# algbio/founderblockgraphs

Hardware: AMD Instinct MI355X
Metric: MSA columns segmented/sec (higher is better)
Workload: dtype u32

## Files before the change

founderblockgraphs_amd/csrc/ctx.hip:

```cpp
#include "fbg_internal.h"
#include <chrono>
#include <stdarg.h>
#include <stdio.h>
#include <ctype.h>
#include <string.h>
#include <algorithm>
#include <atomic>
#include <thread>
#include <vector>

static std::string g_global_err;

int fbg_fail(fbg_ctx *ctx, int code, const char *fmt, ...)
{
    char buf[1024];
    va_list ap;
    va_start(ap, fmt);
    vsnprintf(buf, sizeof(buf), fmt, ap);
    va_end(ap);
    if (ctx) ctx->err = buf; else g_global_err = buf;
    return code;
}

int fbg_reserve(fbg_ctx *ctx, DevBuf &b, size_t bytes, std::vector<DevBuf *> *owner, bool accounted)
{
    if (bytes == 0) bytes = 256;
    if (b.cap >= bytes) return FBG_OK;
    const auto t_begin = std::chrono::steady_clock::now();
    if (b.p) {
        FBG_HIP_TRY(ctx, hipStreamSynchronize(ctx->stream));
        FBG_HIP_TRY(ctx, hipFree(b.p));
        if (accounted) ctx->held_bytes -= b.cap;
        b.p = nullptr; b.cap = 0;
    }
    size_t want = (bytes + 255) & ~(size_t)255;
    hipError_t e = hipMalloc(&b.p, want);
    if (e != hipSuccess) {
        b.p = nullptr;
        return fbg_fail(ctx, FBG_ERR_OOM, "hipMalloc(%zu bytes) failed: %s (context already holds %llu bytes)",
                        want, hipGetErrorString(e), (unsigned long long)ctx->held_bytes);
    }
    b.cap = want;
    if (owner && !b.listed) { owner->push_back(&b); b.listed = true; }
    if (!accounted) return FBG_OK;
    ctx->held_bytes += want;
    ctx->alloc_calls++;
    ctx->alloc_us += (uint64_t)std::chrono::duration_cast<std::chrono::microseconds>(std::chrono::steady_clock::now() - t_begin).count();
    if (ctx->opt.poison) FBG_HIP_TRY(ctx, hipMemsetAsync(b.p, (int)(ctx->opt.poison & 255), want, ctx->stream));
    return FBG_OK;
}

void fbg_release(fbg_ctx *ctx, DevBuf &b)
{
    if (b.p) {
        (void)hipFree(b.p);
        if (ctx) ctx->held_bytes -= b.cap;
        b.p = nullptr; b.cap = 0;
    }
}

void fbg_release_all(fbg_ctx *ctx, std::vector<DevBuf *> &bufs)
{
    for (DevBuf *b : bufs) { fbg_release(ctx, *b); b->listed = false; }
    bufs.clear();
}

#define FBG_STAGE_SLOT (8u << 20)
#define FBG_STAGE_SLOTS 16
#define FBG_STAGE_MIN (32u << 20)

static bool host_pointer_is_pinned(const void *p)
{
    hipPointerAttribute_t at;
    const hipError_t e = hipPointerGetAttributes(&at, p);
    if (e != hipSuccess) { (void)hipGetLastError(); return false; }
    return at.type == hipMemoryTypeHost;
}

static int stager_ready(fbg_ctx *ctx)
{
    Stager &s = ctx->stager;
    if (s.base) return FBG_OK;
    FBG_HIP_TRY(ctx, hipHostMalloc(&s.base, (size_t)FBG_STAGE_SLOT * FBG_STAGE_SLOTS, hipHostMallocDefault));
    s.slot_bytes = FBG_STAGE_SLOT; s.nslots = FBG_STAGE_SLOTS;
    s.ev = new hipEvent_t[s.nslots];
    for (int i = 0; i < s.nslots; i++) FBG_HIP_TRY(ctx, hipEventCreateWithFlags(&s.ev[i], hipEventDisableTiming));
    FBG_HIP_TRY(ctx, hipStreamCreateWithFlags(&s.stream, hipStreamNonBlocking));
    return FBG_OK;
}

static int staged_copy(fbg_ctx *ctx, void *dst, const void *src, size_t bytes, bool to_device)
{
    FBG_HIP_TRY(ctx, hipSetDevice(ctx->device));
    FBG_HIP_TRY(ctx, hipStreamSynchronize(ctx->stream));
    const void *host = to_device ? src : dst;
    if (bytes < FBG_STAGE_MIN || host_pointer_is_pinned(host)) {
        FBG_HIP_TRY(ctx, hipMemcpyAsync(dst, src, bytes, to_device ? hipMemcpyHostToDevice : hipMemcpyDeviceToHost, ctx->stream));
        FBG_HIP_TRY(ctx, hipStreamSynchronize(ctx->stream));
        return FBG_OK;
    }
    FBG_TRY(stager_ready(ctx));
    Stager &s = ctx->stager;
    const size_t nchunks = (bytes + s.slot_bytes - 1) / s.slot_bytes;
    unsigned hw = std::thread::hardware_concurrency();
    int T = (int)std::min<size_t>(std::min<unsigned>(std::max(2u, hw / 2), 8u), nchunks);
    if (T > s.nslots / 2) T = s.nslots / 2;
    std::atomic<int> failed{0};
    auto worker = [&](int t) {
        if (hipSetDevice(ctx->device) != hipSuccess) { failed = 1; return; }
        const int slots[2] = {t, t + T};
        uint8_t *pins[2] = {static_cast<uint8_t *>(s.base) + (size_t)slots[0] * s.slot_bytes,
                            static_cast<uint8_t *>(s.base) + (size_t)slots[1] * s.slot_bytes};
        if (to_device) {
            size_t k = 0;
            for (size_t c = (size_t)t; c < nchunks && !failed; c += (size_t)T, k++) {
                const int w = (int)(k & 1);
                const size_t off = c * s.slot_bytes, len = std::min(s.slot_bytes, bytes - off);
                if (k >= 2 && hipEventSynchronize(s.ev[slots[w]]) != hipSuccess) { failed = 1; return; }
                memcpy(pins[w], static_cast<const uint8_t *>(src) + off, len);
                if (hipMemcpyAsync(static_cast<uint8_t *>(dst) + off, pins[w], len, hipMemcpyHostToDevice, s.stream) != hipSuccess ||
                    hipEventRecord(s.ev[slots[w]], s.stream) != hipSuccess) { failed = 1; return; }
            }
        } else {
            auto issue = [&](size_t c, int w) {
                const size_t off = c * s.slot_bytes, len = std::min(s.slot_bytes, bytes - off);
                return hipMemcpyAsync(pins[w], static_cast<const uint8_t *>(src) + off, len, hipMemcpyDeviceToHost, s.stream) == hipSuccess &&
                       hipEventRecord(s.ev[slots[w]], s.stream) == hipSuccess;
            };
            if ((size_t)t < nchunks && !issue((size_t)t, 0)) { failed = 1; return; }
            size_t k = 0;
            for (size_t c = (size_t)t; c < nchunks && !failed; c += (size_t)T, k++) {
                const int w = (int)(k & 1);
                if (c + (size_t)T < nchunks && !issue(c + (size_t)T, w ^ 1)) { failed = 1; return; }
                if (hipEventSynchronize(s.ev[slots[w]]) != hipSuccess) { failed = 1; return; }
                const size_t off = c * s.slot_bytes, len = std::min(s.slot_bytes, bytes - off);
                memcpy(static_cast<uint8_t *>(dst) + off, pins[w], len);
            }
        }
    };
    std::vector<std::thread> th;
    for (int t = 1; t < T; t++) th.emplace_back(worker, t);
    worker(0);
    for (auto &t : th) t.join();
    FBG_HIP_TRY(ctx, hipStreamSynchronize(s.stream));
    if (failed) return fbg_fail(ctx, FBG_ERR_HIP, "staged %s copy of %zu bytes failed: %s", to_device ? "host-to-device" : "device-to-host",
                                bytes, hipGetErrorString(hipGetLastError()));
    return FBG_OK;
}

int fbg_upload(fbg_ctx *ctx, void *d_dst, const void *h_src, size_t bytes) { return staged_copy(ctx, d_dst, h_src, bytes, true); }
int fbg_download(fbg_ctx *ctx, void *h_dst, const void *d_src, size_t bytes) { return staged_copy(ctx, h_dst, d_src, bytes, false); }

int fbg_stage_begin(fbg_ctx *ctx, int stage)
{
    StageTimer &t = ctx->timers[stage];
    if (!t.start) {
        FBG_HIP_TRY(ctx, hipEventCreate(&t.start));
        FBG_HIP_TRY(ctx, hipEventCreate(&t.stop));
    }
    t.recorded = false;
    FBG_HIP_TRY(ctx, hipEventRecord(t.start, ctx->stream));
    return FBG_OK;
}

int fbg_stage_end(fbg_ctx *ctx, int stage, int launches)
{
    StageTimer &t = ctx->timers[stage];
    FBG_HIP_TRY(ctx, hipEventRecord(t.stop, ctx->stream));
    t.recorded = true;
    t.launches = launches;
    return FBG_OK;
}

struct OptKey { const char *name; int64_t FbgOptions::*field; };
static const OptKey g_opt_keys[] = {
    {"no_ranked", &FbgOptions::no_ranked},
    {"no_packed", &FbgOptions::no_packed},
    {"force_wide", &FbgOptions::force_wide},
    {"full_keys", &FbgOptions::full_keys},
    {"no_msd_sort", &FbgOptions::no_msd_sort},
    {"msd_min", &FbgOptions::msd_min},
    {"bp_min", &FbgOptions::bp_min},
    {"record_scatter", &FbgOptions::record_scatter},
    {"lcp_text", &FbgOptions::lcp_text},
    {"no_aux_stream", &FbgOptions::no_aux_stream},
    {"rank_no_threshold", &FbgOptions::rank_no_threshold},
    {"dp_literal", &FbgOptions::dp_literal},
    {"dp_wave", &FbgOptions::dp_wave},
    {"dp_safe_window", &FbgOptions::dp_safe_window},
    {"dp_tile", &FbgOptions::dp_tile},
    {"pure_scan", &FbgOptions::pure_scan},
    {"gapped_rank", &FbgOptions::gapped_rank},
    {"part_tricks_off", &FbgOptions::part_tricks_off},
    {"msd_sample_bins", &FbgOptions::msd_sample_bins},
    {"msd_min_force", &FbgOptions::msd_min_force},
    {"msd_probe", &FbgOptions::msd_probe},
    {"msd_xcd", &FbgOptions::msd_xcd},
    {"rank_no_lean", &FbgOptions::rank_no_lean},
    {"no_stream_upload", &FbgOptions::no_stream_upload},
    {"span_scan", &FbgOptions::span_scan},
    {"span_key_flags", &FbgOptions::span_key_flags},
    {"span_slow_split", &FbgOptions::span_slow_split},
    {"poison", &FbgOptions::poison},
    {"dpw_matrix", &FbgOptions::dpw_matrix},
    {"dp_chain1", &FbgOptions::dp_chain1},
    {"msd_ext", &FbgOptions::msd_ext},
    {"rows_wave", &FbgOptions::rows_wave},
    {"pairs_in_scan", &FbgOptions::pairs_in_scan},
    {"runs_wave_min", &FbgOptions::runs_wave_min},
    {"wave_list_cap", &FbgOptions::wave_list_cap},
    {"cand_local_sort", &FbgOptions::cand_local_sort},
    {"cand_lds_cap", &FbgOptions::cand_lds_cap},
    {"cand_sort_check", &FbgOptions::cand_sort_check},
    {"tie_gallop", &FbgOptions::tie_gallop},
    {"cand_counts_fused", &FbgOptions::cand_counts_fused},
    {"tie_sample_loop", &FbgOptions::tie_sample_loop},
    {"row_count_fast", &FbgOptions::row_count_fast},
    {"twin_hash", &FbgOptions::twin_hash},
    {"front_one_fill", &FbgOptions::front_one_fill},
    {"scan_rows_ahead", &FbgOptions::scan_rows_ahead},
    {"msd_cursors", &FbgOptions::msd_cursors},
    {"msd_lds_batch", &FbgOptions::msd_lds_batch},
    {"path_batch_kib", &FbgOptions::path_batch_kib},
    {"byrow_max", &FbgOptions::byrow_max},
    {"byrow_lds", &FbgOptions::byrow_lds},
    {"graph_batch_kib", &FbgOptions::graph_batch_kib},
};

struct InfoKey { const char *name; int64_t (*get)(const fbg_ctx &); };
static const InfoKey g_info_keys[] = {
    {"grs_threshold", [](const fbg_ctx &c) -> int64_t { return c.grs_t; }},
    {"grs_redone", [](const fbg_ctx &c) -> int64_t { return (int64_t)c.grs_redone; }},
    {"dp_kind", [](const fbg_ctx &c) -> int64_t { return c.dp_kind; }},
    {"dp_attempts", [](const fbg_ctx &c) -> int64_t { return c.dp_attempts; }},
    {"ne_dp_kind", [](const fbg_ctx &c) -> int64_t { return c.ne_dp_kind; }},
    {"msd_decline", [](const fbg_ctx &c) -> int64_t { return c.diag.msd_decline; }},
    {"pass1_ahead", [](const fbg_ctx &c) -> int64_t { return c.diag.pass1_ahead; }},
    {"ext_pairs", [](const fbg_ctx &c) -> int64_t { return c.diag.ext_pairs; }},
    {"text_pairs", [](const fbg_ctx &c) -> int64_t { return c.diag.text_pairs; }},
    {"sample_twins", [](const fbg_ctx &c) -> int64_t { return c.diag.sample_twins; }},
    {"cand_inversions", [](const fbg_ctx &c) -> int64_t { return c.diag.cand_inversions; }},
    {"cand_local_sorted", [](const fbg_ctx &c) -> int64_t { return c.diag.cand_local_sorted; }},
    {"wave_runs", [](const fbg_ctx &c) -> int64_t { return c.diag.wave_runs; }},
    {"rank_lean_used", [](const fbg_ctx &c) -> int64_t { return c.diag.rank_lean_used; }},
    {"rank_lean_launched", [](const fbg_ctx &c) -> int64_t { return c.diag.rank_lean_launched; }},
    {"pairs_rb", [](const fbg_ctx &c) -> int64_t { return c.diag.pairs_rb; }},
    {"key_b", [](const fbg_ctx &c) -> int64_t { return c.key_b; }},
    {"key_K", [](const fbg_ctx &c) -> int64_t { return c.key_K; }},
    {"key_packed", [](const fbg_ctx &c) -> int64_t { return c.key_packed; }},
    {"key_compact", [](const fbg_ctx &c) -> int64_t { return c.key_compact; }},
    {"alloc_calls", [](const fbg_ctx &c) -> int64_t { return (int64_t)c.alloc_calls; }},
    {"alloc_us", [](const fbg_ctx &c) -> int64_t { return (int64_t)c.alloc_us; }},
    {"span_decline", [](const fbg_ctx &c) -> int64_t { return c.diag.sp_decline; }},
    {"span_key_flags_used", [](const fbg_ctx &c) -> int64_t { return c.ix.index_valid && c.ix.spanned() && c.ix.sp_key_flags_sorted; }},
    {"span_scan_used", [](const fbg_ctx &c) -> int64_t { return c.ix.index_valid && c.ix.spanned(); }},
    {"span_scan_work", [](const fbg_ctx &c) -> int64_t { return (int64_t)c.sp_work; }},
    {"span_groups", [](const fbg_ctx &c) -> int64_t { return (int64_t)c.sp_G; }},
    {"span_odd_groups", [](const fbg_ctx &c) -> int64_t { return (int64_t)c.sp_n_odd[0] + c.sp_n_odd[1] + c.sp_n_odd[2] + c.sp_n_odd[3]; }},
    {"span_irregular", [](const fbg_ctx &c) -> int64_t { return (int64_t)c.sp_n_irr; }},
    {"span_chain", [](const fbg_ctx &c) -> int64_t { return (int64_t)c.sp_chain_n; }},
    {"span_slow_groups", [](const fbg_ctx &c) -> int64_t { return (int64_t)c.sp_slow_n; }},
    {"index_kind", [](const fbg_ctx &c) -> int64_t { return !c.ix.index_valid ? -1 : c.ix.part_active ? 3 : c.ix.granked() ? 2 : c.ix.ranked() ? 1 : 0; }},
};

static void options_from_env(FbgOptions &o)
{
    auto env = [](const std::string &name) -> const char * { return getenv(name.c_str()); };
    const char *dbg = env("FBG_DEBUG_ENV");
    if (!dbg || strcmp(dbg, "1") != 0) return;
    for (const OptKey &k : g_opt_keys) {
        std::string name = "FBG_";
        for (const char *c = k.name; *c; c++) name += (char)toupper((unsigned char)*c);
        if (const char *v = env(name)) o.*(k.field) = *v ? strtoll(v, nullptr, 10) : 1;
    }
}

void fbg_index_reset(fbg_ctx *ctx)
{
    ctx->ix = IndexState();
    ctx->diag = BuildDiag();
}

static int host_dp_v(fbg_ctx *ctx, int (*dp)(fbg_ctx *, const uint64_t *, uint64_t, uint64_t *, uint64_t *, uint64_t *, uint64_t *), const char *name,
                     const uint64_t *v, uint64_t n, uint64_t *s_out, uint64_t *prev_out, uint64_t *boundaries_out, uint64_t *count_out)
{
    if (!ctx) return FBG_ERR_INVALID;
    if (!v || !boundaries_out || !count_out || n == 0 || n >= (1ull << 31))
        return fbg_fail(ctx, FBG_ERR_INVALID, "%s: bad arguments", name);
    FBG_HIP_TRY(ctx, hipSetDevice(ctx->device));
    size_t w = n * sizeof(uint64_t);
    for (DevBuf *b : {&ctx->io_a, &ctx->io_b, &ctx->io_c, &ctx->io_d}) FBG_TRY(fbg_reserve(ctx, *b, w));
    FBG_HIP_TRY(ctx, hipMemcpyAsync(ctx->io_a.p, v, w, hipMemcpyHostToDevice, ctx->stream));
    int rc = dp(ctx, ctx->io_a.as<uint64_t>(), n, ctx->io_c.as<uint64_t>(), ctx->io_d.as<uint64_t>(), ctx->io_b.as<uint64_t>(), count_out);
    if (rc != FBG_OK && rc != FBG_ERR_NO_SEGMENTATION) return rc;
    if (s_out) FBG_HIP_TRY(ctx, hipMemcpyAsync(s_out, ctx->io_c.p, w, hipMemcpyDeviceToHost, ctx->stream));
    if (prev_out) FBG_HIP_TRY(ctx, hipMemcpyAsync(prev_out, ctx->io_d.p, w, hipMemcpyDeviceToHost, ctx->stream));
    if (rc == FBG_OK)
        FBG_HIP_TRY(ctx, hipMemcpyAsync(boundaries_out, ctx->io_b.p, *count_out * sizeof(uint64_t),
                                        hipMemcpyDeviceToHost, ctx->stream));
    FBG_HIP_TRY(ctx, hipStreamSynchronize(ctx->stream));
    return rc;
}

extern "C" {

int fbg_set_option(fbg_ctx *ctx, const char *key, int64_t value)
{
    if (!ctx || !key) return FBG_ERR_INVALID;
    for (const OptKey &k : g_opt_keys)
        if (strcmp(k.name, key) == 0) { ctx->opt.*(k.field) = value; return FBG_OK; }
    return fbg_fail(ctx, FBG_ERR_INVALID, "fbg_set_option: unknown key '%s'", key);
}

int fbg_get_option(const fbg_ctx *ctx, const char *key, int64_t *value)
{
    if (!ctx || !key || !value) return FBG_ERR_INVALID;
    for (const OptKey &k : g_opt_keys)
        if (strcmp(k.name, key) == 0) { *value = ctx->opt.*(k.field); return FBG_OK; }
    for (const InfoKey &k : g_info_keys)
        if (strcmp(k.name, key) == 0) { *value = k.get(*ctx); return FBG_OK; }
    if (strncmp(key, "span_dbg", 8) == 0 && key[8] >= '0' && key[8] <= '7' && !key[9]) {
        unsigned long long v = 0;
        if (hipStreamSynchronize(ctx->stream) != hipSuccess || ctx->scalars.cap < FBG_SCALARS_BYTES ||
            hipMemcpy(&v, fbg_scalars(ctx)->span + 24 + (key[8] - '0'), 8, hipMemcpyDeviceToHost) != hipSuccess) return FBG_ERR_HIP;
        *value = (int64_t)v;
        return FBG_OK;
    }
    return FBG_ERR_INVALID;
}

void *fbg_host_alloc(uint64_t bytes)
{
    void *p = nullptr;
    if (hipHostMalloc(&p, bytes ? bytes : 1, hipHostMallocDefault) != hipSuccess) { (void)hipGetLastError(); return nullptr; }
    return p;
}
void fbg_host_free(void *p) { if (p) (void)hipHostFree(p); }

int fbg_ctx_create(int device, fbg_ctx **out)
{
    if (!out) return FBG_ERR_INVALID;
    *out = nullptr;
    int count = 0;
    hipError_t e = hipGetDeviceCount(&count);
    if (e != hipSuccess || count <= 0)
        return fbg_fail(nullptr, FBG_ERR_NO_DEVICE,
                        "no HIP device visible (%s); libfbg_hip has no CPU fallback",
                        e != hipSuccess ? hipGetErrorString(e) : "device count 0");
    if (device < 0 || device >= count)
        return fbg_fail(nullptr, FBG_ERR_INVALID, "device %d out of range (0..%d)", device, count - 1);
    e = hipSetDevice(device);
    if (e != hipSuccess) return fbg_fail(nullptr, FBG_ERR_HIP, "hipSetDevice: %s", hipGetErrorString(e));
    fbg_ctx *ctx = new fbg_ctx();
    ctx->device = device;
    options_from_env(ctx->opt);
    e = hipStreamCreateWithFlags(&ctx->stream, hipStreamNonBlocking);
    if (e != hipSuccess) {
        delete ctx;
        return fbg_fail(nullptr, FBG_ERR_HIP, "hipStreamCreate: %s", hipGetErrorString(e));
    }
    ctx->own_stream = true;
    *out = ctx;
    return FBG_OK;
}

void fbg_ctx_destroy(fbg_ctx *ctx)
{
    if (!ctx) return;
    (void)hipSetDevice(ctx->device);
    (void)hipStreamSynchronize(ctx->stream);
    fbg_release_all(ctx, ctx->bufs);
    fbg_msd_pre_free(ctx);
    if (ctx->up_stream) {
        (void)hipStreamSynchronize(ctx->up_stream);
        for (auto &e : ctx->up_ev) if (e) (void)hipEventDestroy(e);
        (void)hipStreamDestroy(ctx->up_stream);
    }
    for (auto &t : ctx->timers) {
        if (t.start) (void)hipEventDestroy(t.start);
        if (t.stop) (void)hipEventDestroy(t.stop);
    }
    if (ctx->stager.base) {
        for (int i = 0; i < ctx->stager.nslots; i++) (void)hipEventDestroy(ctx->stager.ev[i]);
        delete[] ctx->stager.ev;
        (void)hipStreamDestroy(ctx->stager.stream);
        (void)hipHostFree(ctx->stager.base);
    }
    if (ctx->pin_pair) (void)hipHostFree(ctx->pin_pair);
    if (ctx->pin_twins) (void)hipHostFree(ctx->pin_twins);
    if (ctx->twin_ev) (void)hipEventDestroy(ctx->twin_ev);
    if (ctx->pin_front) (void)hipHostFree(ctx->pin_front);
    if (ctx->aux_fork) (void)hipEventDestroy(ctx->aux_fork);
    if (ctx->aux_join) (void)hipEventDestroy(ctx->aux_join);
    if (ctx->aux) (void)hipStreamDestroy(ctx->aux);
    if (ctx->own_stream) (void)hipStreamDestroy(ctx->stream);
    delete ctx;
}

const char *fbg_last_error(const fbg_ctx *ctx) { return ctx ? ctx->err.c_str() : g_global_err.c_str(); }

int fbg_set_stream(fbg_ctx *ctx, void *hip_stream)
{
    if (!ctx) return FBG_ERR_INVALID;
    FBG_HIP_TRY(ctx, hipStreamSynchronize(ctx->stream));
    if (ctx->own_stream) { (void)hipStreamDestroy(ctx->stream); ctx->own_stream = false; }
    if (hip_stream) {
        ctx->stream = (hipStream_t)hip_stream;
    } else {
        FBG_HIP_TRY(ctx, hipStreamCreateWithFlags(&ctx->stream, hipStreamNonBlocking));
        ctx->own_stream = true;
    }
    return FBG_OK;
}

int fbg_stage_ms(fbg_ctx *ctx, int stage, float *ms, int *launches)
{
    if (!ctx || stage < 0 || stage >= FBG_STAGE_COUNT) return FBG_ERR_INVALID;
    StageTimer &t = ctx->timers[stage];
    if (ms) *ms = 0.f;
    if (launches) *launches = 0;
    if (!t.recorded) return FBG_OK;
    FBG_HIP_TRY(ctx, hipEventSynchronize(t.stop));
    float v = 0.f;
    FBG_HIP_TRY(ctx, hipEventElapsedTime(&v, t.start, t.stop));
    if (ms) *ms = v;
    if (launches) *launches = t.launches;
    return FBG_OK;
}

uint64_t fbg_device_bytes(const fbg_ctx *ctx) { return ctx ? ctx->held_bytes : 0; }

int fbg_release_scratch(fbg_ctx *ctx)
{
    if (!ctx) return FBG_ERR_INVALID;
    FBG_HIP_TRY(ctx, hipSetDevice(ctx->device));
    FBG_HIP_TRY(ctx, hipStreamSynchronize(ctx->stream));
    const bool sorted_in_A = (ctx->ix.ranked() || ctx->ix.granked()) && ctx->ix.rk_keys == ctx->keysA.as<uint64_t>();
    const DevBuf *keep[] = {
        &ctx->msa_own, &ctx->text, &ctx->pos, &ctx->tot, &ctx->segtab, &ctx->colT, &ctx->gwin_rows,
        &ctx->valsB, sorted_in_A ? &ctx->keysA : &ctx->keysB,
        &ctx->prow, &ctx->igrow, &ctx->rec, &ctx->xlist, &ctx->gmax, &ctx->excol, &ctx->xslot, &ctx->xbits, &ctx->exc, &ctx->exc_scratch,
        &ctx->big_groups, &ctx->gwin, &ctx->gbits, &ctx->sp_cwin, &ctx->sp_gstart, &ctx->sp_gcol, &ctx->sp_gflags, &ctx->sp_rstart, &ctx->sp_rid,
        &ctx->sp_gplo, &ctx->sp_gphi, &ctx->sp_gval, &ctx->sp_odd, &ctx->sp_irr, &ctx->sp_chain, &ctx->sp_slow, &ctx->sp_mins,
        &ctx->small, &ctx->scalars, &ctx->kargs, &ctx->io_a, &ctx->io_b, &ctx->io_c, &ctx->io_d, &ctx->bt_up, &ctx->bt_dep};
    for (DevBuf *b : ctx->bufs)
        if (std::find(std::begin(keep), std::end(keep), b) == std::end(keep)) fbg_release(ctx, *b);
    return FBG_OK;
}

int fbg_sync(fbg_ctx *ctx)
{
    if (!ctx) return FBG_ERR_INVALID;
    FBG_HIP_TRY(ctx, hipStreamSynchronize(ctx->stream));
    return FBG_OK;
}

static int check_dims(fbg_ctx *ctx, uint64_t m, uint64_t n)
{
    if (!ctx) return FBG_ERR_INVALID;
    if (m == 0 || n == 0) return fbg_fail(ctx, FBG_ERR_INVALID, "empty MSA (m=%llu, n=%llu)",
                                          (unsigned long long)m, (unsigned long long)n);
    if (n >= (1ull << 31) || m * (n + 1) + 1 >= (1ull << 40))
        return fbg_fail(ctx, FBG_ERR_TOO_LARGE, "MSA of %llu x %llu cells is beyond this engine (n < 2^31, text < 2^40)",
                        (unsigned long long)m, (unsigned long long)n);
    return FBG_OK;
}

int fbg_msa_set_device(fbg_ctx *ctx, const uint8_t *d_msa, uint64_t m, uint64_t n)
{
    FBG_TRY(check_dims(ctx, m, n));
    if (!d_msa) return fbg_fail(ctx, FBG_ERR_INVALID, "null MSA pointer");
    ctx->d_msa = d_msa; ctx->m = m; ctx->n = n; ctx->ix.index_valid = false;
    return FBG_OK;
}

int fbg_msa_load_host(fbg_ctx *ctx, const uint8_t *msa, uint64_t m, uint64_t n)
{
    FBG_TRY(check_dims(ctx, m, n));
    if (!msa) return fbg_fail(ctx, FBG_ERR_INVALID, "null MSA pointer");
    FBG_HIP_TRY(ctx, hipSetDevice(ctx->device));
    FBG_TRY(fbg_reserve(ctx, ctx->msa_own, m * n));
    FBG_TRY(fbg_upload(ctx, ctx->msa_own.p, msa, m * n));
    ctx->d_msa = ctx->msa_own.as<uint8_t>(); ctx->m = m; ctx->n = n; ctx->ix.index_valid = false;
    return FBG_OK;
}

int fbg_index_build(fbg_ctx *ctx, int reversed, const uint8_t *ignore_chars, uint64_t ignore_len)
{
    if (!ctx) return FBG_ERR_INVALID;
    if (!ctx->d_msa) return fbg_fail(ctx, FBG_ERR_INVALID, "fbg_index_build: no MSA set");
    FBG_HIP_TRY(ctx, hipSetDevice(ctx->device));
    for (int st : {FBG_STAGE_SORT_PASS1, FBG_STAGE_SORT_PASS2, FBG_STAGE_SORT_PASS3, FBG_STAGE_RANK_KERNEL}) {
        ctx->timers[st].recorded = false;
        ctx->timers[st].launches = 0;
    }
    fbg_index_reset(ctx);
    ctx->reversed = reversed ? 1 : 0;
    FBG_TRY(fbg_build_text(ctx, reversed ? nullptr : ignore_chars, reversed ? 0 : ignore_len));
    FBG_TRY(fbg_suffix_sort(ctx));
    FBG_TRY(fbg_neighbour_lcp(ctx));
    if (ctx->N > 1500000000ull) {
        size_t free_b = 0, total_b = 0;
        FBG_HIP_TRY(ctx, hipMemGetInfo(&free_b, &total_b));
        if (free_b < total_b / 2) FBG_TRY(fbg_release_scratch(ctx));
    }
    ctx->ix.index_valid = true;
    return FBG_OK;
}

int fbg_part_index_build(fbg_ctx *ctx, int reversed, int part, int nparts, void *d_blob, int *ok)
{
    return fbg_part_index_build_ignore(ctx, reversed, part, nparts, nullptr, 0, d_blob, ok);
}

int fbg_part_index_build_ignore(fbg_ctx *ctx, int reversed, int part, int nparts, const uint8_t *ignore_chars, uint64_t ignore_len, void *d_blob, int *ok)
{
    if (!ctx) return FBG_ERR_INVALID;
    if (!ctx->d_msa) return fbg_fail(ctx, FBG_ERR_INVALID, "fbg_part_index_build: no MSA set");
    if (!d_blob || !ok || nparts < 1 || part < 0 || part >= nparts || (ignore_len && !ignore_chars))
        return fbg_fail(ctx, FBG_ERR_INVALID, "fbg_part_index_build: bad arguments");
    FBG_HIP_TRY(ctx, hipSetDevice(ctx->device));
    fbg_index_reset(ctx);
    ctx->reversed = reversed ? 1 : 0;
    ctx->allow_wide = true;
    const int rc = fbg_build_text(ctx, reversed ? nullptr : ignore_chars, reversed ? 0 : ignore_len);
    ctx->allow_wide = false;
    FBG_TRY(rc);
    return fbg_part_sort(ctx, part, nparts, static_cast<uint8_t *>(d_blob), ok);
}

int fbg_part_scan(fbg_ctx *ctx, const void *d_blobs, uint32_t *d_gmax, int *ok)
{
    if (!ctx) return FBG_ERR_INVALID;
    if (!ctx->ix.part_active || ctx->ix.index_valid)
        return fbg_fail(ctx, FBG_ERR_INVALID, "fbg_part_scan needs fbg_part_index_build first");
    if (!d_blobs || !d_gmax || !ok) return fbg_fail(ctx, FBG_ERR_INVALID, "fbg_part_scan: bad arguments");
    FBG_HIP_TRY(ctx, hipSetDevice(ctx->device));
    if (ctx->ix.gpart) return fbg_grs_part_scan(ctx, static_cast<const uint8_t *>(d_blobs), d_gmax, ok);
    return fbg_rank_part_runs(ctx, static_cast<const uint8_t *>(d_blobs), d_gmax, ok);
}

int fbg_part_finish(fbg_ctx *ctx, const uint32_t *d_gmax, int *ok)
{
    if (!ctx) return FBG_ERR_INVALID;
    if (!ctx->ix.part_active || ctx->ix.index_valid)
        return fbg_fail(ctx, FBG_ERR_INVALID, "fbg_part_finish needs fbg_part_scan first");
    if (!d_gmax || !ok) return fbg_fail(ctx, FBG_ERR_INVALID, "fbg_part_finish: bad arguments");
    FBG_HIP_TRY(ctx, hipSetDevice(ctx->device));
    uint32_t verdict = 1;
    FBG_HIP_TRY(ctx, hipMemcpyAsync(ctx->gmax.p, d_gmax, (ctx->n + 1) * 4, hipMemcpyDeviceToDevice, ctx->stream));
    FBG_HIP_TRY(ctx, hipMemcpyAsync(&verdict, d_gmax + ctx->n, 4, hipMemcpyDeviceToHost, ctx->stream));
    FBG_HIP_TRY(ctx, hipStreamSynchronize(ctx->stream));
    *ok = verdict == 0;
    if (*ok) {
        uint64_t unfilled = 0;
        if (ctx->ix.gpart) FBG_TRY(fbg_grs_part_unfilled(ctx, &unfilled));
        else FBG_TRY(fbg_rank_part_unfilled(ctx, &unfilled));
        if (unfilled) { *ok = 2; return FBG_OK; }
        ctx->ix.n_exc = 0; ctx->ix.index_valid = true;
        ctx->ix.kind = ctx->ix.gpart ? IndexKind::gapped : IndexKind::ranked;
    }
    return FBG_OK;
}

int fbg_part_rescan(fbg_ctx *ctx, uint32_t *d_gmax)
{
    if (!ctx) return FBG_ERR_INVALID;
    if (!ctx->ix.part_active || ctx->ix.index_valid)
        return fbg_fail(ctx, FBG_ERR_INVALID, "fbg_part_rescan follows a fbg_part_finish that returned *ok = 2");
    if (!d_gmax) return fbg_fail(ctx, FBG_ERR_INVALID, "fbg_part_rescan: bad arguments");
    FBG_HIP_TRY(ctx, hipSetDevice(ctx->device));
    uint32_t verdict = 0;
    if (ctx->ix.gpart) { FBG_TRY(fbg_grs_part_rescan(ctx)); verdict = ctx->grs_part_failed ? 1u : 0u; }
    else FBG_TRY(fbg_rank_part_rescan(ctx));
    FBG_HIP_TRY(ctx, hipMemcpyAsync(d_gmax, ctx->gmax.p, (ctx->n + 1) * 4, hipMemcpyDeviceToDevice, ctx->stream));
    FBG_HIP_TRY(ctx, hipMemcpyAsync(d_gmax + ctx->n, &verdict, 4, hipMemcpyHostToDevice, ctx->stream));
    FBG_HIP_TRY(ctx, hipStreamSynchronize(ctx->stream));
    return FBG_OK;
}

int fbg_scan_f(fbg_ctx *ctx, uint64_t x0, uint64_t x1, int disable_tricks, uint64_t *d_f)
{
    if (!ctx) return FBG_ERR_INVALID;
    if (!ctx->ix.index_valid || ctx->reversed)
        return fbg_fail(ctx, FBG_ERR_INVALID, "fbg_scan_f needs fbg_index_build(reversed=0) first");
    if (x0 > x1 || x1 > ctx->n || !d_f) return fbg_fail(ctx, FBG_ERR_INVALID, "fbg_scan_f: bad column range");
    FBG_HIP_TRY(ctx, hipSetDevice(ctx->device));
    return fbg_scan_columns(ctx, x0, x1, FBG_SCAN_F, disable_tricks, d_f);
}

int fbg_scan_v(fbg_ctx *ctx, uint64_t x0, uint64_t x1, uint64_t *d_v)
{
    if (!ctx) return FBG_ERR_INVALID;
    if (!ctx->ix.index_valid || !ctx->reversed)
        return fbg_fail(ctx, FBG_ERR_INVALID, "fbg_scan_v needs fbg_index_build(reversed=1) first");
    if (x0 > x1 || x1 > ctx->n || !d_v) return fbg_fail(ctx, FBG_ERR_INVALID, "fbg_scan_v: bad column range");
    FBG_HIP_TRY(ctx, hipSetDevice(ctx->device));
    return fbg_scan_columns(ctx, x0, x1, FBG_SCAN_V, 1, d_v);
}

int fbg_minmax_dp_device(fbg_ctx *ctx, const uint64_t *d_f, uint64_t n, uint64_t *d_boundaries,
                         uint64_t *count_out, uint64_t *d_mml, uint64_t *d_bt)
{
    if (!ctx) return FBG_ERR_INVALID;
    if (!d_f || !d_boundaries || !count_out || n == 0 || n >= (1ull << 31))
        return fbg_fail(ctx, FBG_ERR_INVALID, "fbg_minmax_dp_device: bad arguments");
    FBG_HIP_TRY(ctx, hipSetDevice(ctx->device));
    return fbg_dp_minmax(ctx, d_f, n, d_boundaries, count_out, d_mml, d_bt);
}

int fbg_repeatfree_dp_device(fbg_ctx *ctx, const uint64_t *d_v, uint64_t n, uint64_t *d_s,
                             uint64_t *d_prev, uint64_t *d_boundaries, uint64_t *count_out)
{
    if (!ctx) return FBG_ERR_INVALID;
    if (!d_v || !d_boundaries || !count_out || n == 0 || n >= (1ull << 31))
        return fbg_fail(ctx, FBG_ERR_INVALID, "fbg_repeatfree_dp_device: bad arguments");
    FBG_HIP_TRY(ctx, hipSetDevice(ctx->device));
    return fbg_dp_repeatfree(ctx, d_v, n, d_s, d_prev, d_boundaries, count_out);
}

int fbg_scan_gapped_v(fbg_ctx *ctx, uint64_t *d_v)
{
    if (!ctx) return FBG_ERR_INVALID;
    if (!ctx->ix.index_valid || ctx->reversed)
        return fbg_fail(ctx, FBG_ERR_INVALID, "fbg_scan_gapped_v needs fbg_index_build(reversed=0) first");
    if (!d_v) return fbg_fail(ctx, FBG_ERR_INVALID, "fbg_scan_gapped_v: null d_v");
    FBG_HIP_TRY(ctx, hipSetDevice(ctx->device));
    const uint64_t n = ctx->n;
    FBG_TRY(fbg_reserve(ctx, ctx->io_d, n * sizeof(uint64_t)));
    uint64_t *d_f = ctx->io_d.as<uint64_t>();
    FBG_HIP_TRY(ctx, hipMemsetAsync(d_f, 0, n * sizeof(uint64_t), ctx->stream));
    FBG_TRY(fbg_scan_columns(ctx, 0, n, FBG_SCAN_F, 1, d_f));
    return fbg_gapped_v_from_f(ctx, d_f, n, d_v);
}

int fbg_gapped_dp_device(fbg_ctx *ctx, const uint64_t *d_v, uint64_t n, uint64_t *d_s,
                         uint64_t *d_prev, uint64_t *d_boundaries, uint64_t *count_out)
{
    if (!ctx) return FBG_ERR_INVALID;
    if (!d_v || !d_boundaries || !count_out || n == 0 || n >= (1ull << 31))
        return fbg_fail(ctx, FBG_ERR_INVALID, "fbg_gapped_dp_device: bad arguments");
    FBG_HIP_TRY(ctx, hipSetDevice(ctx->device));
    return fbg_dp_gapped(ctx, d_v, n, d_s, d_prev, d_boundaries, count_out);
}


int fbg_elastic_f(fbg_ctx *ctx, const uint8_t *msa, uint64_t m, uint64_t n, const uint8_t *ignore_chars,
                  uint64_t ignore_len, int disable_tricks, uint64_t *f)
{
    if (!ctx) return FBG_ERR_INVALID;
    if (!f) return fbg_fail(ctx, FBG_ERR_INVALID, "fbg_elastic_f: null f");
    if (msa && ignore_len == 0 && !ctx->opt.no_stream_upload && m * n >= FBG_STAGE_MIN && host_pointer_is_pinned(msa) && check_dims(ctx, m, n) == FBG_OK) {
        FBG_HIP_TRY(ctx, hipSetDevice(ctx->device));
        FBG_HIP_TRY(ctx, hipStreamSynchronize(ctx->stream));
        FBG_TRY(fbg_reserve(ctx, ctx->msa_own, m * n));
        ctx->d_msa = ctx->msa_own.as<uint8_t>(); ctx->m = m; ctx->n = n; ctx->ix.index_valid = false;
        ctx->up_host = msa;
        const int rc = fbg_index_build(ctx, 0, ignore_chars, ignore_len);
        ctx->up_host = nullptr;
        if (ctx->up_stream) (void)hipStreamSynchronize(ctx->up_stream);
        if (rc != FBG_OK) return rc;
    } else {
        FBG_TRY(fbg_msa_load_host(ctx, msa, m, n));
        FBG_TRY(fbg_index_build(ctx, 0, ignore_chars, ignore_len));
    }
    FBG_TRY(fbg_reserve(ctx, ctx->io_a, n * sizeof(uint64_t)));
    FBG_HIP_TRY(ctx, hipMemcpyAsync(ctx->io_a.p, f, n * sizeof(uint64_t), hipMemcpyHostToDevice, ctx->stream));
    FBG_TRY(fbg_scan_f(ctx, 0, n, disable_tricks, ctx->io_a.as<uint64_t>()));
    FBG_HIP_TRY(ctx, hipMemcpyAsync(f, ctx->io_a.p, n * sizeof(uint64_t), hipMemcpyDeviceToHost, ctx->stream));
    FBG_HIP_TRY(ctx, hipStreamSynchronize(ctx->stream));
    if (disable_tricks && f[0] == n)
        return fbg_fail(ctx, FBG_ERR_NO_SEGMENTATION, "No valid segmentation found!");
    return FBG_OK;
}

int fbg_minmax_dp(fbg_ctx *ctx, const uint64_t *f, uint64_t n, uint64_t *boundaries_out, uint64_t *count_out,
                  uint64_t *minmaxlength_out, uint64_t *backtrack_out)
{
    if (!ctx) return FBG_ERR_INVALID;
    if (!f || !boundaries_out || !count_out || n == 0 || n >= (1ull << 31))
        return fbg_fail(ctx, FBG_ERR_INVALID, "fbg_minmax_dp: bad arguments");
    FBG_HIP_TRY(ctx, hipSetDevice(ctx->device));
    size_t w = (n + 1) * sizeof(uint64_t);
    for (DevBuf *b : {&ctx->io_a, &ctx->io_b, &ctx->io_c, &ctx->io_d}) FBG_TRY(fbg_reserve(ctx, *b, w));
    FBG_HIP_TRY(ctx, hipMemcpyAsync(ctx->io_a.p, f, n * sizeof(uint64_t), hipMemcpyHostToDevice, ctx->stream));
    int rc = fbg_dp_minmax(ctx, ctx->io_a.as<uint64_t>(), n, ctx->io_b.as<uint64_t>(), count_out,
                           ctx->io_c.as<uint64_t>(), ctx->io_d.as<uint64_t>());
    if (rc != FBG_OK && rc != FBG_ERR_NO_SEGMENTATION) return rc;
    if (minmaxlength_out)
        FBG_HIP_TRY(ctx, hipMemcpyAsync(minmaxlength_out, ctx->io_c.p, w, hipMemcpyDeviceToHost, ctx->stream));
    if (backtrack_out)
        FBG_HIP_TRY(ctx, hipMemcpyAsync(backtrack_out, ctx->io_d.p, w, hipMemcpyDeviceToHost, ctx->stream));
    if (rc == FBG_OK)
        FBG_HIP_TRY(ctx, hipMemcpyAsync(boundaries_out, ctx->io_b.p, *count_out * sizeof(uint64_t),
                                        hipMemcpyDeviceToHost, ctx->stream));
    FBG_HIP_TRY(ctx, hipStreamSynchronize(ctx->stream));
    return rc;
}

int fbg_repeatfree_v(fbg_ctx *ctx, const uint8_t *msa, uint64_t m, uint64_t n, uint64_t *v)
{
    if (!ctx) return FBG_ERR_INVALID;
    if (!v) return fbg_fail(ctx, FBG_ERR_INVALID, "fbg_repeatfree_v: null v");
    FBG_TRY(fbg_msa_load_host(ctx, msa, m, n));
    FBG_TRY(fbg_index_build(ctx, 1, nullptr, 0));
    FBG_TRY(fbg_reserve(ctx, ctx->io_a, n * sizeof(uint64_t)));
    FBG_TRY(fbg_scan_v(ctx, 0, n, ctx->io_a.as<uint64_t>()));
    FBG_HIP_TRY(ctx, hipMemcpyAsync(v, ctx->io_a.p, n * sizeof(uint64_t), hipMemcpyDeviceToHost, ctx->stream));
    FBG_HIP_TRY(ctx, hipStreamSynchronize(ctx->stream));
    return FBG_OK;
}

int fbg_repeatfree_dp(fbg_ctx *ctx, const uint64_t *v, uint64_t n, uint64_t *s_out, uint64_t *prev_out,
                      uint64_t *boundaries_out, uint64_t *count_out)
{
    return host_dp_v(ctx, fbg_dp_repeatfree, "fbg_repeatfree_dp", v, n, s_out, prev_out, boundaries_out, count_out);
}

int fbg_gapped_v(fbg_ctx *ctx, const uint8_t *msa, uint64_t m, uint64_t n, uint64_t *v)
{
    if (!ctx) return FBG_ERR_INVALID;
    if (!v) return fbg_fail(ctx, FBG_ERR_INVALID, "fbg_gapped_v: null v");
    FBG_TRY(fbg_msa_load_host(ctx, msa, m, n));
    FBG_TRY(fbg_index_build(ctx, 0, nullptr, 0));
    FBG_TRY(fbg_reserve(ctx, ctx->io_a, n * sizeof(uint64_t)));
    FBG_TRY(fbg_scan_gapped_v(ctx, ctx->io_a.as<uint64_t>()));
    FBG_HIP_TRY(ctx, hipMemcpyAsync(v, ctx->io_a.p, n * sizeof(uint64_t), hipMemcpyDeviceToHost, ctx->stream));
    FBG_HIP_TRY(ctx, hipStreamSynchronize(ctx->stream));
    return FBG_OK;
}

int fbg_gapped_dp(fbg_ctx *ctx, const uint64_t *v, uint64_t n, uint64_t *s_out, uint64_t *prev_out,
                  uint64_t *boundaries_out, uint64_t *count_out)
{
    return host_dp_v(ctx, fbg_dp_gapped, "fbg_gapped_dp", v, n, s_out, prev_out, boundaries_out, count_out);
}

uint64_t fbg_text_length(const fbg_ctx *ctx) { return ctx && ctx->ix.index_valid ? ctx->N : 0; }

int fbg_index_download(fbg_ctx *ctx, uint8_t *text, uint32_t *sa, uint32_t *isa, uint32_t *lcp_prev,
                       uint32_t *lcp_next)
{
    if (!ctx) return FBG_ERR_INVALID;
    if (!ctx->ix.index_valid) return fbg_fail(ctx, FBG_ERR_INVALID, "fbg_index_download: no index");
    if (ctx->ix.part_active) return fbg_fail(ctx, FBG_ERR_INVALID, "fbg_index_download: the index is partitioned over several GPUs");
    if (ctx->N >= (1ull << 32)) return fbg_fail(ctx, FBG_ERR_TOO_LARGE, "fbg_index_download: 32-bit arrays");
    if (ctx->ix.spanned() && (sa || isa || lcp_prev || lcp_next))
        return fbg_fail(ctx, FBG_ERR_INVALID, "fbg_index_download: the group-level scan (span_scan.hip) leaves the suffixes with equal keys unordered; "
                                              "set option span_scan = -1 for an index with a suffix array");
    size_t N = ctx->N;
    FBG_HIP_TRY(ctx, hipStreamSynchronize(ctx->stream));
    if (text) FBG_HIP_TRY(ctx, hipMemcpy(text, ctx->text.p, N, hipMemcpyDeviceToHost));
    if (sa && !ctx->ix.ranked() && !ctx->ix.granked()) FBG_HIP_TRY(ctx, hipMemcpy(sa, ctx->ix.sa_ptr, N * 4, hipMemcpyDeviceToHost));
    if ((sa || isa || lcp_prev || lcp_next) && (ctx->ix.ranked() || ctx->ix.granked())) {
        for (DevBuf *b : {&ctx->io_a, &ctx->io_b, &ctx->io_c, &ctx->io_d}) FBG_TRY(fbg_reserve(ctx, *b, N * 4));
        if (ctx->ix.granked())
            FBG_TRY(fbg_grs_materialize(ctx, ctx->io_d.as<uint32_t>(), ctx->io_a.as<uint32_t>(), ctx->io_b.as<uint32_t>(), ctx->io_c.as<uint32_t>()));
        else
            FBG_TRY(fbg_rank_materialize(ctx, ctx->io_d.as<uint32_t>(), ctx->io_a.as<uint32_t>(), ctx->io_b.as<uint32_t>(),
                                         ctx->io_c.as<uint32_t>()));
        FBG_HIP_TRY(ctx, hipStreamSynchronize(ctx->stream));
        if (sa) FBG_HIP_TRY(ctx, hipMemcpy(sa, ctx->io_d.p, N * 4, hipMemcpyDeviceToHost));
        if (isa) FBG_HIP_TRY(ctx, hipMemcpy(isa, ctx->io_a.p, N * 4, hipMemcpyDeviceToHost));
        if (lcp_prev) FBG_HIP_TRY(ctx, hipMemcpy(lcp_prev, ctx->io_b.p, N * 4, hipMemcpyDeviceToHost));
        if (lcp_next) FBG_HIP_TRY(ctx, hipMemcpy(lcp_next, ctx->io_c.p, N * 4, hipMemcpyDeviceToHost));
    } else if (isa || lcp_prev || lcp_next) {
        uint32_t *dst[3] = {isa, lcp_prev, lcp_next};
        for (int w = 0; w < 3; w++) {
            if (!dst[w]) continue;
            FBG_HIP_TRY(ctx, hipMemcpy2DAsync(dst[w], 4, (const char *)ctx->rec.p + 4 * w, 16, 4, N,
                                              hipMemcpyDeviceToHost, ctx->stream));
        }
        FBG_HIP_TRY(ctx, hipStreamSynchronize(ctx->stream));
        for (int w = 1; w < 3; w++)
            if (dst[w]) for (size_t k = 0; k < N; k++) dst[w][k] &= 0x7fffffffu;
    }
    FBG_HIP_TRY(ctx, hipStreamSynchronize(ctx->stream));
    return FBG_OK;
}

}
```

founderblockgraphs_amd/csrc/fbg_internal.h:

```cpp
#pragma once
#include <cstddef>
#include <cstring>
#include <cstdlib>
#include <hip/hip_runtime.h>
#include <stdint.h>
#include <string>
#include <vector>
#include "../../include/fbg_hip.h"

#define FBG_WAVE 64

struct DevBuf {
    void *p = nullptr;
    size_t cap = 0;
    bool listed = false;
    template <class T> T *as() const { return reinterpret_cast<T *>(p); }
};

struct Stager {
    void *base = nullptr;
    size_t slot_bytes = 0;
    int nslots = 0;
    hipEvent_t *ev = nullptr;
    hipStream_t stream = nullptr;
};

struct StageTimer {
    hipEvent_t start = nullptr, stop = nullptr;
    bool recorded = false;
    int launches = 0;
};

struct FbgOptions {
    int64_t no_ranked = 0, no_packed = 0, force_wide = 0, full_keys = 0, no_msd_sort = 0, msd_min = -1, bp_min = -1,
            record_scatter = 0, lcp_text = 0, no_aux_stream = 0, rank_no_threshold = 0, dp_literal = 0, dp_wave = 0,
            dp_safe_window = 0, dp_tile = 0, pure_scan = 0, gapped_rank = 0, part_tricks_off = 0, msd_sample_bins = 0, msd_min_force = 0, msd_probe = 0, msd_xcd = -1, rank_no_lean = 0, no_stream_upload = 0,
            span_scan = 0, span_key_flags = 0, span_slow_split = 0, poison = 0, dpw_matrix = 0, dp_chain1 = 0, msd_ext = 1, rows_wave = 0,
            pairs_in_scan = 1, runs_wave_min = 16, wave_list_cap = 0,
            cand_local_sort = 1, cand_lds_cap = 0, cand_sort_check = 0,
            tie_gallop = 1, cand_counts_fused = 1, tie_sample_loop = 1,
            row_count_fast = 1, twin_hash = 1, front_one_fill = 1,
            scan_rows_ahead = 0, msd_cursors = 1, msd_lds_batch = 1,
            path_batch_kib = 1 << 20, byrow_max = 1024, byrow_lds = 0, graph_batch_kib = 1 << 20;
};

enum class IndexKind { none, record, ranked, gapped, span };

struct IndexState {
    bool index_valid = false;
    IndexKind kind = IndexKind::none;
    bool ranked() const { return kind == IndexKind::ranked; }
    bool granked() const { return kind == IndexKind::gapped || kind == IndexKind::span; }
    bool spanned() const { return kind == IndexKind::span; }
    uint32_t *sa_ptr = nullptr;
    uint64_t *rk_keys = nullptr;
    int rk_b = 0, rk_key_bits = 0, rk_K = 0;
    int rk_layout = 0, rk_pb = 0;
    bool grs_flagged = false;
    bool sp_key_flags_sorted = false;
    bool msd_ext_valid = false;
    bool lcp_from_keys = false;
    bool grs_ties_done = false;
    uint32_t n_exc = 0;
    bool part_active = false;
    bool gpart = false;
    int part = 0, nparts = 1;
    uint64_t part_count = 0;
    uint64_t part_T = 0;
    uint32_t part_gmin = 0;
};

struct BuildDiag {
    int64_t msd_decline = -1;
    int pass1_ahead = 0;
    int64_t ext_pairs = -1, text_pairs = -1;
    int64_t sample_twins = -1;
    int64_t wave_runs = -1;
    int64_t cand_inversions = -1;
    int cand_local_sorted = -1;
    int rank_lean_launched = 0;
    int rank_lean_used = 0;
    int pairs_rb = -1;
    int sp_decline = 0;
};

struct SortExtras {
    const uint64_t *ebits = nullptr;
    const uint32_t *payload = nullptr;
    bool key_flags = false;
};

struct MsdPlan;
struct fbg_ctx {
    int device = 0;
    FbgOptions opt;
    std::string err;
    hipStream_t stream = nullptr;
    bool own_stream = false;
    hipStream_t aux = nullptr;
    hipEvent_t aux_fork = nullptr, aux_join = nullptr;
    bool aux_pending = false;
    uint32_t *pin_pair = nullptr;
    unsigned long long *pin_twins = nullptr;
    hipEvent_t twin_ev = nullptr;
    bool twin_pending = false;
    unsigned long long *pin_front = nullptr;
    Stager stager;
    StageTimer timers[FBG_STAGE_COUNT];

    const uint8_t *d_msa = nullptr;
    DevBuf msa_own;
    uint64_t m = 0, n = 0;
    int reversed = 0;
    bool gapfree = true;
    bool have_ignore = false;
    uint8_t ignore_tab[256] = {0};
    uint64_t N = 0;
    uint64_t byte_hist[256] = {0};
    bool allow_wide = false;
    uint32_t mp = 0;
    DevBuf text;
    DevBuf pos, tot;
    DevBuf segtab;
    DevBuf colT;
    DevBuf gwin_rows;

    const uint8_t *up_host = nullptr;
    hipStream_t up_stream = nullptr;
    hipEvent_t up_ev[9] = {};
    bool pre_pass1 = false;
    uint64_t pre_symbols[4] = {0, 0, 0, 0};
    MsdPlan *pre_plan = nullptr;
    uint64_t pre_tiles = 0;

    IndexState ix;
    BuildDiag diag;
    int key_b = -1, key_K = -1, key_packed = -1, key_compact = -1;
    int dp_kind = -1;
    int dp_attempts = 0;
    int ne_dp_kind = -1;
    bool grs_skip = false;
    bool cells_built = false;
    uint64_t held_bytes = 0;
    uint64_t alloc_calls = 0, alloc_us = 0;
    std::vector<DevBuf *> bufs;

    DevBuf prow;
    DevBuf igrow;
    DevBuf rec;
    DevBuf xlist;
    DevBuf gmax, excol, xslot;
    DevBuf xbits;
    DevBuf exc_scratch;
    DevBuf exc;
    int grs_tricks_off = 0;
    uint32_t grs_ign_lo = 0, grs_ign_hi = 0;
    DevBuf gwin;
    DevBuf gbits;
    bool pairs_similar = false;
    bool grs_part_failed = false;
    uint32_t grs_t = 1;
    uint64_t grs_redone = 0;
    DevBuf sp_cells;
    DevBuf sp_flagT;
    DevBuf sp_cwin;
    DevBuf sp_tiles, sp_gstart, sp_gcol, sp_gflags, sp_rstart, sp_rid, sp_gplo, sp_gphi, sp_gval, sp_odd, sp_irr, sp_chain, sp_slow, sp_mins;
    uint32_t sp_chain_n = 0, sp_slow_n = 0;
    uint64_t sp_G = 0, sp_R = 0, sp_n_irr = 0, sp_work = 0;
    uint32_t sp_n_odd[4] = {0, 0, 0, 0}, sp_odd_cap = 0;

    DevBuf keysA, keysB, valsA, valsB, grp, flags, list, tie_list, big_groups, tmp, small, scalars;
    DevBuf msd_ext;
    DevBuf wave_list;
    DevBuf kargs;
    alignas(16) unsigned char kargs_host[512];
    uint8_t code_host[256];
    DevBuf msd_w, msd_v;
    DevBuf dp_a, dp_b, dp_c, dp_d, dp_e, dp_f, dp_g, dp_h, io_a, io_b, io_c, io_d;
    DevBuf bt_up, bt_dep;
    DevBuf ps_a, ps_b, ps_c, ps_d, ps_e, ps_f, ps_g, ps_h;
};

int fbg_fail(fbg_ctx *ctx, int code, const char *fmt, ...);
#define FBG_HIP_TRY(ctx, expr)                                                              \
    do {                                                                                    \
        hipError_t e_ = (expr);                                                             \
        if (e_ != hipSuccess)                                                               \
            return fbg_fail((ctx), e_ == hipErrorOutOfMemory ? FBG_ERR_OOM : FBG_ERR_HIP,   \
                            "%s failed: %s (%s:%d)", #expr, hipGetErrorString(e_), __FILE__, \
                            __LINE__);                                                      \
    } while (0)
#define FBG_TRY(expr)                \
    do {                             \
        int rc_ = (expr);            \
        if (rc_ != FBG_OK) return rc_; \
    } while (0)

int fbg_reserve(fbg_ctx *ctx, DevBuf &b, size_t bytes, std::vector<DevBuf *> *owner, bool accounted);
inline int fbg_reserve(fbg_ctx *ctx, DevBuf &b, size_t bytes) { return fbg_reserve(ctx, b, bytes, &ctx->bufs, true); }

struct FbgScalars {
    alignas(64) unsigned long long front[8];
    unsigned long long sample_count;
    alignas(64) unsigned long long dp[16];
    unsigned long long scan_exceptions;
    alignas(64) unsigned long long rank[8];
    unsigned long long rank_hist[32];
    alignas(64) unsigned long long pure[4];
    alignas(64) unsigned long long msd[4];
    unsigned long long sample_twins;
    unsigned long long graph_collision;
    unsigned long long pair_stats[2];
    unsigned long long cand_inversions;
    unsigned long long by_position;
    alignas(64) unsigned long long gapped[8 + 66];
    alignas(64) unsigned long long span[34];
};
constexpr size_t FBG_SCALARS_WORDS = 256, FBG_SCALARS_BYTES = FBG_SCALARS_WORDS * sizeof(unsigned long long);
static_assert(sizeof(FbgScalars) <= FBG_SCALARS_BYTES, "the scalar words fit their buffer, whose size is part of fbg_device_bytes");
static_assert(offsetof(FbgScalars, rank_hist) == offsetof(FbgScalars, rank) + sizeof(FbgScalars::rank), "one fill clears counters and histogram");
inline int fbg_reserve_scalars(fbg_ctx *ctx) { return fbg_reserve(ctx, ctx->scalars, FBG_SCALARS_BYTES); }
inline FbgScalars *fbg_scalars(const fbg_ctx *ctx) { return ctx->scalars.as<FbgScalars>(); }

struct FbgSmall {
    alignas(2048) uint8_t ignore_tab[256];
    alignas(2048) uint8_t code_tab[256];
    alignas(2048) unsigned long long hist[256];
};
constexpr size_t FBG_SMALL_BYTES = 8192;
static_assert(sizeof(FbgSmall) <= FBG_SMALL_BYTES, "the byte tables fit their buffer");
inline FbgSmall *fbg_small(const fbg_ctx *ctx) { return ctx->small.as<FbgSmall>(); }

template <class F> int fbg_with_tmp(fbg_ctx *ctx, DevBuf &tmp, std::vector<DevBuf *> *owner, bool accounted, F &&call)
{
    size_t bytes = 0;
    hipError_t e = call(nullptr, bytes);
    if (e != hipSuccess) return fbg_fail(ctx, FBG_ERR_HIP, "rocprim size query: %s", hipGetErrorString(e));
    FBG_TRY(fbg_reserve(ctx, tmp, bytes, owner, accounted));
    size_t have = tmp.cap;
    e = call(tmp.p, have);
    if (e != hipSuccess)
        return fbg_fail(ctx, e == hipErrorOutOfMemory ? FBG_ERR_OOM : FBG_ERR_HIP, "rocprim call: %s", hipGetErrorString(e));
    return FBG_OK;
}
template <class F> int fbg_with_tmp(fbg_ctx *ctx, F &&call) { return fbg_with_tmp(ctx, ctx->tmp, &ctx->bufs, true, call); }

void fbg_release(fbg_ctx *ctx, DevBuf &b);
void fbg_release_all(fbg_ctx *ctx, std::vector<DevBuf *> &bufs);
void fbg_index_reset(fbg_ctx *ctx);
int fbg_upload(fbg_ctx *ctx, void *d_dst, const void *h_src, size_t bytes);
int fbg_download(fbg_ctx *ctx, void *h_dst, const void *d_src, size_t bytes);
int fbg_stage_begin(fbg_ctx *ctx, int stage);
int fbg_stage_end(fbg_ctx *ctx, int stage, int launches);

#define FBG_SLOTS_PAIRS 0
#define FBG_SLOTS_PACKED 1
#define FBG_SLOTS_WIDE 2
struct KeyGeom {
    int b = 0, K = 0, key_bits = 0;
    bool compact = false, packed = false;
    bool wide = false;
    int pb = 0;
    const uint8_t *d_code = nullptr;
};

inline void fbg_remember_slots(fbg_ctx *ctx, uint64_t *keys, uint32_t *vals, int layout, const KeyGeom &g)
{
    ctx->ix.rk_keys = keys; ctx->ix.sa_ptr = vals; ctx->ix.rk_layout = layout; ctx->ix.rk_pb = g.pb;
    ctx->ix.rk_b = g.b; ctx->ix.rk_key_bits = g.key_bits; ctx->ix.rk_K = g.K;
}

inline void fbg_note_key_geom(fbg_ctx *ctx, const KeyGeom &g)
{
    ctx->key_b = g.b; ctx->key_K = g.K; ctx->key_packed = g.packed ? 1 : 0; ctx->key_compact = g.compact ? 1 : 0;
}

int fbg_build_text(fbg_ctx *ctx, const uint8_t *ignore, uint64_t ignore_len);
int fbg_suffix_sort(fbg_ctx *ctx);
int fbg_neighbour_lcp(fbg_ctx *ctx);
int fbg_rank_scan_try(fbg_ctx *ctx, uint64_t *keys, uint32_t *vals, const KeyGeom &g, int *done);
int fbg_pure_scan_try(fbg_ctx *ctx, uint64_t *keys, uint32_t *vals, const KeyGeom &g, int *done);
int fbg_rank_finish(fbg_ctx *ctx, uint64_t x0, uint64_t x1, int mode, int disable_tricks, uint64_t *d_out);
int fbg_rank_materialize(fbg_ctx *ctx, uint32_t *d_sa, uint32_t *d_isa, uint32_t *d_pl, uint32_t *d_pr);
#define FBG_STAGE_RANKSCAN FBG_STAGE_TILE
int fbg_grs_prepare(fbg_ctx *ctx, const uint64_t **ebits, int *launches);
int fbg_grs_part_classify(fbg_ctx *ctx, uint64_t *keys, uint32_t *vals, uint64_t count, const KeyGeom &g, int eligible, uint8_t *d_blob, int *ok);
int fbg_grs_part_scan(fbg_ctx *ctx, const uint8_t *d_blobs, uint32_t *d_gmax, int *ok);
int fbg_grs_part_unfilled(fbg_ctx *ctx, uint64_t *unfilled);
int fbg_grs_part_rescan(fbg_ctx *ctx);
int fbg_grs_strip(fbg_ctx *ctx, uint32_t *vals);
int fbg_grs_try(fbg_ctx *ctx, uint64_t *keys, uint32_t *vals, const KeyGeom &g, int *done);
int fbg_grs_finish(fbg_ctx *ctx, uint64_t x0, uint64_t x1, int disable_tricks, uint64_t *d_out, int *ok);
int fbg_grs_materialize(fbg_ctx *ctx, uint32_t *d_sa, uint32_t *d_isa, uint32_t *d_pl, uint32_t *d_pr);
bool fbg_span_eligible(fbg_ctx *ctx, const KeyGeom &g);
bool fbg_span_key_flags(fbg_ctx *ctx, KeyGeom &g);
int fbg_span_prepare(fbg_ctx *ctx, const KeyGeom &g, const SortExtras &x, int *launches);
int fbg_span_try(fbg_ctx *ctx, uint64_t *keys, uint32_t *vals, const KeyGeom &g, int *done);
int fbg_span_rescan(fbg_ctx *ctx, int disable_tricks, int *ok);
int fbg_build_cell_tables(fbg_ctx *ctx);
int fbg_key_setup(fbg_ctx *ctx, bool compact, KeyGeom *g, int *launches);
int fbg_rank_part_classify(fbg_ctx *ctx, uint64_t *keys, uint32_t *vals, uint64_t count, const KeyGeom &g, int pre_ok,
                           uint8_t *d_blob, int *ok);
int fbg_rank_part_runs(fbg_ctx *ctx, const uint8_t *d_blobs, uint32_t *d_gmax, int *ok);
int fbg_rank_part_unfilled(fbg_ctx *ctx, uint64_t *unfilled);
int fbg_rank_part_rescan(fbg_ctx *ctx);
int fbg_part_sort(fbg_ctx *ctx, int part, int nparts, uint8_t *d_blob, int *ok);
int fbg_msd_sort(fbg_ctx *ctx, const KeyGeom &g, uint64_t **sorted, int *ok, int *launches);
int fbg_msd_pre_begin(fbg_ctx *ctx, int *ok);
int fbg_msd_pre_pass1(fbg_ctx *ctx, uint64_t avail);
bool fbg_msd_pre_geom(fbg_ctx *ctx, KeyGeom *g);
void fbg_msd_pre_free(fbg_ctx *ctx);
int fbg_msd_sort_part(fbg_ctx *ctx, const KeyGeom &g, uint64_t lo, uint64_t hi, int nohi, int nparts, uint64_t out_offset,
                      uint64_t *count, int *ok, int *launches);
int fbg_sample_sort_pairs(fbg_ctx *ctx, const KeyGeom &g, const SortExtras &x, int *ok, int *launches);
int fbg_scan_columns(fbg_ctx *ctx, uint64_t x0, uint64_t x1, int mode, int disable_tricks,
                     uint64_t *d_out);
int fbg_dp_minmax(fbg_ctx *ctx, const uint64_t *d_f, uint64_t n, uint64_t *d_boundaries,
                  uint64_t *count_out, uint64_t *d_mml, uint64_t *d_bt);
struct BlockGraphDev {
    const uint64_t *bounds = nullptr;
    const uint32_t *node_of = nullptr, *rep_row = nullptr, *count = nullptr;
    const unsigned long long *first = nullptr, *edge_count = nullptr, *edges = nullptr;
    uint64_t n_nodes = 0;
    bool collision = false;
};
int fbg_block_graph_device(fbg_ctx *ctx, const uint64_t *boundaries, uint64_t nb, BlockGraphDev *g);
int fbg_dp_repeatfree(fbg_ctx *ctx, const uint64_t *d_v, uint64_t n, uint64_t *d_s,
                      uint64_t *d_prev, uint64_t *d_boundaries, uint64_t *count_out);
int fbg_gapped_v_from_f(fbg_ctx *ctx, const uint64_t *d_f, uint64_t n, uint64_t *d_v);
int fbg_dp_gapped(fbg_ctx *ctx, const uint64_t *d_v, uint64_t n, uint64_t *d_s, uint64_t *d_prev,
                  uint64_t *d_boundaries, uint64_t *count_out);

#define FBG_SCAN_F 0
#define FBG_SCAN_V 1

static inline unsigned fbg_blocks(uint64_t work, unsigned per_block, unsigned cap = 0x7fffffffu)
{
    uint64_t b = (work + per_block - 1) / per_block;
    if (b < 1) b = 1;
    if (b > cap) b = cap;
    return (unsigned)b;
}
```

founderblockgraphs_amd/csrc/host/host_selftest.cpp:

```cpp
#include <cstdio>
#include <cstdlib>
#include <string>
#include <vector>
#include "fasta.hpp"
#include "xgfa.hpp"
#include "../tie_extent.h"
#include "../twin_hash.h"
#include "../pindex_stage.h"

static int tie_extent_selftest()
{
    const uint32_t cap = 8192;
    std::vector<uint32_t> sizes;
    for (uint32_t s = 1; s <= 70; s++) sizes.push_back(s);
    for (uint32_t s = 8191; s <= 8194; s++) sizes.push_back(s);
    unsigned long long cases = 0;
    for (const uint32_t s : sizes)
        for (int where = 0; where < 3; where++) {
            const uint64_t before = where == 0 ? 0 : 37, after = where == 2 ? 0 : 29;
            std::vector<uint64_t> keys;
            for (uint64_t i = 0; i < before; i++) keys.push_back(10 + i / 3);
            const uint64_t key = 1000;
            for (uint32_t i = 0; i < s; i++) keys.push_back(key);
            for (uint64_t i = 0; i < after; i++) keys.push_back(2000 + i / 2);
            const uint64_t k0 = before;
            uint64_t reads = 0;
            auto key_at = [&](uint64_t k) -> uint64_t {
                reads++;
                if (k >= keys.size()) { std::fprintf(stderr, "tie_extent: read of slot %llu beyond the array\n", (unsigned long long)k); std::exit(1); }
                return keys[k];
            };
            std::vector<uint64_t> his = {keys.size()};
            for (uint64_t cut = 0; cut <= 3 && cut < s; cut++) his.push_back(k0 + s - cut);
            for (const uint64_t hi : his) {
                uint32_t want = 1;
                while (k0 + want < hi && want <= cap && keys[k0 + want] == key) want++;
                reads = 0;
                const uint32_t got = fbg_tie_extent(k0, hi, cap, key, key_at);
                const uint64_t most = FBG_TIE_PROBE + 2 * 14;
                if (got != want || reads > most) {
                    std::printf("tie_extent differs: size %u position %d hi %llu: got %u, want %u, %llu reads\n", s, where,
                                (unsigned long long)hi, got, want, (unsigned long long)reads);
                    return 1;
                }
                cases++;
            }
        }
    std::printf("tie_extent ok %llu\n", cases);
    return 0;
}

static int pindex_stages_selftest()
{
    std::printf("stages");
    for (int s = 0; s < PS_COUNT; s++) std::printf(" %s", ps_table[s].name);
    std::printf("\n");
    for (int x = 0; x < PS_COUNT; x++) {
        bool done[PS_COUNT] = {};
        for (int s = 0; s < PS_COUNT; s++) ps_finish(done, (PsStage)s);
        ps_begin(done, (PsStage)x);
        std::printf("begin %s", ps_table[x].name);
        for (int s = 0; s < PS_COUNT; s++)
            if (done[s]) std::printf(" %s", ps_table[s].name);
        std::printf("\n");
    }
    for (unsigned mask = 0; mask < 1u << PS_COUNT; mask++) {
        bool done[PS_COUNT] = {};
        for (int s = 0; s < PS_COUNT; s++)
            if (mask >> s & 1) ps_finish(done, (PsStage)s);
        std::printf("need %u", mask);
        for (int y = 0; y < PS_COUNT; y++) {
            const int miss = ps_missing(done, (PsStage)y);
            std::printf(" %s", miss == PS_COUNT ? "-" : ps_table[miss].name);
        }
        std::printf("\n");
    }
    return 0;
}

static int twin_hash_selftest(const char *path, int bits, bool slots_only)
{
    FILE *fh = std::fopen(path, "rb");
    if (!fh || bits < 1 || bits > 30) { std::fprintf(stderr, "twin-hash: cannot read %s, or BITS not in 1 .. 30\n", path); return 2; }
    std::vector<uint64_t> keys;
    uint64_t k;
    while (std::fread(&k, 8, 1, fh) == 1) keys.push_back(k);
    std::fclose(fh);
    if (slots_only) {
        for (const uint64_t key : keys) std::printf("%llu\n", (unsigned long long)fbg_twin_slot(key, bits));
        return 0;
    }
    std::vector<uint64_t> table((1ull << bits) + 2, FBG_TWIN_EMPTY);
    uint64_t *counters = table.data() + (1ull << bits);
    uint64_t longest = 0;
    for (const uint64_t key : keys) {
        if (key == FBG_TWIN_EMPTY) { counters[1]++; continue; }
        uint64_t probes = 0;
        counters[0] += fbg_twin_insert(key, bits, [&](uint64_t slot, uint64_t kk) -> uint64_t {
            if (slot >= (1ull << bits)) { std::fprintf(stderr, "twin-hash: slot %llu beyond the table\n", (unsigned long long)slot); std::exit(1); }
            probes++;
            const uint64_t seen = table[slot];
            if (seen == FBG_TWIN_EMPTY) table[slot] = kk;
            return seen;
        });
        if (probes > longest) longest = probes;
    }
    std::printf("twin_hash %llu %llu\n", (unsigned long long)fbg_twin_total(counters[0], counters[1]), (unsigned long long)longest);
    return 0;
}

int main(int argc, char **argv)
{
    if (argc == 4 && (std::string(argv[1]) == "twin-hash" || std::string(argv[1]) == "twin-slots"))
        return twin_hash_selftest(argv[2], std::atoi(argv[3]), std::string(argv[1]) == "twin-slots");
    if (argc == 2 && std::string(argv[1]) == "tie-extent") return tie_extent_selftest();
    if (argc == 2 && std::string(argv[1]) == "pindex-stages") return pindex_stages_selftest();
    if (argc < 6) {
        std::fprintf(stderr, "usage: %s FASTA GAP_LIMIT ELASTIC PATHS OUT.gfa [BOUNDARY ...]\n", argv[0]);
        return 2;
    }
    Msa msa;
    if (!read_msa(argv[1], std::atol(argv[2]), std::atoi(argv[3]) != 0, std::atoi(argv[4]) != 0, msa)) {
        std::fprintf(stderr, "cannot read %s\n", argv[1]);
        return 3;
    }
    std::printf("%llu %llu\n", (unsigned long long)msa.m, (unsigned long long)msa.n);
    if (argc == 6 || msa.m == 0) return 0;
    std::vector<uint64_t> boundaries;
    int first_boundary = 6;
    BlockGraph g;
    bool have_graph = false;
    if (std::string(argv[6]).rfind("GRAPH=", 0) == 0) {
        first_boundary = 7;
        have_graph = true;
        FILE *fh = std::fopen(argv[6] + 6, "rb");
        uint64_t hdr[2];
        if (!fh || std::fread(hdr, 8, 2, fh) != 2) { std::fprintf(stderr, "cannot read %s\n", argv[6] + 6); return 5; }
        const uint64_t nb = hdr[0], m = hdr[1];
        g.node_of.resize(nb * m); g.rep_row.resize(nb * m); g.first_node.resize(nb + 1); g.edge_count.resize(nb); g.edges.resize(nb * m);
        const bool ok = std::fread(g.node_of.data(), 4, nb * m, fh) == nb * m && std::fread(g.rep_row.data(), 4, nb * m, fh) == nb * m &&
                        std::fread(g.first_node.data(), 8, nb + 1, fh) == nb + 1 && std::fread(g.edge_count.data(), 8, nb, fh) == nb &&
                        std::fread(g.edges.data(), 8, nb * m, fh) == nb * m;
        std::fclose(fh);
        if (!ok || m != msa.m) { std::fprintf(stderr, "%s does not hold the arrays of this MSA\n", argv[6] + 6); return 5; }
    }
    for (int i = first_boundary; i < argc; i++) boundaries.push_back(std::strtoull(argv[i], nullptr, 10));
    std::string error;
    const bool paths = std::atoi(argv[4]) != 0;
    if (!(have_graph ? write_xgfa_graph(msa, boundaries, g, paths, argv[5], error) : write_xgfa(msa, boundaries, paths, argv[5], error))) {
        std::fprintf(stderr, "%s\n", error.c_str());
        return 4;
    }
    const GraphStats st = segment_stats(msa, boundaries);
    std::printf("%llu %llu %llu %llu\n", (unsigned long long)st.nodes, (unsigned long long)st.total_label_length,
                (unsigned long long)st.founders, (unsigned long long)st.edges);
    return 0;
}
```

founderblockgraphs_amd/csrc/rank_scan.hip:

```cpp
#include <algorithm>
#include <cstring>
#include <vector>
#include "fbg_internal.h"
#include "text_cmp.h"
#include <rocprim/rocprim.hpp>

#include "rank_common.h"
#include "tie_extent.h"

#define RS_ITEMS 4
#define RS_THREADS 256
#define RS_CHUNK (RS_THREADS * RS_ITEMS)

template <int L, bool PLAIN> __global__ __launch_bounds__(RS_THREADS) __attribute__((amdgpu_waves_per_eu(7, 8))) void k_rank_scan(RankArgs a)
{
    __shared__ uint64_t skey[RS_CHUNK + 2 * RS_HALO];
    __shared__ uint32_t srem[RS_CHUNK + 2 * RS_HALO];
    __shared__ uint16_t sq[RS_CHUNK];
    __shared__ uint32_t sqn, s_cand_n, s_tie_n;
    const int lane = threadIdx.x & 63;
    const uint64_t nchunks = (a.own_hi - a.own_lo + RS_CHUNK - 1) / RS_CHUNK;
    if (threadIdx.x == 0) { s_cand_n = 0; s_tie_n = 0; }
    uint64_t w[RS_ITEMS + 1];
    uint32_t v[RS_ITEMS + 1];
    const int my_i = RS_HALO + RS_ITEMS * (int)threadIdx.x;
    const int halo_i = (int)threadIdx.x < RS_HALO ? (int)threadIdx.x : RS_CHUNK + (int)threadIdx.x;
    auto fetch = [&](uint64_t c) {
        const uint64_t base = a.own_lo + c * RS_CHUNK;
        const int lo_i = c == 0 ? RS_HALO : 0;
        const int hi_i = (int)min((uint64_t)(RS_CHUNK + 2 * RS_HALO), a.own_hi - base + RS_HALO);
#pragma unroll
        for (int r = 0; r < RS_ITEMS; r++) {
            w[r] = 0; v[r] = 0;
            if (my_i + r < hi_i) {
                w[r] = a.keys[base + (uint64_t)(my_i + r - RS_HALO)];
                if (L != FBG_SLOTS_PACKED) v[r] = a.vals[base + (uint64_t)(my_i + r - RS_HALO)];
            }
        }
        w[RS_ITEMS] = 0; v[RS_ITEMS] = 0;
        if (threadIdx.x < 2 * RS_HALO && halo_i >= lo_i && halo_i < hi_i) {
            w[RS_ITEMS] = a.keys[base + halo_i - RS_HALO];
            if (L != FBG_SLOTS_PACKED) v[RS_ITEMS] = a.vals[base + halo_i - RS_HALO];
        }
    };
    if (blockIdx.x < nchunks) fetch(blockIdx.x);
    for (uint64_t c = blockIdx.x; c < nchunks; c += gridDim.x) {
        const uint64_t base = a.own_lo + c * RS_CHUNK;
        const int lo_i = c == 0 ? RS_HALO : 0;
        const int hi_i = (int)min((uint64_t)(RS_CHUNK + 2 * RS_HALO), a.own_hi - base + RS_HALO);
        if (threadIdx.x == 0) sqn = 0;
        uint64_t kk[RS_ITEMS + 6];
        uint32_t cc[RS_ITEMS + 4];
#pragma unroll
        for (int r = 0; r < RS_ITEMS; r++) {
            uint64_t key = 0;
            uint32_t rem = 0;
            if (my_i + r < hi_i) {
                key = w[r] >> a.pb;
                rem = rs_rem<L>(a, rs_pos_of<L>(a, w[r], v[r]));
            }
            kk[r + 3] = key; cc[r + 2] = rem;
            skey[my_i + r] = key; srem[my_i + r] = rem;
        }
        if (threadIdx.x < 2 * RS_HALO) {
            uint64_t key = 0;
            uint32_t rem = 0;
            if (halo_i >= lo_i && halo_i < hi_i) {
                key = w[RS_ITEMS] >> a.pb;
                rem = rs_rem<L>(a, rs_pos_of<L>(a, w[RS_ITEMS], v[RS_ITEMS]));
            }
            skey[halo_i] = key; srem[halo_i] = rem;
        }
        __syncthreads();
        if (c + gridDim.x < nchunks) fetch(c + gridDim.x);
#pragma unroll
        for (int j = 0; j < 3; j++) {
            kk[j] = __shfl_up(kk[RS_ITEMS + j], 1, 64);
            kk[RS_ITEMS + 3 + j] = __shfl_down(kk[3 + j], 1, 64);
        }
#pragma unroll
        for (int j = 0; j < 2; j++) {
            cc[j] = __shfl_up(cc[RS_ITEMS + j], 1, 64);
            cc[RS_ITEMS + 2 + j] = __shfl_down(cc[2 + j], 1, 64);
        }
        if (lane == 0) {
#pragma unroll
            for (int j = 0; j < 3; j++) kk[j] = skey[my_i - 3 + j];
            cc[0] = srem[my_i - 2]; cc[1] = srem[my_i - 1];
        }
        if (lane == 63) {
#pragma unroll
            for (int j = 0; j < 3; j++) kk[RS_ITEMS + 3 + j] = skey[my_i + RS_ITEMS + j];
            cc[RS_ITEMS + 2] = srem[my_i + RS_ITEMS]; cc[RS_ITEMS + 3] = srem[my_i + RS_ITEMS + 1];
        }
        uint32_t upd_g[RS_ITEMS], upd_c[RS_ITEMS];
#pragma unroll
        for (int r = 0; r < RS_ITEMS; r++) { upd_g[r] = 0; upd_c[r] = 0; }
        uint32_t slow4 = 0, tie4 = 0, cand4 = 0;
        uint32_t lcp[RS_ITEMS + 1];
#pragma unroll
        for (int r = 0; r <= RS_ITEMS; r++) lcp[r] = PLAIN ? rs_key_lcp(kk[r + 2], kk[r + 3], a.b, a.key_bits) : 0u;
#pragma unroll
        for (int r = 0; r < RS_ITEMS; r++) {
            const int i = my_i + r;
            const bool in = i < hi_i;
            const bool window = i - 3 >= lo_i && i + 3 < hi_i;
            const uint64_t key = kk[r + 3];
            const uint32_t rem = cc[r + 2];
            const bool eqp = kk[r + 2] == key, eqn = kk[r + 4] == key;
            bool slow = in && !window;
            bool want_cand = false, want_cand2 = false, want_tie = false;
            if (window) {
                const bool prev_tie = kk[r + 1] == kk[r + 2], next_tie = kk[r + 5] == kk[r + 4];
                if (!eqp && !eqn) {
                    if (rem != 0) {
                        if ((prev_tie && kk[r] == kk[r + 1]) || (next_tie && kk[r + 6] == kk[r + 5])) slow = true;
                        else {
                            bool run = cc[r + 1] == rem || cc[r + 3] == rem;
                            uint32_t mrp = cc[r + 1], mrn = cc[r + 3];
                            if (prev_tie) { run = run || cc[r] == rem; mrp = max(mrp, cc[r]); }
                            if (next_tie) { run = run || cc[r + 4] == rem; mrn = max(mrn, cc[r + 4]); }
                            if (run) want_cand = true;
                            else if (PLAIN) {
                                const uint32_t g = max(min(lcp[r], min(rem, mrp)), min(lcp[r + 1], min(rem, mrn))) + 1;
                                if (g >= a.g_min || rem <= 64) { upd_g[r] = g; upd_c[r] = rs_col_of_rem(a, rem); }
                            } else if (rem <= 64) slow = true;
                        }
                    }
                } else if (!eqp && kk[r + 5] != key && i + 4 < hi_i) {
                    const uint32_t r1 = cc[r + 3], rb = cc[r + 1], ra = cc[r + 4];
                    const bool simple = rem >= (uint32_t)a.K && r1 >= (uint32_t)a.K && rem != r1 &&
                                        !prev_tie && rb != rem && rb != r1 &&
                                        kk[r + 6] != kk[r + 5] && ra != rem && ra != r1;
                    if (simple) want_tie = true;
                    else { want_cand = true; want_cand2 = true; }
                } else if (!(eqp && !eqn && kk[r + 1] != key && i - 4 >= lo_i)) slow = true;
            }
            slow4 |= (slow ? 1u : 0u) << r;
            tie4 |= (want_tie ? 1u : 0u) << r;
            cand4 |= ((want_cand ? 1u : 0u) << r) | ((want_cand2 ? 16u : 0u) << r);
        }
        for (uint32_t bits = slow4; __ballot(bits != 0);) {
            const bool on = bits != 0;
            const int rr = on ? __ffs((int)bits) - 1 : 0;
            bits &= bits - 1;
            const unsigned long long smask = __ballot(on);
            uint32_t qb = 0;
            const int leader = __ffsll((long long)smask) - 1;
            if (lane == leader) qb = atomicAdd(&sqn, (uint32_t)__popcll(smask));
            qb = __shfl(qb, leader, 64);
            if (on) sq[qb + (uint32_t)__popcll(smask & ((1ull << lane) - 1))] = (uint16_t)(my_i + rr);
        }
        if (!a.values_only) {
            const uint32_t k_first = (uint32_t)(base + (uint64_t)(my_i - RS_HALO));
            for (uint32_t bits = tie4; __ballot(bits != 0);) {
                const bool on = bits != 0;
                const int rr = on ? __ffs((int)bits) - 1 : 0;
                bits &= bits - 1;
                rs_append(on, &s_tie_n, a.ties, a.tie_region, k_first + (uint32_t)rr);
            }
            for (uint32_t bits = cand4; __ballot(bits != 0);) {
                const bool on = bits != 0;
                const int rr = on ? __ffs((int)bits) - 1 : 0;
                bits &= bits - 1;
                rs_append(on, &s_cand_n, a.cand, a.region, k_first + (uint32_t)(rr & 3) + (uint32_t)(rr >> 2));
            }
        }
        uint32_t cur[RS_ITEMS];
#pragma unroll
        for (int r = 0; r < RS_ITEMS; r++) cur[r] = (PLAIN && upd_g[r]) ? a.gmax[upd_c[r]] : 0xffffffffu;
        __syncthreads();
        {
            const uint32_t qn = sqn;
            for (uint32_t q0 = 0; q0 < qn; q0 += RS_THREADS) {
                if (q0 + (threadIdx.x & ~63u) >= qn) break;
                const uint32_t q = q0 + threadIdx.x;
                bool want_cand = false, want_tie = false;
                uint64_t k = 0;
                if (q < qn) {
                    const int i = sq[q];
                    k = base + (uint64_t)(i - RS_HALO);
                    const bool is_tie = (i > lo_i && skey[i - 1] == skey[i]) || (i + 1 < hi_i && skey[i + 1] == skey[i]);
                    if (!(a.values_only && is_tie)) rank_scan_slow(a, RsLdsView{skey, srem}, i, lo_i, hi_i, k, want_cand, want_tie);
                }
                if (!a.values_only) {
                    rs_append(want_cand, &s_cand_n, a.cand, a.region, (uint32_t)k);
                    rs_append(want_tie, &s_tie_n, a.ties, a.tie_region, (uint32_t)k);
                }
            }
        }
        if (PLAIN) {
#pragma unroll
            for (int r = 0; r < RS_ITEMS; r++)
                if (cur[r] < upd_g[r]) atomicMax(&a.gmax[upd_c[r]], upd_g[r]);
        }
        __syncthreads();
    }
    if (threadIdx.x == 0 && !a.values_only) { a.blk_count[blockIdx.x] = s_cand_n; a.tie_count[blockIdx.x] = s_tie_n; }
}

#define RL_EV_LO 3
#define RL_EV_HI 60
#define RL_EV (RL_EV_HI - RL_EV_LO + 1)
#define RL_THREADS 256
#define RL_WAVES (RL_THREADS / 64)
#define RL_LIST 128

struct LeanArgs {
    const uint64_t *keys;
    const uint8_t *ext;
    uint64_t own_lo, own_hi;
    uint32_t per_wave, pmask;
    int pb;
    float inv_row_len, eps, one_minus_eps, near_end;
};

__device__ __forceinline__ uint32_t rl_from_next(uint32_t v) { return (uint32_t)__builtin_amdgcn_update_dpp(0, (int)v, 0x130, 0xf, 0xf, false); }
__device__ __forceinline__ uint32_t rl_lanes_below(unsigned long long m)
{
    return __builtin_amdgcn_mbcnt_hi((uint32_t)(m >> 32), __builtin_amdgcn_mbcnt_lo((uint32_t)m, 0u));
}

__device__ __attribute__((noinline)) void rl_noted(const RankArgs &a, const uint2 *list, uint32_t n, uint32_t *s_pair_n, uint32_t *s_code_n)
{
    const int lane = threadIdx.x & 63;
    bool keep = (uint32_t)lane < n;
    const uint2 p = keep ? list[lane] : make_uint2(0u, 0u);
    if (a.pairs_in_scan) {
        const uint32_t c = (p.x >> 30) | (((p.y >> 30) & 1u) << 2);
        const bool coded = keep && c < 4;
        if (coded) {
            const uint32_t g = fbg_clamp_lcp((uint32_t)a.K + c) + 1;
            rs_update(a, rs_col_of_rem(a, rs_rem<FBG_SLOTS_PACKED>(a, p.x & 0x3fffffffu)), g);
            rs_update(a, rs_col_of_rem(a, rs_rem<FBG_SLOTS_PACKED>(a, p.y & 0x3fffffffu)), g);
        }
        keep = keep && !coded;
        const unsigned long long cm = __ballot(coded);
        if (lane == 0 && cm) atomicAdd(s_code_n, (uint32_t)__popcll(cm));
    }
    const unsigned long long mask = __ballot(keep);
    if (!mask) return;
    uint32_t base = 0;
    const int leader = __ffsll((long long)mask) - 1;
    if (lane == leader) base = atomicAdd(s_pair_n, (uint32_t)__popcll(mask));
    base = __shfl(base, leader, 64) + rl_lanes_below(mask);
    if (keep && base < a.tie_region) a.pairs[(size_t)blockIdx.x * a.tie_region + base] = p;
}

__device__ __attribute__((noinline)) void rl_queued(const RankArgs &a, const uint32_t *list, uint32_t n, uint32_t *s_cand_n, uint32_t *s_tie_n)
{
    const int lane = threadIdx.x & 63;
    bool want_cand = false, want_tie = false;
    uint64_t k = 0;
    if ((uint32_t)lane < n) {
        k = list[lane];
        const int64_t base = (int64_t)k - RS_HALO;
        const int lo_i = (int)max((int64_t)0, (int64_t)a.own_lo - base);
        const int hi_i = (int)min((int64_t)(2 * RS_HALO + 1), (int64_t)a.own_hi - base);
        const RsWordView view{a.keys + base, &a, lo_i, hi_i};
        rank_scan_slow(a, view, RS_HALO, lo_i, hi_i, k, want_cand, want_tie);
    }
    rs_append(want_cand, s_cand_n, a.cand, a.region, (uint32_t)k);
    rs_append(want_tie, s_tie_n, a.ties, a.tie_region, (uint32_t)k);
}

template <class E> __device__ __forceinline__ void rl_shift(E *list, uint32_t &n)
{
    const int lane = threadIdx.x & 63;
    const uint32_t rest = n - 64;
    if ((uint32_t)lane < rest) { const E v = list[64 + lane]; list[lane] = v; }
    n = rest;
}

#define RL_ROWS_AHEAD_DEFAULT 3
template <int D, bool EXT>
__global__ __launch_bounds__(RL_THREADS) __attribute__((amdgpu_waves_per_eu(8, 8))) void k_rank_scan_lean(const RankArgs *__restrict__ ap, LeanArgs f)
{
    __shared__ uint2 s_note[RL_WAVES][RL_LIST];
    __shared__ uint32_t s_queue[RL_WAVES][RL_LIST];
    __shared__ uint32_t s_cand_n, s_tie_n, s_pair_n, s_code_n;
    const int lane = threadIdx.x & 63;
    const int wv = __builtin_amdgcn_readfirstlane((int)(threadIdx.x >> 6));
    if (threadIdx.x == 0) { s_cand_n = 0; s_tie_n = 0; s_pair_n = 0; s_code_n = 0; }
    __syncthreads();
    uint2 *my_note = s_note[wv];
    uint32_t *my_queue = s_queue[wv];
    uint32_t nn = 0, nq = 0;
    const uint32_t own_lo = (uint32_t)f.own_lo, own_hi = (uint32_t)f.own_hi;
    const uint32_t wlo = own_lo + ((uint32_t)blockIdx.x * RL_WAVES + (uint32_t)wv) * f.per_wave;
    const uint32_t whi = min(own_hi, wlo + f.per_wave);
    const unsigned long long EVM = ((1ull << (RL_EV_HI + 1)) - 1) & ~((1ull << RL_EV_LO) - 1);
    const unsigned long long RNG = ~(1ull << 63);
    const uint64_t *__restrict__ keys = f.keys;
    const uint8_t *__restrict__ ext = f.ext;
    auto row_slot = [&](uint32_t k0) -> uint32_t { return min(max(k0 - RL_EV_LO + (uint32_t)lane, own_lo), own_hi - 1); };
    auto row = [&](const uint32_t k0, const uint64_t x, const uint32_t ex) __attribute__((always_inline)) {
        const uint32_t slot = k0 - RL_EV_LO + (uint32_t)lane;
        if (k0 < own_lo + 2 * RS_HALO || k0 + RL_EV + 2 * RS_HALO > own_hi || k0 + RL_EV > whi) {
            const unsigned long long Q = EVM & __ballot(slot < whi);
            if ((Q >> lane) & 1ull) my_queue[nq + rl_lanes_below(Q)] = slot;
            nq += (uint32_t)__popcll(Q);
        } else {
            const uint32_t hi = (uint32_t)(x >> 32), lo = (uint32_t)x;
            const uint32_t lo_n = rl_from_next(lo);
            const uint32_t dh = hi ^ rl_from_next(hi), dl = (lo ^ lo_n) >> f.pb;
            const float fr = __builtin_amdgcn_fractf((float)(lo & f.pmask) * f.inv_row_len);
            const float f1 = __uint_as_float(rl_from_next(__float_as_uint(fr))), f2 = __uint_as_float(rl_from_next(__float_as_uint(f1)));
            const float d1 = fabsf(fr - f1), d2 = fabsf(fr - f2);
            const unsigned long long E = __ballot((dh | dl) == 0);
            const unsigned long long R1 = __ballot(d1 < f.eps) | __ballot(d1 > f.one_minus_eps);
            const unsigned long long R2 = __ballot(d2 < f.eps) | __ballot(d2 > f.one_minus_eps);
            const unsigned long long NE = __ballot(fr >= f.near_end) | __ballot(fr < f.eps);
            unsigned long long SS, Q;
            if (((R1 | R2 | NE | (E & (E << 1))) & RNG) == 0) {
                SS = EVM & E & ~((E << 2) | (E >> 2));
                Q = EVM & E & ~SS;
                Q |= Q << 1;
            } else {
                const unsigned long long TIE = E | (E << 1);
                const unsigned long long PH = E & ~((E << 1) | (E >> 1));
                const unsigned long long LONG = TIE & ~(PH | (PH << 1));
                const unsigned long long ADJL = ((LONG >> 1) | (LONG << 1)) & ~TIE;
                SS = EVM & PH & ~(NE | (NE >> 1) | R1 | (R1 << 1) | (R2 << 1) | R2 | (R1 >> 1) | (E << 2) | (E >> 2));
                const unsigned long long QP = EVM & PH & ~SS;
                const unsigned long long RUN = R1 | (R1 << 1) | ((PH & R2) << 2) | ((PH >> 1) & R2);
                Q = QP | (QP << 1) | (EVM & (LONG | ADJL | (~TIE & (RUN | NE))));
            }
            if (SS) {
                uint32_t cx = 0, cy = 0;
                if (EXT) {
                    const uint32_t d = (ex ^ rl_from_next(ex)) & 255u;
                    const uint32_t c = d ? (uint32_t)(__builtin_clz(d) - 24) >> 1 : 4u;
                    cx = c << 30; cy = (c >> 2) << 30;
                }
                if ((SS >> lane) & 1ull) my_note[nn + rl_lanes_below(SS)] = make_uint2((lo & f.pmask) | cx, (lo_n & f.pmask) | cy);
                nn += (uint32_t)__popcll(SS);
            }
            if (Q) {
                if ((Q >> lane) & 1ull) my_queue[nq + rl_lanes_below(Q)] = slot;
                nq += (uint32_t)__popcll(Q);
            }
        }
        while (nq >= 64) { rl_queued(*ap, my_queue, 64, &s_cand_n, &s_tie_n); rl_shift(my_queue, nq); }
        if (nn >= 64) { rl_noted(*ap, my_note, 64, &s_pair_n, &s_code_n); rl_shift(my_note, nn); }
    };
    if constexpr (D == 1) {
        uint64_t xnext = wlo < whi ? keys[row_slot(wlo)] : 0ull;
        uint32_t enext = EXT && wlo < whi ? ext[row_slot(wlo)] : 0u;
        for (uint32_t k0 = wlo; k0 < whi; k0 += RL_EV) {
            const uint64_t x = xnext;
            const uint32_t ex = enext;
            if (k0 + RL_EV < whi) {
                const uint32_t kn = row_slot(k0 + RL_EV);
                xnext = keys[kn];
                if (EXT) enext = ext[kn];
            }
            row(k0, x, ex);
        }
    } else if constexpr (D == 4) {
        uint64_t xs[D];
        uint32_t es[D];
#pragma unroll
        for (int d = 0; d < D; d++) {
            const uint32_t kn = row_slot(wlo + (uint32_t)d * RL_EV);
            xs[d] = keys[kn];
            es[d] = EXT ? ext[kn] : 0u;
        }
        for (uint32_t k0 = wlo; k0 < whi; k0 += D * RL_EV) {
#pragma unroll
            for (int d = 0; d < D; d++) {
                const uint64_t x = xs[d];
                const uint32_t ex = es[d];
                const uint32_t kn = row_slot(k0 + (uint32_t)(D + d) * RL_EV);
                xs[d] = keys[kn];
                es[d] = EXT ? ext[kn] : 0u;
                if (k0 + (uint32_t)d * RL_EV < whi) row(k0 + (uint32_t)d * RL_EV, x, ex);
            }
        }
    } else {
        uint64_t xa[D], xb[D];
        uint32_t ea[D], eb[D];
        auto fetch = [&](const uint32_t k0, uint64_t (&xs)[D], uint32_t (&es)[D]) __attribute__((always_inline)) {
#pragma unroll
            for (int d = 0; d < D; d++) {
                const uint32_t kn = row_slot(k0 + (uint32_t)d * RL_EV);
                xs[d] = keys[kn];
                es[d] = EXT ? ext[kn] : 0u;
            }
        };
        if (wlo < whi) fetch(wlo, xa, ea);
        for (uint32_t k0 = wlo; k0 < whi; k0 += 2 * D * RL_EV) {
            fetch(k0 + D * RL_EV, xb, eb);
#pragma unroll
            for (int d = 0; d < D; d++)
                if (k0 + (uint32_t)d * RL_EV < whi) row(k0 + (uint32_t)d * RL_EV, xa[d], ea[d]);
            fetch(k0 + 2 * D * RL_EV, xa, ea);
#pragma unroll
            for (int d = 0; d < D; d++)
                if (k0 + (uint32_t)(D + d) * RL_EV < whi) row(k0 + (uint32_t)(D + d) * RL_EV, xb[d], eb[d]);
        }
    }
    if (nn) rl_noted(*ap, my_note, nn, &s_pair_n, &s_code_n);
    if (nq) rl_queued(*ap, my_queue, nq, &s_cand_n, &s_tie_n);
    __syncthreads();
    if (threadIdx.x == 0) { ap->blk_count[blockIdx.x] = s_cand_n; ap->tie_count[blockIdx.x] = s_tie_n; ap->pair_count[blockIdx.x] = s_pair_n; }
    if (threadIdx.x == 0 && s_code_n) atomicAdd(&ap->pair_stats[0], (unsigned long long)s_code_n);
}

static bool rs_lean_setup(const RankArgs &a, int pb, unsigned blocks, LeanArgs *f)
{
    const uint64_t own = a.own_hi - a.own_lo, waves = (uint64_t)blocks * RL_WAVES;
    f->per_wave = (uint32_t)(((own + waves - 1) / waves + RL_EV - 1) / RL_EV * RL_EV);
    f->keys = a.keys; f->ext = nullptr; f->own_lo = a.own_lo; f->own_hi = a.own_hi; f->pmask = (uint32_t)a.pmask; f->pb = pb;
    const double L = (double)a.row_len;
    const double delta = (ldexp(1.0, pb - 25) + ldexp(1.0, pb - 22) + 2.0) / L + 1e-6;
    f->inv_row_len = (float)(1.0 / L);
    f->eps = (float)(2.0 * delta);
    f->one_minus_eps = 1.0f - f->eps;
    f->near_end = (float)(1.0 - 65.0 / L - delta);
    return 2.0 * delta < 0.01 && pb <= 31 && a.own_hi < (1ull << 31);
}

template <int L> __global__ __launch_bounds__(256) void k_tie_simple(RankArgs a)
{
    const uint32_t have = a.tie_count[blockIdx.x];
    if (have > a.tie_region) { if (threadIdx.x == 0) a.counters[1] = 1; return; }
    for (uint32_t e = threadIdx.x; e < have; e += blockDim.x) {
        const uint64_t h = a.ties[(size_t)blockIdx.x * a.tie_region + e];
        uint64_t key[RS_TG], pos[RS_TG];
        uint32_t best[RS_TG];
#pragma unroll
        for (int i = 0; i < RS_TG; i++) {
            const bool ok = h + i < a.own_hi;
            const uint64_t w = ok ? a.keys[h + i] : 0ull;
            key[i] = w >> a.pb;
            pos[i] = rs_pos_of<L>(a, w, (ok && L != FBG_SLOTS_PACKED) ? a.vals[h + i] : 0u);
            if (!ok) key[i] = ~key[0];
            best[i] = 0;
        }
        int s = 1;
#pragma unroll
        for (int i = 1; i < RS_TG; i++)
            if (s == i && key[i] == key[0]) s = i + 1;
        const uint64_t x01 = fbg_load8(a.T, pos[0] + a.K) ^ fbg_load8(a.T, pos[1] + a.K);
#pragma unroll
        for (int i = 0; i < RS_TG; i++)
#pragma unroll
            for (int j = i + 1; j < RS_TG; j++)
                if (j < s) {
                    uint32_t x;
                    if (i == 0 && j == 1 && x01 != 0) x = (uint32_t)(__ffsll((unsigned long long)x01) - 1) / 8;
                    else x = fbg_extend_match(a.T, pos[i] + a.K, pos[j] + a.K, 0);
                    best[i] = max(best[i], x);
                    best[j] = max(best[j], x);
                }
#pragma unroll
        for (int i = 0; i < RS_TG; i++)
            if (i < s) rs_update(a, rs_col_of_rem(a, rs_rem<L>(a, pos[i])), fbg_clamp_lcp(best[i] + (uint32_t)a.K) + 1);
    }
}

__global__ __launch_bounds__(256) void k_tie_pairs(RankArgs a)
{
    __shared__ uint32_t s_stats[2];
    const uint32_t have = a.pair_count[blockIdx.x];
    if (have > a.tie_region) { if (threadIdx.x == 0) a.counters[1] = 1; return; }
    if (threadIdx.x < 2) s_stats[threadIdx.x] = 0;
    __syncthreads();
    uint32_t n_code = 0, n_text = 0;
    for (uint32_t e = threadIdx.x; e < have; e += blockDim.x) {
        uint2 p = a.pairs[(size_t)blockIdx.x * a.tie_region + e];
        uint32_t h, from = (uint32_t)a.K;
        const uint32_t c = a.pair_codes ? (p.x >> 30) | (((p.y >> 30) & 1u) << 2) : 4u;
        if (a.pair_codes) { p.x &= 0x3fffffffu; p.y &= 0x3fffffffu; from += 4; }
        if (c < 4) {
            h = c;
            n_code++;
        } else {
            const uint64_t x = fbg_load8(a.T, (uint64_t)p.x + from) ^ fbg_load8(a.T, (uint64_t)p.y + from);
            h = (from - (uint32_t)a.K) +
                (x != 0 ? (uint32_t)(__ffsll((unsigned long long)x) - 1) / 8 : fbg_extend_match(a.T, (uint64_t)p.x + from, (uint64_t)p.y + from, 8));
            n_text++;
        }
        const uint32_t g = fbg_clamp_lcp(h + (uint32_t)a.K) + 1;
        rs_update(a, rs_col_of_rem(a, rs_rem<FBG_SLOTS_PACKED>(a, p.x)), g);
        rs_update(a, rs_col_of_rem(a, rs_rem<FBG_SLOTS_PACKED>(a, p.y)), g);
    }
    if (a.pair_stats) {
        if (n_code) atomicAdd(&s_stats[0], n_code);
        if (n_text) atomicAdd(&s_stats[1], n_text);
        __syncthreads();
        if (threadIdx.x < 2 && s_stats[threadIdx.x]) atomicAdd(&a.pair_stats[threadIdx.x], (unsigned long long)s_stats[threadIdx.x]);
    }
}

__global__ __launch_bounds__(256) void k_tie_sample(const uint64_t *__restrict__ keys, int shift, uint64_t N, int b, int key_bits,
                                                    unsigned long long *__restrict__ counters,
                                                    unsigned int *__restrict__ hist)
{
    __shared__ unsigned int sh[64];
    __shared__ unsigned int sties;
    if (threadIdx.x < 64) sh[threadIdx.x] = 0;
    if (threadIdx.x == 0) sties = 0;
    __syncthreads();
    const uint64_t k = (uint64_t)blockIdx.x * 1024 * 256 + threadIdx.x;
    uint32_t bin = 0xffffffffu;
    if (k < N) {
        const uint64_t key = keys[k] >> shift;
        const uint64_t kp = k > 0 ? keys[k - 1] >> shift : ~key, kn = k + 1 < N ? keys[k + 1] >> shift : ~key;
        if (kp == key || kn == key) {
            bin = 64;
        } else {
            const uint32_t lp = k > 0 ? rs_key_lcp(kp, key, b, key_bits) : 0u;
            const uint32_t ln = k + 1 < N ? rs_key_lcp(key, kn, b, key_bits) : 0u;
            bin = min(max(lp, ln) + 1, 63u);
        }
    }
    {
        const int lane = threadIdx.x & 63;
        unsigned long long rest = __ballot(bin != 0xffffffffu);
        while (rest) {
            const int l = __ffsll((long long)rest) - 1;
            const uint32_t v = __shfl(bin, l, 64);
            const unsigned long long same = __ballot(bin == v);
            if (lane == l) { if (v == 64) atomicAdd(&sties, (uint32_t)__popcll(same)); else atomicAdd(&sh[v], (uint32_t)__popcll(same)); }
            rest &= ~same;
        }
    }
    __syncthreads();
    if (threadIdx.x < 64 && sh[threadIdx.x]) atomicAdd(&hist[threadIdx.x], sh[threadIdx.x]);
    if (threadIdx.x == 0) {
        atomicAdd(&counters[2], (unsigned long long)sties);
        atomicAdd(&counters[3], (unsigned long long)min((uint64_t)256, N - (uint64_t)blockIdx.x * 1024 * 256));
    }
}

#define RS_SAMPLE_BLOCKS 512
__global__ __launch_bounds__(256) void k_tie_sample_loop(const uint64_t *__restrict__ keys, int shift, uint64_t N, int b, int key_bits,
                                                         uint64_t clusters, unsigned long long *__restrict__ counters,
                                                         unsigned int *__restrict__ hist)
{
    __shared__ unsigned int sh[64];
    __shared__ unsigned int sties;
    if (threadIdx.x < 64) sh[threadIdx.x] = 0;
    if (threadIdx.x == 0) sties = 0;
    __syncthreads();
    const int lane = threadIdx.x & 63;
    unsigned long long looked = 0;
    uint64_t w[3] = {0, 0, 0};
    auto fetch = [&](uint64_t c) {
        const uint64_t k = c * 1024 * 256 + threadIdx.x;
        if (k < N) {
            w[1] = keys[k];
            w[0] = k > 0 ? keys[k - 1] : 0ull;
            w[2] = k + 1 < N ? keys[k + 1] : 0ull;
        }
    };
    if (blockIdx.x < clusters) fetch(blockIdx.x);
    for (uint64_t c = blockIdx.x; c < clusters; c += gridDim.x) {
        const uint64_t k = c * 1024 * 256 + threadIdx.x;
        const uint64_t key = w[1] >> shift;
        const uint64_t kp = k > 0 ? w[0] >> shift : ~key, kn = k + 1 < N ? w[2] >> shift : ~key;
        if (c + gridDim.x < clusters) fetch(c + gridDim.x);
        uint32_t bin = 0xffffffffu;
        if (k < N) {
            if (kp == key || kn == key) {
                bin = 64;
            } else {
                const uint32_t lp = k > 0 ? rs_key_lcp(kp, key, b, key_bits) : 0u;
                const uint32_t ln = k + 1 < N ? rs_key_lcp(key, kn, b, key_bits) : 0u;
                bin = min(max(lp, ln) + 1, 63u);
            }
        }
        unsigned long long rest = __ballot(bin != 0xffffffffu);
        while (rest) {
            const int l = __ffsll((long long)rest) - 1;
            const uint32_t v = __shfl(bin, l, 64);
            const unsigned long long same = __ballot(bin == v);
            if (lane == l) { if (v == 64) atomicAdd(&sties, (uint32_t)__popcll(same)); else atomicAdd(&sh[v], (uint32_t)__popcll(same)); }
            rest &= ~same;
        }
        looked += min((uint64_t)256, N - c * 1024 * 256);
    }
    __syncthreads();
    if (threadIdx.x < 64 && sh[threadIdx.x]) atomicAdd(&hist[threadIdx.x], sh[threadIdx.x]);
    if (threadIdx.x == 0 && looked) {
        if (sties) atomicAdd(&counters[2], (unsigned long long)sties);
        atomicAdd(&counters[3], looked);
    }
}

__global__ void k_count_unfilled(const uint32_t *__restrict__ gmax, uint64_t n, uint32_t g_min, int reversed,
                                 unsigned long long *__restrict__ counters)
{
    const uint64_t x = (uint64_t)blockIdx.x * blockDim.x + threadIdx.x;
    const uint64_t rem = reversed ? x + 1 : n - x;
    const bool miss = x < n && rem > 64 && gmax[x] < g_min;
    const unsigned long long mask = __ballot(miss);
    if ((threadIdx.x & 63) == 0 && mask) atomicAdd(&counters[1 + 3], (unsigned long long)__popcll(mask));
}

__global__ void k_cand_compact(const uint32_t *__restrict__ regions, const uint32_t *__restrict__ counts,
                               const uint32_t *__restrict__ offsets, uint32_t region, uint32_t *__restrict__ out)
{
    const uint32_t c = counts[blockIdx.x] < region ? counts[blockIdx.x] : region, o = offsets[blockIdx.x];
    for (uint32_t i = threadIdx.x; i < c; i += blockDim.x) out[o + i] = regions[(size_t)blockIdx.x * region + i];
}

#define RS_CAND_LDS 4096
__global__ __launch_bounds__(256) void k_cand_sort_compact(const uint32_t *__restrict__ regions, const uint32_t *__restrict__ counts,
                                                           const uint32_t *__restrict__ offsets, uint32_t region, uint32_t *__restrict__ out)
{
    __shared__ uint32_t buf[RS_CAND_LDS];
    const uint32_t c = min(min(counts[blockIdx.x], region), (uint32_t)RS_CAND_LDS), o = offsets[blockIdx.x];
    if (c == 0) return;
    uint32_t P = 2;
    while (P < c) P <<= 1;
    for (uint32_t i = threadIdx.x; i < P; i += blockDim.x) buf[i] = i < c ? regions[(size_t)blockIdx.x * region + i] : 0xffffffffu;
    __syncthreads();
    for (uint32_t k = 2; k <= P; k <<= 1)
        for (uint32_t j = k >> 1; j > 0; j >>= 1) {
            for (uint32_t i = threadIdx.x; i < P; i += blockDim.x) {
                const uint32_t l = i ^ j;
                if (l > i) {
                    const uint32_t x = buf[i], y = buf[l];
                    if ((x > y) == ((i & k) == 0)) { buf[i] = y; buf[l] = x; }
                }
            }
            __syncthreads();
        }
    for (uint32_t i = threadIdx.x; i < c; i += blockDim.x) out[o + i] = buf[i];
}

#define RS_COUNTS_THREADS 1024
__global__ __launch_bounds__(RS_COUNTS_THREADS) void k_cand_counts(const uint32_t *__restrict__ counts, uint32_t nb, uint32_t *__restrict__ offs,
                                                                   uint32_t *__restrict__ tot_max)
{
    __shared__ uint32_t wsum[RS_COUNTS_THREADS / 64], wmax[RS_COUNTS_THREADS / 64];
    const uint32_t lane = threadIdx.x & 63, wv = threadIdx.x >> 6;
    const uint32_t per = (nb + RS_COUNTS_THREADS - 1) / RS_COUNTS_THREADS;
    const uint32_t i0 = min(threadIdx.x * per, nb), i1 = min(i0 + per, nb);
    uint32_t sum = 0, mx = 0;
    for (uint32_t i = i0; i < i1; i++) { const uint32_t c = counts[i]; sum += c; mx = max(mx, c); }
    uint32_t inc = sum;
    for (int d = 1; d < 64; d <<= 1) {
        const uint32_t o = __shfl_up(inc, d, 64);
        if (lane >= (uint32_t)d) inc += o;
    }
    for (int d = 32; d > 0; d >>= 1) mx = max(mx, (uint32_t)__shfl_xor(mx, d, 64));
    if (lane == 63) wsum[wv] = inc;
    if (lane == 0) wmax[wv] = mx;
    __syncthreads();
    uint32_t before = inc - sum, total = 0, largest = 0;
    for (uint32_t v = 0; v < RS_COUNTS_THREADS / 64; v++) {
        if (v < wv) before += wsum[v];
        total += wsum[v];
        largest = max(largest, wmax[v]);
    }
    for (uint32_t i = i0; i < i1; i++) { offs[i] = before; before += counts[i]; }
    if (threadIdx.x == 0) { offs[nb] = total; tot_max[0] = total; tot_max[1] = largest; }
}

__global__ void k_cand_inversions(const uint32_t *__restrict__ cand, uint64_t T, unsigned long long *__restrict__ count)
{
    const uint64_t t = (uint64_t)blockIdx.x * blockDim.x + threadIdx.x;
    const unsigned long long mask = __ballot(t + 1 < T && cand[t] >= cand[t + 1]);
    if ((threadIdx.x & 63) == 0 && mask) atomicAdd(count, (unsigned long long)__popcll(mask));
}

#define RS_BIG_GROUPS 1024
#define RS_BIG_MEMBERS 8192
template <int L> __global__ void k_tie_groups(RankArgs a, uint64_t T, int by_list, int gallop)
{
    const uint64_t t = (uint64_t)blockIdx.x * blockDim.x + threadIdx.x;
    if (t >= T) return;
    const uint64_t k0 = by_list ? (uint64_t)a.cand[t] : a.own_lo + t;
    const uint64_t key = rs_key<L>(a, k0);
    if (k0 > a.own_lo && rs_key<L>(a, k0 - 1) == key) return;
    if (k0 + 1 >= a.own_hi || rs_key<L>(a, k0 + 1) != key) return;
    uint32_t s = 1;
    if (gallop) s = fbg_tie_extent(k0, a.own_hi, RS_BIG_MEMBERS, key, [&](uint64_t k) { return rs_key<L>(a, k); });
    else while (k0 + s < a.own_hi && s <= RS_BIG_MEMBERS && rs_key<L>(a, k0 + s) == key) s++;
    if (s > 64) {
        if (s > RS_BIG_MEMBERS) { a.counters[1] = 1; return; }
        const unsigned long long e = atomicAdd(&a.counters[5], 1ull);
        if (e >= RS_BIG_GROUPS) { a.counters[1] = 1; return; }
        a.big[2 * e] = (uint32_t)k0;
        a.big[2 * e + 1] = s;
        return;
    }
    typedef typename PosT<L>::type pos_t;
    pos_t pos[64];
    uint32_t from = (uint32_t)a.K;
    for (uint32_t i = 0; i < s; i++) {
        pos[i] = (pos_t)rs_pos<L>(a, k0 + i);
        if (rs_rem<L>(a, pos[i]) < (uint32_t)a.K) from = 0;
    }
    for (uint32_t i = 1; i < s; i++) {
        const pos_t cur = pos[i];
        uint32_t j = i;
        while (j > 0) {
            const pos_t o = pos[j - 1];
            const uint32_t h = fbg_extend_match(a.T, (uint64_t)o + from, (uint64_t)cur + from, 0);
            if (a.T[(uint64_t)o + from + h] < a.T[(uint64_t)cur + from + h]) break;
            pos[j] = o;
            j--;
        }
        pos[j] = cur;
    }
    for (uint32_t i = 0; i < s; i++) rs_set_pos<L>(a, k0 + i, pos[i]);
}

template <int L> __global__ __launch_bounds__(256) void k_tie_big(RankArgs a, int exact)
{
    __shared__ uint32_t pos_lo[RS_BIG_MEMBERS];
    __shared__ uint8_t pos_hi[L == FBG_SLOTS_WIDE ? RS_BIG_MEMBERS : 1];
    __shared__ uint8_t cls[RS_BIG_MEMBERS];
    __shared__ uint32_t offs[66];
    __shared__ uint32_t q_start, q_count;
    if (blockIdx.x >= a.counters[5]) return;
    const uint64_t k0 = a.big[2 * blockIdx.x];
    const uint32_t s = a.big[2 * blockIdx.x + 1];
    auto member = [&](uint32_t i) -> uint64_t {
        return L == FBG_SLOTS_WIDE ? ((uint64_t)pos_hi[L == FBG_SLOTS_WIDE ? i : 0] << 32) | pos_lo[i] : (uint64_t)pos_lo[i];
    };
    if (threadIdx.x < 66) offs[threadIdx.x] = 0;
    __syncthreads();
    for (uint32_t i = threadIdx.x; i < s; i += blockDim.x) {
        const uint64_t p = rs_pos<L>(a, k0 + i);
        const uint32_t c = min(rs_rem<L>(a, p), (uint32_t)a.K);
        pos_lo[i] = (uint32_t)p;
        if (L == FBG_SLOTS_WIDE) pos_hi[L == FBG_SLOTS_WIDE ? i : 0] = (uint8_t)(p >> 32);
        cls[i] = (uint8_t)c;
        atomicAdd(&offs[c + 1], 1u);
    }
    __syncthreads();
    if (threadIdx.x == 0) {
        q_count = offs[a.K + 1];
        for (int c = 1; c <= a.K + 1; c++) offs[c] += offs[c - 1];
        q_start = offs[a.K];
    }
    __syncthreads();
    if (!exact) {
        for (uint32_t i = threadIdx.x; i < s; i += blockDim.x) {
            const uint32_t dst = atomicAdd(&offs[cls[i]], 1u);
            rs_set_pos<L>(a, k0 + dst, member(i));
        }
        __threadfence();
        __syncthreads();
        if (threadIdx.x == 0) {
            const uint32_t q = q_count;
            if (q > 64) { a.counters[1] = 1; return; }
            const uint64_t kq = k0 + q_start;
            for (uint32_t i = 1; i < q; i++) {
                const uint64_t cur = rs_pos<L>(a, kq + i);
                uint32_t j = i;
                while (j > 0) {
                    const uint64_t o = rs_pos<L>(a, kq + j - 1);
                    const uint32_t h = fbg_extend_match(a.T, o + a.K, cur + a.K, 0);
                    if (a.T[o + a.K + h] < a.T[cur + a.K + h]) break;
                    rs_set_pos<L>(a, kq + j, o);
                    j--;
                }
                rs_set_pos<L>(a, kq + j, cur);
            }
        }
        return;
    }
    for (uint32_t i = threadIdx.x; i < s; i += blockDim.x) {
        const uint64_t p = member(i);
        uint32_t rank = 0;
        for (uint32_t j = 0; j < s; j++) {
            if (j == i) continue;
            const uint64_t o = member(j);
            const uint32_t h = fbg_extend_match(a.T, o, p, 0);
            rank += a.T[o + h] < a.T[p + h] ? 1u : 0u;
        }
        rs_set_pos<L>(a, k0 + rank, p);
    }
}

template <int L> __device__ __forceinline__ uint32_t rs_slot_lcp(const RankArgs &a, uint64_t k)
{
    if (k == (a.first_part ? a.own_lo : 0) || k >= (a.last_part ? a.own_hi : a.N)) return 0;
    const Slot x = rs_slot<L>(a, k - 1), y = rs_slot<L>(a, k);
    if (x.key != y.key) return min(min(rs_key_lcp(x.key, y.key, a.b, a.key_bits), x.rem), y.rem);
    const uint32_t from = (x.rem < (uint32_t)a.K || y.rem < (uint32_t)a.K) ? 0u : (uint32_t)a.K;
    return fbg_clamp_lcp(fbg_extend_match(a.T, (uint64_t)x.pos + from, (uint64_t)y.pos + from, 0) + from);
}

template <int L> __global__ void k_rank_materialize(RankArgs a, uint32_t *sa, uint32_t *isa, uint32_t *pl, uint32_t *pr)
{
    const uint64_t k = (uint64_t)blockIdx.x * blockDim.x + threadIdx.x;
    if (k >= a.N) return;
    const uint32_t p = (uint32_t)rs_pos<L>(a, k);
    sa[k] = p;
    isa[p] = (uint32_t)k;
    pl[p] = rs_slot_lcp<L>(a, k);
    pr[p] = rs_slot_lcp<L>(a, k + 1);
}

template <int L> __global__ void k_runs(RankArgs a, uint64_t T)
{
    const uint64_t t = (uint64_t)blockIdx.x * blockDim.x + threadIdx.x;
    if (t >= T) return;
    const uint64_t k0 = a.cand[t];
    const uint32_t col = rs_col<L>(a, k0);
    if (col == a.n) return;
    if (k0 > a.own_lo && rs_col<L>(a, k0 - 1) == col) return;
    const uint64_t lo_slot = a.first_part ? a.own_lo : 0, hi_slot = a.last_part ? a.own_hi : a.N;
    uint64_t ks = k0;
    while (ks > lo_slot && rs_col<L>(a, ks - 1) == col) ks--;
    if (ks == 0 && !a.first_part) { a.counters[1] = 1; return; }
    uint32_t run = rs_slot_lcp<L>(a, ks);
    uint64_t s = ks;
    for (;;) {
        if (s >= k0 && s < a.own_hi) a.pm[t + (s - k0)] = run;
        if (s + 1 >= hi_slot || rs_col<L>(a, s + 1) != col) break;
        s++;
        if (a.runs_wave_min && s - ks + 1 == a.runs_wave_min) {
            const unsigned long long e = atomicAdd(&a.counters[7], 1ull);
            if (e < a.wl_cap) { a.wl[2 * e] = (uint32_t)t; a.wl[2 * e + 1] = (uint32_t)ks; return; }
        }
        run = min(run, rs_slot_lcp<L>(a, s));
    }
    if (s + 1 == a.N && !a.last_part) { a.counters[1] = 1; return; }
    uint32_t rmin = 0xffffffffu;
    for (;; s--) {
        rmin = min(rmin, rs_slot_lcp<L>(a, s + 1));
        if (s >= k0 && s < a.own_hi) rs_update(a, col, max(a.pm[t + (s - k0)], rmin) + 1);
        if (s == ks || s <= k0) break;
    }
}

template <int L> __global__ __launch_bounds__(64) void k_runs_long(RankArgs a)
{
    if (blockIdx.x >= a.counters[7]) return;
    const uint64_t t = a.wl[2 * blockIdx.x], ks = a.wl[2 * blockIdx.x + 1];
    const uint32_t lane = threadIdx.x;
    const uint32_t col = rs_col<L>(a, ks);
    uint64_t len = 0;
    uint32_t carry = 0xffffffffu;
    for (uint64_t c0 = 0;; c0 += 64) {
        const uint64_t s = ks + c0 + lane;
        const unsigned long long out = ~__ballot(s < a.own_hi && rs_col<L>(a, s) == col);
        const uint32_t cnt = out ? (uint32_t)__ffsll((long long)out) - 1 : 64u;
        uint32_t v = lane < cnt ? rs_slot_lcp<L>(a, s) : 0xffffffffu;
        for (int d = 1; d < 64; d <<= 1) {
            const uint32_t o = __shfl_up(v, d, 64);
            if (lane >= (uint32_t)d) v = min(v, o);
        }
        v = min(v, carry);
        if (lane < cnt) a.pm[t + c0 + lane] = v;
        carry = __shfl(v, 63, 64);
        len += cnt;
        if (cnt < 64) break;
    }
    uint32_t best = 0;
    carry = 0xffffffffu;
    for (uint64_t c0 = (len - 1) / 64 * 64;; c0 -= 64) {
        const uint64_t i = c0 + lane;
        uint32_t v = i < len ? rs_slot_lcp<L>(a, ks + i + 1) : 0xffffffffu;
        for (int d = 1; d < 64; d <<= 1) {
            const uint32_t o = __shfl_down(v, d, 64);
            if (lane + (uint32_t)d < 64) v = min(v, o);
        }
        v = min(v, carry);
        if (i < len) best = max(best, max(a.pm[t + i], v) + 1);
        carry = __shfl(v, 0, 64);
        if (c0 == 0) break;
    }
    for (int d = 32; d > 0; d >>= 1) best = max(best, (uint32_t)__shfl_xor(best, d, 64));
    if (lane == 0) rs_update(a, col, best);
}

struct FinishArgs {
    const uint32_t *gmax;
    uint64_t n, x0, x1;
    int mode, disable_tricks;
    uint64_t *out;
};

__global__ void k_rank_finish(FinishArgs a)
{
    const uint64_t x = a.x0 + (uint64_t)blockIdx.x * blockDim.x + threadIdx.x;
    if (x >= a.x1) return;
    const unsigned long long g = a.gmax[x];
    if (a.mode == FBG_SCAN_V) {
        a.out[x] = g <= x + 1 ? x + 1 - g : x + 1;
        return;
    }
    unsigned long long fx = x;
    const bool any_active = a.disable_tricks || x != 0;
    if (any_active && g > 0) {
        const unsigned long long gg = x + g;
        const unsigned long long fi = gg > a.n ? (a.disable_tricks ? a.n : a.n - 1) : gg - 1;
        fx = max(fx, fi);
    }
    a.out[x] = max((unsigned long long)a.out[x], fx);
}

#define RS_LAUNCH(kernel, layout, grid, block, st, ...)                                                     \
    do {                                                                                                    \
        if ((layout) == FBG_SLOTS_PACKED) hipLaunchKernelGGL((kernel<FBG_SLOTS_PACKED>), grid, block, 0, st, __VA_ARGS__);  \
        else if ((layout) == FBG_SLOTS_WIDE) hipLaunchKernelGGL((kernel<FBG_SLOTS_WIDE>), grid, block, 0, st, __VA_ARGS__); \
        else hipLaunchKernelGGL((kernel<FBG_SLOTS_PAIRS>), grid, block, 0, st, __VA_ARGS__);                                \
    } while (0)

#define RS_LAUNCH_SCAN(layout, plain, grid, st, args)                                                                         \
    do {                                                                                                                     \
        const dim3 blk_(RS_THREADS);                                                                                         \
        if ((layout) == FBG_SLOTS_PACKED) { if (plain) hipLaunchKernelGGL((k_rank_scan<FBG_SLOTS_PACKED, true>), grid, blk_, 0, st, args);   \
                                            else hipLaunchKernelGGL((k_rank_scan<FBG_SLOTS_PACKED, false>), grid, blk_, 0, st, args); }      \
        else if ((layout) == FBG_SLOTS_WIDE) { if (plain) hipLaunchKernelGGL((k_rank_scan<FBG_SLOTS_WIDE, true>), grid, blk_, 0, st, args);  \
                                               else hipLaunchKernelGGL((k_rank_scan<FBG_SLOTS_WIDE, false>), grid, blk_, 0, st, args); }     \
        else { if (plain) hipLaunchKernelGGL((k_rank_scan<FBG_SLOTS_PAIRS, true>), grid, blk_, 0, st, args);                               \
               else hipLaunchKernelGGL((k_rank_scan<FBG_SLOTS_PAIRS, false>), grid, blk_, 0, st, args); }                                  \
    } while (0)

static int rs_fork(fbg_ctx *ctx)
{
    if (!ctx->aux) {
        FBG_HIP_TRY(ctx, hipStreamCreateWithFlags(&ctx->aux, hipStreamNonBlocking));
        FBG_HIP_TRY(ctx, hipEventCreateWithFlags(&ctx->aux_fork, hipEventDisableTiming));
        FBG_HIP_TRY(ctx, hipEventCreateWithFlags(&ctx->aux_join, hipEventDisableTiming));
    }
    FBG_HIP_TRY(ctx, hipEventRecord(ctx->aux_fork, ctx->stream));
    FBG_HIP_TRY(ctx, hipStreamWaitEvent(ctx->aux, ctx->aux_fork, 0));
    ctx->aux_pending = true;
    return FBG_OK;
}
static int rs_join(fbg_ctx *ctx)
{
    if (!ctx->aux_pending) return FBG_OK;
    ctx->aux_pending = false;
    FBG_HIP_TRY(ctx, hipEventRecord(ctx->aux_join, ctx->aux));
    FBG_HIP_TRY(ctx, hipStreamWaitEvent(ctx->stream, ctx->aux_join, 0));
    return FBG_OK;
}

static int rs_wave_list(fbg_ctx *ctx, RankArgs &a)
{
    FBG_TRY(fbg_reserve(ctx, ctx->wave_list, (size_t)2 * RS_WAVE_LIST * 4));
    a.wl = ctx->wave_list.as<uint32_t>();
    const int64_t cap = ctx->opt.wave_list_cap;
    a.wl_cap = cap > 0 && cap < RS_WAVE_LIST ? (uint32_t)cap : RS_WAVE_LIST;
    a.runs_wave_min = ctx->opt.runs_wave_min > 0 ? (uint32_t)ctx->opt.runs_wave_min : 0u;
    return FBG_OK;
}

static int rs_order_candidates(fbg_ctx *ctx, RankArgs &a, int layout, uint64_t T, bool sorted_already, int *launches)
{
    hipStream_t st = ctx->stream;
    FBG_TRY(fbg_reserve(ctx, ctx->dp_a, T * 4));
    FBG_TRY(fbg_reserve(ctx, ctx->dp_b, T * 4));
    uint32_t *sorted = ctx->dp_a.as<uint32_t>();
    uint32_t *flat = ctx->dp_e.as<uint32_t>();
    if (!sorted_already)
        FBG_TRY(fbg_with_tmp(ctx, [&](void *tmp, size_t &bytes) {
            return rocprim::radix_sort_keys(tmp, bytes, flat, sorted, (size_t)T, 0u, 32u, st);
        }));
    if (ctx->opt.cand_sort_check) {
        unsigned long long *d_inv = &fbg_scalars(ctx)->cand_inversions, inv = 0;
        FBG_HIP_TRY(ctx, hipMemsetAsync(d_inv, 0, sizeof(inv), st));
        hipLaunchKernelGGL(k_cand_inversions, dim3(fbg_blocks(T, 256)), dim3(256), 0, st, sorted, T, d_inv);
        FBG_HIP_TRY(ctx, hipMemcpyAsync(&inv, d_inv, sizeof(inv), hipMemcpyDeviceToHost, st));
        FBG_HIP_TRY(ctx, hipStreamSynchronize(st));
        ctx->diag.cand_inversions = (int64_t)inv;
    }
    a.cand = sorted;
    a.pm = ctx->dp_b.as<uint32_t>();
    RS_LAUNCH(k_tie_groups, layout, dim3(fbg_blocks(T, 64)), dim3(64), st, a, T, 1, ctx->opt.tie_gallop != 0 ? 1 : 0);
    RS_LAUNCH(k_tie_big, layout, dim3(RS_BIG_GROUPS), dim3(256), st, a, 0);
    *launches += 3;
    return FBG_OK;
}

static int rs_classify(fbg_ctx *ctx, RankArgs &a, int layout, uint64_t *T_out, int *launches)
{
    hipStream_t st = ctx->stream;
    const uint64_t own = a.own_hi - a.own_lo;
    const unsigned rs_blocks = fbg_blocks(own, RS_CHUNK, 256 * 16);
    const uint32_t region = (uint32_t)((own / rs_blocks) / 8 + 256);
    const uint32_t tie_region = (uint32_t)((own / rs_blocks) / 6 + 256);
    FBG_TRY(fbg_reserve(ctx, ctx->list, (size_t)rs_blocks * region * 4));
    FBG_TRY(fbg_reserve(ctx, ctx->tie_list, (size_t)rs_blocks * tie_region * 4));
    FBG_TRY(fbg_reserve(ctx, ctx->big_groups, RS_BIG_GROUPS * 8));
    a.big = ctx->big_groups.as<uint32_t>();
    if (!a.part_mode) FBG_TRY(rs_wave_list(ctx, a));
    FBG_TRY(fbg_reserve(ctx, ctx->dp_c, (size_t)(rs_blocks + 1) * 4));
    FBG_TRY(fbg_reserve(ctx, ctx->dp_d, (size_t)(rs_blocks + 1) * 4));
    FBG_TRY(fbg_reserve(ctx, ctx->dp_f, (size_t)(rs_blocks + 1) * 4));
    FBG_HIP_TRY(ctx, hipMemsetAsync(ctx->dp_c.p, 0, (size_t)(rs_blocks + 1) * 4, st));
    FBG_HIP_TRY(ctx, hipMemsetAsync(ctx->dp_f.p, 0, (size_t)(rs_blocks + 1) * 4, st));
    a.cand = ctx->list.as<uint32_t>();
    a.blk_count = ctx->dp_c.as<uint32_t>(); a.region = region;
    a.ties = ctx->tie_list.as<uint32_t>();
    a.tie_count = ctx->dp_f.as<uint32_t>(); a.tie_region = tie_region;
    FBG_TRY(fbg_stage_begin(ctx, FBG_STAGE_RANK_KERNEL));
    LeanArgs lf;
    const bool lean = layout == FBG_SLOTS_PACKED && a.g_min > (uint32_t)a.K && !a.values_only && !a.part_mode && !ctx->opt.rank_no_lean &&
                      rs_lean_setup(a, a.pb, rs_blocks, &lf);
    ctx->diag.rank_lean_launched = lean ? 1 : 0;
    if (ctx->opt.cand_sort_check) ctx->diag.cand_inversions = 0;
    if (lean)
    {
        if (ctx->ix.msd_ext_valid && a.keys == ctx->keysA.as<uint64_t>() && a.b == 2 && a.pb <= 30 && a.own_lo == 0 && a.own_hi == ctx->N) {
            lf.ext = ctx->msd_ext.as<uint8_t>();
            a.pair_codes = 1;
            a.pairs_in_scan = ctx->opt.pairs_in_scan != 0;
        }
        a.pair_stats = fbg_scalars(ctx)->pair_stats;
        FBG_HIP_TRY(ctx, hipMemsetAsync(a.pair_stats, 0, 2 * sizeof(unsigned long long), st));
        FBG_TRY(fbg_reserve(ctx, ctx->ps_g, (size_t)rs_blocks * tie_region * 8));
        FBG_TRY(fbg_reserve(ctx, ctx->ps_h, (size_t)rs_blocks * 4));
        a.pairs = ctx->ps_g.as<uint2>(); a.pair_count = ctx->ps_h.as<uint32_t>();
        static_assert(sizeof(RankArgs) <= sizeof(ctx->kargs_host), "room for the scan's arguments");
        FBG_TRY(fbg_reserve(ctx, ctx->kargs, sizeof(RankArgs)));
        memcpy(ctx->kargs_host, &a, sizeof(RankArgs));
        FBG_HIP_TRY(ctx, hipMemcpyAsync(ctx->kargs.p, ctx->kargs_host, sizeof(RankArgs), hipMemcpyHostToDevice, st));
        const RankArgs *d_args = (const RankArgs *)ctx->kargs.p;
#define RL_LAUNCH(D) \
    do { \
        if (lf.ext) hipLaunchKernelGGL((k_rank_scan_lean<D, true>), dim3(rs_blocks), dim3(RL_THREADS), 0, st, d_args, lf); \
        else hipLaunchKernelGGL((k_rank_scan_lean<D, false>), dim3(rs_blocks), dim3(RL_THREADS), 0, st, d_args, lf); \
    } while (0)
        switch (ctx->opt.scan_rows_ahead >= 1 && ctx->opt.scan_rows_ahead <= 4 ? (int)ctx->opt.scan_rows_ahead : RL_ROWS_AHEAD_DEFAULT) {
        case 1: RL_LAUNCH(1); break;
        case 2: RL_LAUNCH(2); break;
        case 3: RL_LAUNCH(3); break;
        default: RL_LAUNCH(4); break;
        }
#undef RL_LAUNCH
    }
    else
        RS_LAUNCH_SCAN(layout, a.g_min <= (uint32_t)a.K || a.values_only, dim3(rs_blocks), st, a);
    FBG_TRY(fbg_stage_end(ctx, FBG_STAGE_RANK_KERNEL, 1));
    {
        hipStream_t ts = st;
        if (!ctx->opt.no_aux_stream) { FBG_TRY(rs_fork(ctx)); ts = ctx->aux; }
        if (lean) hipLaunchKernelGGL(k_tie_pairs, dim3(rs_blocks), dim3(256), 0, ts, a);
        RS_LAUNCH(k_tie_simple, layout, dim3(rs_blocks), dim3(256), ts, a);
    }
    *launches += 2;
    const int rc_rest = [&]() -> int {
        uint32_t *d_counts = a.blk_count, *d_offs = ctx->dp_d.as<uint32_t>();
        uint32_t *d_max = reinterpret_cast<uint32_t *>(a.counters + 6);
        uint32_t tot = 0, mx = 0;
        if (ctx->opt.cand_counts_fused) {
            if (!ctx->pin_pair) FBG_HIP_TRY(ctx, hipHostMalloc(reinterpret_cast<void **>(&ctx->pin_pair), 2 * sizeof(uint32_t), hipHostMallocDefault));
            hipLaunchKernelGGL(k_cand_counts, dim3(1), dim3(RS_COUNTS_THREADS), 0, st, d_counts, (uint32_t)rs_blocks, d_offs, d_max);
            FBG_HIP_TRY(ctx, hipMemcpyAsync(ctx->pin_pair, d_max, 2 * sizeof(uint32_t), hipMemcpyDeviceToHost, st));
            FBG_HIP_TRY(ctx, hipStreamSynchronize(st));
            tot = ctx->pin_pair[0]; mx = ctx->pin_pair[1];
        } else {
            FBG_TRY(fbg_with_tmp(ctx, [&](void *tmp, size_t &bytes) {
                return rocprim::exclusive_scan(tmp, bytes, d_counts, d_offs, 0u, (size_t)(rs_blocks + 1), rocprim::plus<uint32_t>(), st);
            }));
            FBG_TRY(fbg_with_tmp(ctx, [&](void *tmp, size_t &bytes) {
                return rocprim::reduce(tmp, bytes, d_counts, d_max, 0u, (size_t)rs_blocks, rocprim::maximum<uint32_t>(), st);
            }));
            FBG_HIP_TRY(ctx, hipMemcpyAsync(&tot, d_offs + rs_blocks, 4, hipMemcpyDeviceToHost, st));
            FBG_HIP_TRY(ctx, hipMemcpyAsync(&mx, d_max, 4, hipMemcpyDeviceToHost, st));
            FBG_HIP_TRY(ctx, hipStreamSynchronize(st));
        }
        const uint64_t T = tot;
        *T_out = T;
        if (mx > region) { *T_out = ~0ull; return rs_join(ctx); }
        if (T > 0) {
            const int64_t cap_opt = ctx->opt.cand_lds_cap;
            const uint32_t lds_cap = cap_opt > 0 && cap_opt < RS_CAND_LDS ? (uint32_t)cap_opt : RS_CAND_LDS;
            const bool local = lean && ctx->opt.cand_local_sort && mx <= lds_cap;
            ctx->diag.cand_local_sorted = local ? 1 : 0;
            if (local) {
                FBG_TRY(fbg_reserve(ctx, ctx->dp_a, T * 4));
                hipLaunchKernelGGL(k_cand_sort_compact, dim3(rs_blocks), dim3(256), 0, st, a.cand, d_counts, d_offs, region, ctx->dp_a.as<uint32_t>());
            } else {
                FBG_TRY(fbg_reserve(ctx, ctx->dp_e, T * 4));
                hipLaunchKernelGGL(k_cand_compact, dim3(rs_blocks), dim3(256), 0, st, a.cand, d_counts, d_offs, region, ctx->dp_e.as<uint32_t>());
            }
            FBG_TRY(rs_order_candidates(ctx, a, layout, T, local, launches));
        }
        return FBG_OK;
    }();
    if (rc_rest != FBG_OK) { (void)rs_join(ctx); return rc_rest; }
    return FBG_OK;
}

static int rs_zero_counters(fbg_ctx *ctx, unsigned long long *cnt, uint64_t count)
{
    const size_t bytes = 8 * sizeof(unsigned long long) + (count > (1u << 22) ? 64 * sizeof(unsigned int) : 0);
    FBG_HIP_TRY(ctx, hipMemsetAsync(cnt, 0, bytes, ctx->stream));
    return FBG_OK;
}

static int rs_pick_threshold(fbg_ctx *ctx, RankArgs &a, const uint64_t *keys, uint64_t count, const KeyGeom &geom, int *reject,
                             int *launches)
{
    *reject = 0;
    if (count <= (1u << 22)) return FBG_OK;
    hipStream_t st = ctx->stream;
    unsigned long long *cnt = a.counters;
    unsigned int *d_hist = reinterpret_cast<unsigned int *>(cnt + 8);
    const unsigned clusters = fbg_blocks(count, 1024 * 256);
    if (ctx->opt.tie_sample_loop > 0) {
        const unsigned grid = ctx->opt.tie_sample_loop == 1 ? RS_SAMPLE_BLOCKS : (unsigned)std::min<int64_t>(ctx->opt.tie_sample_loop, 4096);
        hipLaunchKernelGGL(k_tie_sample_loop, dim3(std::min(clusters, grid)), dim3(256), 0, st, keys, a.pb, count, geom.b, geom.key_bits,
                           (uint64_t)clusters, cnt, d_hist);
    }
    else
        hipLaunchKernelGGL(k_tie_sample, dim3(clusters), dim3(256), 0, st, keys, a.pb, count, geom.b, geom.key_bits, cnt, d_hist);
    (*launches)++;
    unsigned long long hs[4];
    unsigned int hh[64];
    FBG_HIP_TRY(ctx, hipMemcpyAsync(hs, cnt, sizeof(hs), hipMemcpyDeviceToHost, st));
    FBG_HIP_TRY(ctx, hipMemcpyAsync(hh, d_hist, sizeof(hh), hipMemcpyDeviceToHost, st));
    FBG_HIP_TRY(ctx, hipStreamSynchronize(st));
    if (hs[2] * 4 > hs[3]) { *reject = 1; return FBG_OK; }
    if (!ctx->opt.rank_no_threshold) {
        const double need = 32.0 / (double)ctx->m * (double)hs[3];
        unsigned long long above = 0;
        for (int g = 63; g >= 1; g--) {
            above += hh[g];
            if ((double)above >= need) { a.g_min = (uint32_t)g; break; }
        }
        if ((double)hs[2] / (double)hs[3] * (double)ctx->m >= 32.0) a.g_min = (uint32_t)geom.K + 1;
    }
    return FBG_OK;
}

int fbg_rank_scan_try(fbg_ctx *ctx, uint64_t *keys, uint32_t *vals, const KeyGeom &geom, int *done)
{
    *done = 0;
    const uint64_t N = ctx->N, n = ctx->n;
    const int layout = rs_layout(geom);
    hipStream_t st = ctx->stream;
    FBG_TRY(fbg_stage_begin(ctx, FBG_STAGE_RANKSCAN));
    unsigned long long *cnt = fbg_scalars(ctx)->rank;
    int launches = 0;
    FBG_TRY(fbg_reserve(ctx, ctx->gmax, (n + 1) * 4));
    RankArgs a;
    rs_args_init(ctx, a, keys, vals, N, layout, geom.pb, geom.b, geom.key_bits, geom.K);
    uint64_t T = 0;
    FBG_TRY(rs_zero_counters(ctx, cnt, N));
    FBG_HIP_TRY(ctx, hipMemsetAsync(ctx->gmax.p, 0, (n + 1) * 4, st));
    int reject = 0;
    FBG_TRY(rs_pick_threshold(ctx, a, keys, N, geom, &reject, &launches));
    if (reject) return fbg_stage_end(ctx, FBG_STAGE_RANKSCAN, launches);
    FBG_TRY(rs_classify(ctx, a, layout, &T, &launches));
    if (T == ~0ull) return fbg_stage_end(ctx, FBG_STAGE_RANKSCAN, launches);
    if (T > 0) {
        RS_LAUNCH(k_runs, layout, dim3(fbg_blocks(T, 64)), dim3(64), st, a, T);
        launches++;
        if (a.runs_wave_min) { RS_LAUNCH(k_runs_long, layout, dim3(a.wl_cap), dim3(64), st, a); launches++; }
    }
    FBG_TRY(rs_join(ctx));
    unsigned long long h[8], ps[2] = {0, 0};
    if (a.g_min > 1)
        hipLaunchKernelGGL(k_count_unfilled, dim3(fbg_blocks(n, 256)), dim3(256), 0, st, a.gmax, n, a.g_min, a.reversed, cnt);
    FBG_HIP_TRY(ctx, hipMemcpyAsync(h, cnt, sizeof(h), hipMemcpyDeviceToHost, st));
    if (a.pair_stats) FBG_HIP_TRY(ctx, hipMemcpyAsync(ps, a.pair_stats, sizeof(ps), hipMemcpyDeviceToHost, st));
    FBG_HIP_TRY(ctx, hipStreamSynchronize(st));
    ctx->diag.ext_pairs = (int64_t)ps[0];
    ctx->diag.text_pairs = (int64_t)ps[1];
    ctx->diag.wave_runs = (int64_t)std::min(h[7], (unsigned long long)a.wl_cap);
    launches++;
    if (h[1] != 0) return fbg_stage_end(ctx, FBG_STAGE_RANKSCAN, launches);
    if (a.g_min > 1 && h[4] != 0) {
        a.g_min = 0;
        a.values_only = 1;
        RS_LAUNCH_SCAN(layout, true, dim3(fbg_blocks(N, RS_CHUNK, 256 * 16)), st, a);
        launches++;
    }
    FBG_HIP_TRY(ctx, hipGetLastError());
    ctx->ix.n_exc = 0;
    ctx->ix.kind = IndexKind::ranked;
    ctx->diag.rank_lean_used = ctx->diag.rank_lean_launched;
    fbg_remember_slots(ctx, keys, vals, rs_layout(geom), geom);
    *done = 1;
    return fbg_stage_end(ctx, FBG_STAGE_RANKSCAN, launches);
}

__global__ void k_halo_export(const uint64_t *__restrict__ keys, const uint32_t *__restrict__ vals, uint64_t own_lo,
                              uint64_t own_hi, uint64_t ok, uint8_t *__restrict__ blob)
{
    uint64_t *bk = reinterpret_cast<uint64_t *>(blob);
    uint32_t *bv = reinterpret_cast<uint32_t *>(blob + 2 * FBG_PART_HALO * 8);
    uint64_t *tail = reinterpret_cast<uint64_t *>(blob + 2 * FBG_PART_HALO * 12);
    const uint32_t t = threadIdx.x;
    if (ok & 1) {
        const uint64_t k = t < FBG_PART_HALO ? own_lo + t : own_hi - 2 * FBG_PART_HALO + t;
        bk[t] = keys[k]; bv[t] = vals ? vals[k] : 0u;
    } else { bk[t] = 0; bv[t] = 0; }
    if (t == 0) { tail[0] = ok; tail[1] = own_hi - own_lo; }
}

__global__ void k_halo_import(const uint8_t *__restrict__ blobs, int part, int nparts, uint64_t own_lo, uint64_t own_hi,
                              uint64_t *__restrict__ keys, uint32_t *__restrict__ vals)
{
    const uint32_t t = threadIdx.x;
    if (part > 0) {
        const uint8_t *bl = blobs + (size_t)(part - 1) * FBG_PART_HALO_BYTES;
        keys[t] = reinterpret_cast<const uint64_t *>(bl)[FBG_PART_HALO + t];
        if (vals) vals[t] = reinterpret_cast<const uint32_t *>(bl + 2 * FBG_PART_HALO * 8)[FBG_PART_HALO + t];
    }
    if (part + 1 < nparts) {
        const uint8_t *bl = blobs + (size_t)(part + 1) * FBG_PART_HALO_BYTES;
        keys[own_hi + t] = reinterpret_cast<const uint64_t *>(bl)[t];
        if (vals) vals[own_hi + t] = reinterpret_cast<const uint32_t *>(bl + 2 * FBG_PART_HALO * 8)[t];
    }
}

static void rs_part_args(fbg_ctx *ctx, RankArgs &a)
{
    rs_args_init(ctx, a, ctx->ix.rk_keys, ctx->ix.sa_ptr, ctx->ix.part_count + 2 * FBG_PART_HALO, ctx->ix.rk_layout, ctx->ix.rk_pb, ctx->ix.rk_b,
                 ctx->ix.rk_key_bits, ctx->ix.rk_K);
    a.own_lo = FBG_PART_HALO; a.own_hi = FBG_PART_HALO + ctx->ix.part_count;
    a.first_part = ctx->ix.part == 0; a.last_part = ctx->ix.part + 1 == ctx->ix.nparts;
    a.part_mode = ctx->ix.nparts > 1;
}

int fbg_rank_part_classify(fbg_ctx *ctx, uint64_t *keys, uint32_t *vals, uint64_t count, const KeyGeom &geom, int pre_ok,
                           uint8_t *d_blob, int *ok)
{
    const uint64_t n = ctx->n;
    hipStream_t st = ctx->stream;
    FBG_TRY(fbg_stage_begin(ctx, FBG_STAGE_RANKSCAN));
    int launches = 0;
    ctx->ix.part_count = count;
    ctx->ix.part_T = 0;
    fbg_remember_slots(ctx, keys, vals, rs_layout(geom), geom);
    const int layout = rs_layout(geom);
    FBG_TRY(fbg_reserve(ctx, ctx->gmax, (n + 1) * 4));
    unsigned long long *cnt = fbg_scalars(ctx)->rank;
    FBG_TRY(rs_zero_counters(ctx, cnt, count));
    FBG_HIP_TRY(ctx, hipMemsetAsync(ctx->gmax.p, 0, (n + 1) * 4, st));
    int good = pre_ok && count >= 2 * FBG_PART_HALO;
    RankArgs a;
    rs_part_args(ctx, a);
    if (good) {
        int reject = 0;
        FBG_TRY(rs_pick_threshold(ctx, a, keys + a.own_lo, count, geom, &reject, &launches));
        if (reject) good = 0;
    }
    ctx->ix.part_gmin = a.g_min;
    if (good) {
        uint64_t T = 0;
        FBG_TRY(rs_classify(ctx, a, layout, &T, &launches));
        FBG_TRY(rs_join(ctx));
        if (T == ~0ull) good = 0;
        else {
            ctx->ix.part_T = T;
            unsigned long long h[2];
            FBG_HIP_TRY(ctx, hipMemcpyAsync(h, cnt, sizeof(h), hipMemcpyDeviceToHost, st));
            FBG_HIP_TRY(ctx, hipStreamSynchronize(st));
            if (h[1] != 0) good = 0;
        }
    }
    hipLaunchKernelGGL(k_halo_export, dim3(1), dim3(2 * FBG_PART_HALO), 0, st, keys, vals, a.own_lo, a.own_hi,
                       (uint64_t)good | ((uint64_t)a.g_min << 8), d_blob);
    launches++;
    FBG_HIP_TRY(ctx, hipGetLastError());
    *ok = good;
    return fbg_stage_end(ctx, FBG_STAGE_RANKSCAN, launches);
}

int fbg_rank_part_runs(fbg_ctx *ctx, const uint8_t *d_blobs, uint32_t *d_gmax, int *ok)
{
    const uint64_t n = ctx->n;
    hipStream_t st = ctx->stream;
    FBG_TRY(fbg_stage_begin(ctx, FBG_STAGE_RANKSCAN));
    int launches = 0;
    std::vector<uint8_t> hb((size_t)ctx->ix.nparts * FBG_PART_HALO_BYTES);
    FBG_HIP_TRY(ctx, hipMemcpyAsync(hb.data(), d_blobs, hb.size(), hipMemcpyDeviceToHost, st));
    FBG_HIP_TRY(ctx, hipStreamSynchronize(st));
    int good = 1;
    uint32_t gmin_all = 0;
    for (int p = 0; p < ctx->ix.nparts; p++) {
        uint64_t tail[2];
        memcpy(tail, hb.data() + (size_t)p * FBG_PART_HALO_BYTES + 2 * FBG_PART_HALO * 12, sizeof(tail));
        if (!(tail[0] & 1)) good = 0;
        gmin_all = std::max(gmin_all, (uint32_t)(tail[0] >> 8));
    }
    ctx->ix.part_gmin = gmin_all;
    if (good) {
        RankArgs a;
        rs_part_args(ctx, a);
        a.cand = ctx->dp_a.as<uint32_t>(); a.pm = ctx->dp_b.as<uint32_t>();
        hipLaunchKernelGGL(k_halo_import, dim3(1), dim3(FBG_PART_HALO), 0, st, d_blobs, ctx->ix.part, ctx->ix.nparts, a.own_lo,
                           a.own_hi, a.keys, a.vals);
        launches++;
        if (ctx->ix.part_T > 0) {
            RS_LAUNCH(k_runs, ctx->ix.rk_layout, dim3(fbg_blocks(ctx->ix.part_T, 64)), dim3(64), st, a, ctx->ix.part_T);
            launches++;
            unsigned long long h[2];
            FBG_HIP_TRY(ctx, hipMemcpyAsync(h, a.counters, sizeof(h), hipMemcpyDeviceToHost, st));
            FBG_HIP_TRY(ctx, hipStreamSynchronize(st));
            if (h[1] != 0) good = 0;
        }
    }
    FBG_HIP_TRY(ctx, hipMemcpyAsync(d_gmax, ctx->gmax.p, (n + 1) * 4, hipMemcpyDeviceToDevice, st));
    const uint32_t verdict = good ? 0u : 1u;
    FBG_HIP_TRY(ctx, hipMemcpyAsync(d_gmax + n, &verdict, 4, hipMemcpyHostToDevice, st));
    FBG_HIP_TRY(ctx, hipStreamSynchronize(st));
    *ok = good;
    return fbg_stage_end(ctx, FBG_STAGE_RANKSCAN, launches);
}

int fbg_rank_part_unfilled(fbg_ctx *ctx, uint64_t *unfilled)
{
    *unfilled = 0;
    if (ctx->ix.part_gmin <= 1) return FBG_OK;
    hipStream_t st = ctx->stream;
    unsigned long long *cnt = fbg_scalars(ctx)->rank;
    FBG_HIP_TRY(ctx, hipMemsetAsync(cnt + 4, 0, sizeof(unsigned long long), st));
    hipLaunchKernelGGL(k_count_unfilled, dim3(fbg_blocks(ctx->n, 256)), dim3(256), 0, st, ctx->gmax.as<uint32_t>(), ctx->n, ctx->ix.part_gmin,
                       ctx->reversed, cnt);
    unsigned long long h = 0;
    FBG_HIP_TRY(ctx, hipMemcpyAsync(&h, cnt + 4, sizeof(h), hipMemcpyDeviceToHost, st));
    FBG_HIP_TRY(ctx, hipStreamSynchronize(st));
    *unfilled = h;
    return FBG_OK;
}

int fbg_rank_part_rescan(fbg_ctx *ctx)
{
    FBG_TRY(fbg_stage_begin(ctx, FBG_STAGE_RANKSCAN));
    RankArgs a;
    rs_part_args(ctx, a);
    a.g_min = 0;
    a.values_only = 1;
    RS_LAUNCH_SCAN(ctx->ix.rk_layout, true, dim3(fbg_blocks(ctx->ix.part_count, RS_CHUNK, 256 * 16)), ctx->stream, a);
    FBG_HIP_TRY(ctx, hipGetLastError());
    ctx->ix.part_gmin = 0;
    return fbg_stage_end(ctx, FBG_STAGE_RANKSCAN, 1);
}

int fbg_rank_finish(fbg_ctx *ctx, uint64_t x0, uint64_t x1, int mode, int disable_tricks, uint64_t *d_out)
{
    FinishArgs f;
    f.gmax = ctx->gmax.as<uint32_t>();
    f.n = ctx->n; f.x0 = x0; f.x1 = x1; f.mode = mode; f.disable_tricks = disable_tricks; f.out = d_out;
    hipLaunchKernelGGL(k_rank_finish, dim3(fbg_blocks(x1 - x0, 256)), dim3(256), 0, ctx->stream, f);
    FBG_HIP_TRY(ctx, hipGetLastError());
    return FBG_OK;
}

int fbg_rank_materialize(fbg_ctx *ctx, uint32_t *d_sa, uint32_t *d_isa, uint32_t *d_pl, uint32_t *d_pr)
{
    RankArgs a;
    rs_args_init(ctx, a, ctx->ix.rk_keys, ctx->ix.sa_ptr, ctx->N, ctx->ix.rk_layout, ctx->ix.rk_pb, ctx->ix.rk_b, ctx->ix.rk_key_bits, ctx->ix.rk_K);
    FBG_TRY(fbg_reserve(ctx, ctx->big_groups, RS_BIG_GROUPS * 8));
    a.big = ctx->big_groups.as<uint32_t>();
    FBG_HIP_TRY(ctx, hipMemsetAsync(a.counters + 5, 0, sizeof(unsigned long long), ctx->stream));
    RS_LAUNCH(k_tie_groups, ctx->ix.rk_layout, dim3(fbg_blocks(ctx->N, 256)), dim3(256), ctx->stream, a, ctx->N, 0, ctx->opt.tie_gallop != 0 ? 1 : 0);
    RS_LAUNCH(k_tie_big, ctx->ix.rk_layout, dim3(RS_BIG_GROUPS), dim3(256), ctx->stream, a, 1);
    RS_LAUNCH(k_rank_materialize, ctx->ix.rk_layout, dim3(fbg_blocks(ctx->N, 256)), dim3(256), ctx->stream, a, d_sa, d_isa, d_pl, d_pr);
    FBG_HIP_TRY(ctx, hipGetLastError());
    return FBG_OK;
}
```

Before: 71.51 million.

## Fuse candidate region sort, tie grouping and LCP runs into new tail kernels

Adds a new candidate-tail path, on by default. One region kernel sorts candidates in LDS and resolves small tie groups in the same pass, replacing the separate compact, tie-group and sort launches. A dedicated LCP kernel precomputes per-candidate flags and LCP arrays, and new run kernels use them for per-run prefix and suffix minima, with a wave-scan variant for long runs. This is meant to cut launches and repeated slot/text reads, at the cost of extra device buffers, more LDS use and a more complex code path with its own host-side selftest.

```diff
diff --git a/founderblockgraphs_amd/csrc/cand_tail.h b/founderblockgraphs_amd/csrc/cand_tail.h
--- /dev/null
+++ b/founderblockgraphs_amd/csrc/cand_tail.h
@@ -0,0 +1,101 @@
+#pragma once
+#include <stdint.h>
+
+#if defined(__HIPCC__)
+#define FBG_CT_HD __host__ __device__ __forceinline__
+#define FBG_CT_UNROLL _Pragma("unroll")
+#else
+#define FBG_CT_HD inline
+#define FBG_CT_UNROLL
+#endif
+
+#define FBG_CT_NONE 0xffffffffu
+
+template <class KeyAt> FBG_CT_HD bool fbg_ct_heads_group(uint64_t k, uint64_t lo, uint64_t hi, KeyAt key_at)
+{
+    const uint64_t key = key_at(k);
+    if (k > lo && key_at(k - 1) == key) return false;
+    return k + 1 < hi && key_at(k + 1) == key;
+}
+
+template <class SlotAt, class KeyLocal, class KeySlot>
+FBG_CT_HD uint64_t fbg_ct_key_from(uint32_t i, uint32_t c, uint64_t k0, uint64_t k, SlotAt slot_at, KeyLocal key_local, KeySlot key_slot)
+{
+    const uint64_t j = (uint64_t)i + (k - k0);
+    return j < c && slot_at((uint32_t)j) == k ? key_local((uint32_t)j) : key_slot(k);
+}
+
+template <class RemAt> FBG_CT_HD uint32_t fbg_ct_from(uint32_t s, uint32_t K, RemAt rem_at)
+{
+    uint32_t from = K;
+    for (uint32_t i = 0; i < s; i++)
+        if (rem_at(i) < K) from = 0;
+    return from;
+}
+
+template <class Less> FBG_CT_HD uint32_t fbg_ct_rank(uint32_t me, uint32_t s, Less less)
+{
+    uint32_t rank = 0;
+    for (uint32_t j = 0; j < s; j++) rank += less(j, me) ? 1u : 0u;
+    return rank;
+}
+
+template <int S, class Less> FBG_CT_HD void fbg_ct_small_ranks(uint32_t s, Less less, uint32_t (&rank)[S])
+{
+FBG_CT_UNROLL
+    for (int i = 0; i < S; i++) rank[i] = 0;
+FBG_CT_UNROLL
+    for (int i = 0; i < S; i++)
+FBG_CT_UNROLL
+        for (int j = i + 1; j < S; j++)
+            if ((uint32_t)j < s) {
+                if (less(i, j)) rank[j]++;
+                else rank[i]++;
+            }
+}
+
+
+
+template <class LpAt, class PmSet> FBG_CT_HD uint32_t fbg_ct_min_forward(uint32_t i0, uint32_t i1, uint32_t carry, LpAt lp_at, PmSet pm_set)
+{
+    uint32_t i = i0;
+    for (; i1 - i >= 4; i += 4) {
+        uint32_t v[4];
+FBG_CT_UNROLL
+        for (int q = 0; q < 4; q++) v[q] = lp_at(i + (uint32_t)q);
+FBG_CT_UNROLL
+        for (int q = 0; q < 4; q++) {
+            carry = v[q] < carry ? v[q] : carry;
+            pm_set(i + (uint32_t)q, carry);
+        }
+    }
+    for (; i < i1; i++) {
+        const uint32_t v = lp_at(i);
+        carry = v < carry ? v : carry;
+        pm_set(i, carry);
+    }
+    return carry;
+}
+
+template <class NxAt, class PmAt, class Emit>
+FBG_CT_HD uint32_t fbg_ct_min_backward(uint32_t i0, uint32_t i1, uint32_t carry, NxAt nx_at, PmAt pm_at, Emit emit)
+{
+    uint32_t i = i1;
+    for (; i - i0 >= 4; i -= 4) {
+        uint32_t v[4], p[4];
+FBG_CT_UNROLL
+        for (int q = 0; q < 4; q++) { v[q] = nx_at(i - 1 - (uint32_t)q); p[q] = pm_at(i - 1 - (uint32_t)q); }
+FBG_CT_UNROLL
+        for (int q = 0; q < 4; q++) {
+            carry = v[q] < carry ? v[q] : carry;
+            emit(i - 1 - (uint32_t)q, (p[q] > carry ? p[q] : carry) + 1);
+        }
+    }
+    for (; i > i0; i--) {
+        const uint32_t v = nx_at(i - 1);
+        carry = v < carry ? v : carry;
+        const uint32_t p = pm_at(i - 1);
+        emit(i - 1, (p > carry ? p : carry) + 1);
+    }
+    return carry;
+}
diff --git a/founderblockgraphs_amd/csrc/ctx.hip b/founderblockgraphs_amd/csrc/ctx.hip
--- a/founderblockgraphs_amd/csrc/ctx.hip
+++ b/founderblockgraphs_amd/csrc/ctx.hip
@@ -212,6 +212,7 @@
     {"cand_local_sort", &FbgOptions::cand_local_sort},
     {"cand_lds_cap", &FbgOptions::cand_lds_cap},
     {"cand_sort_check", &FbgOptions::cand_sort_check},
+    {"cand_tail", &FbgOptions::cand_tail},
     {"tie_gallop", &FbgOptions::tie_gallop},
     {"cand_counts_fused", &FbgOptions::cand_counts_fused},
     {"tie_sample_loop", &FbgOptions::tie_sample_loop},
@@ -241,6 +242,7 @@
     {"sample_twins", [](const fbg_ctx &c) -> int64_t { return c.diag.sample_twins; }},
     {"cand_inversions", [](const fbg_ctx &c) -> int64_t { return c.diag.cand_inversions; }},
     {"cand_local_sorted", [](const fbg_ctx &c) -> int64_t { return c.diag.cand_local_sorted; }},
+    {"cand_tail_used", [](const fbg_ctx &c) -> int64_t { return c.diag.cand_tail_used; }},
     {"wave_runs", [](const fbg_ctx &c) -> int64_t { return c.diag.wave_runs; }},
     {"rank_lean_used", [](const fbg_ctx &c) -> int64_t { return c.diag.rank_lean_used; }},
     {"rank_lean_launched", [](const fbg_ctx &c) -> int64_t { return c.diag.rank_lean_launched; }},
diff --git a/founderblockgraphs_amd/csrc/fbg_internal.h b/founderblockgraphs_amd/csrc/fbg_internal.h
--- a/founderblockgraphs_amd/csrc/fbg_internal.h
+++ b/founderblockgraphs_amd/csrc/fbg_internal.h
@@ -37,7 +37,7 @@
             dp_safe_window = 0, dp_tile = 0, pure_scan = 0, gapped_rank = 0, part_tricks_off = 0, msd_sample_bins = 0, msd_min_force = 0, msd_probe = 0, msd_xcd = -1, rank_no_lean = 0, no_stream_upload = 0,
             span_scan = 0, span_key_flags = 0, span_slow_split = 0, poison = 0, dpw_matrix = 0, dp_chain1 = 0, msd_ext = 1, rows_wave = 0,
             pairs_in_scan = 1, runs_wave_min = 16, wave_list_cap = 0,
-            cand_local_sort = 1, cand_lds_cap = 0, cand_sort_check = 0,
+            cand_local_sort = 1, cand_lds_cap = 0, cand_sort_check = 0, cand_tail = 1,
             tie_gallop = 1, cand_counts_fused = 1, tie_sample_loop = 1,
             row_count_fast = 1, twin_hash = 1, front_one_fill = 1,
             scan_rows_ahead = 0, msd_cursors = 1, msd_lds_batch = 1,
@@ -78,6 +78,7 @@
     int64_t wave_runs = -1;
     int64_t cand_inversions = -1;
     int cand_local_sorted = -1;
+    int cand_tail_used = -1;
     int rank_lean_launched = 0;
     int rank_lean_used = 0;
     int pairs_rb = -1;
@@ -172,6 +173,7 @@
     DevBuf keysA, keysB, valsA, valsB, grp, flags, list, tie_list, big_groups, tmp, small, scalars;
     DevBuf msd_ext;
     DevBuf wave_list;
+    DevBuf cand_cf, cand_lp, cand_ln;
     DevBuf kargs;
     alignas(16) unsigned char kargs_host[512];
     uint8_t code_host[256];
diff --git a/founderblockgraphs_amd/csrc/host/host_selftest.cpp b/founderblockgraphs_amd/csrc/host/host_selftest.cpp
--- a/founderblockgraphs_amd/csrc/host/host_selftest.cpp
+++ b/founderblockgraphs_amd/csrc/host/host_selftest.cpp
@@ -4,7 +4,10 @@
 #include <vector>
 #include "fasta.hpp"
 #include "xgfa.hpp"
+#include <algorithm>
+#include <cstring>
 #include "../tie_extent.h"
+#include "../cand_tail.h"
 #include "../twin_hash.h"
 #include "../pindex_stage.h"
 
@@ -50,6 +53,124 @@
     return 0;
 }
 
+static int cand_tail_selftest()
+{
+    uint64_t rng = 0x9e3779b97f4a7c15ull;
+    auto rnd = [&](uint32_t mod) -> uint32_t { rng = rng * 6364136223846793005ull + 1442695040888963407ull; return (uint32_t)(rng >> 33) % mod; };
+    unsigned long long n_groups = 0, n_heads = 0, n_runs = 0;
+    const uint32_t K = 8, n = 60, rows = 80;
+    for (int shorts = 0; shorts < 2; shorts++)
+        for (uint32_t g = 2; g <= 70; g++) {
+            std::string T;
+            std::vector<uint32_t> pos;
+            const uint32_t col = rnd(n - K - 4);
+            std::string stretch;
+            for (uint32_t i = 0; i < K; i++) stretch += shorts ? 'A' : "ACGT"[rnd(4)];
+            for (uint32_t r = 0; r < rows; r++) {
+                std::string row;
+                for (uint32_t i = 0; i < n; i++) row += "ACGT"[rnd(4)];
+                if (shorts && r < K && r < g) {
+                    for (uint32_t i = 0; i < r; i++) row[n - 1 - i] = 'A';
+                    if (r < n) row[n - 1 - r] = 'C';
+                    pos.push_back((uint32_t)T.size() + n - r);
+                } else if (pos.size() < g) {
+                    const uint32_t c = shorts ? col + r % 4 : col;
+                    row.replace(c, K, stretch);
+                    pos.push_back((uint32_t)T.size() + c);
+                }
+                T += row + '#';
+            }
+            T.back() = '\0';
+            T += std::string(64, '\0');
+            if (pos.size() != g) { std::printf("cand_tail: group of %u not built\n", g); return 1; }
+            const uint32_t row_len = n + 1;
+            auto rem_at = [&](uint32_t i) { return n - pos[i] % row_len; };
+            const uint32_t from = fbg_ct_from(g, K, rem_at);
+            if (from != (shorts ? 0u : K)) { std::printf("cand_tail: from %u, group of %u, shorts %d\n", from, g, shorts); return 1; }
+            auto less_from = [&](uint32_t x, uint32_t y, uint32_t f) { return x != y && std::strcmp(T.c_str() + pos[x] + f, T.c_str() + pos[y] + f) < 0; };
+            std::vector<uint32_t> order(g);
+            for (uint32_t i = 0; i < g; i++) order[i] = i;
+            std::sort(order.begin(), order.end(), [&](uint32_t x, uint32_t y) { return less_from(x, y, 0); });
+            std::vector<bool> taken(g, false);
+            for (uint32_t me = 0; me < g; me++) {
+                const uint32_t rank = fbg_ct_rank(me, g, [&](uint32_t j, uint32_t i) { return less_from(j, i, from); });
+                if (rank >= g || order[rank] != me || taken[rank]) { std::printf("cand_tail: rank %u of member %u, group of %u, shorts %d\n", rank, me, g, shorts); return 1; }
+                taken[rank] = true;
+            }
+            if (g <= 4) {
+                uint32_t rank[4];
+                fbg_ct_small_ranks<4>(g, [&](int x, int y) { return less_from((uint32_t)x, (uint32_t)y, from); }, rank);
+                for (uint32_t me = 0; me < g; me++)
+                    if (rank[me] >= g || order[rank[me]] != me) { std::printf("cand_tail: small rank %u of member %u, group of %u\n", rank[me], me, g); return 1; }
+            }
+            n_groups++;
+        }
+    {
+        std::vector<uint64_t> keys;
+        std::vector<uint32_t> cand;
+        uint64_t key = 5;
+        for (uint32_t g = 1; g <= 70; g++)
+            for (uint32_t rep = 0; rep < 2; rep++) {
+                key += 1 + rnd(3);
+                const uint32_t s = rep ? 1 + rnd(3) : g;
+                for (uint32_t i = 0; i < s; i++) {
+                    if (s > 1 || rnd(2)) cand.push_back((uint32_t)keys.size());
+                    keys.push_back(key);
+                }
+            }
+        const uint64_t N = keys.size();
+        for (const uint32_t region : {7u, 64u, 100u, 4096u})
+            for (size_t r0 = 0; r0 < cand.size(); r0 += region) {
+                const uint32_t c = (uint32_t)std::min<size_t>(region, cand.size() - r0);
+                std::vector<uint64_t> local(c);
+                for (uint32_t i = 0; i < c; i++) local[i] = keys[cand[r0 + i]];
+                for (uint32_t i = 0; i < c; i++) {
+                    const uint64_t k0 = cand[r0 + i];
+                    const bool want_head = !(k0 > 0 && keys[k0 - 1] == keys[k0]) && k0 + 1 < N && keys[k0 + 1] == keys[k0];
+                    if (fbg_ct_heads_group(k0, 0, N, [&](uint64_t k) { return keys[k]; }) != want_head) { std::printf("cand_tail: head test at slot %llu\n", (unsigned long long)k0); return 1; }
+                    if (!want_head) continue;
+                    uint32_t want = 1;
+                    while (k0 + want < N && keys[k0 + want] == keys[k0]) want++;
+                    uint64_t local_reads = 0;
+                    auto key_at = [&](uint64_t k) {
+                        return fbg_ct_key_from(i, c, k0, k, [&](uint32_t j) { return (uint64_t)cand[r0 + j]; }, [&](uint32_t j) { local_reads++; return local[j]; },
+                                               [&](uint64_t q) { return keys[q]; });
+                    };
+                    const uint32_t got = fbg_tie_extent(k0, N, 8192, keys[k0], key_at);
+                    if (got != want || (i + want <= c && local_reads == 0)) { std::printf("cand_tail: size %u of the group at slot %llu, want %u, region %u, %llu local reads\n", got, (unsigned long long)k0, want, region, (unsigned long long)local_reads); return 1; }
+                    n_heads++;
+                }
+            }
+    }
+    for (uint32_t len = 1; len <= 200; len++) {
+        std::vector<uint32_t> lp(len + 1);
+        for (auto &v : lp) v = rnd(len % 3 ? 50 : 5);
+        std::vector<uint32_t> want(len);
+        for (uint32_t i = 0; i < len; i++) {
+            uint32_t a = FBG_CT_NONE, b = FBG_CT_NONE;
+            for (uint32_t j = 0; j <= i; j++) a = std::min(a, lp[j]);
+            for (uint32_t j = i + 1; j <= len; j++) b = std::min(b, lp[j]);
+            want[i] = std::max(a, b) + 1;
+        }
+        for (const uint32_t piece : {len, 64u, 7u, 1u}) {
+            std::vector<uint32_t> pm(len, 12345), got(len, 0);
+            uint32_t carry = FBG_CT_NONE;
+            for (uint32_t i0 = 0; i0 < len; i0 += piece)
+                carry = fbg_ct_min_forward(i0, std::min(len, i0 + piece), carry, [&](uint32_t i) { return lp[i]; }, [&](uint32_t i, uint32_t v) { pm[i] = v; });
+            carry = FBG_CT_NONE;
+            for (uint32_t i0 = (len - 1) / piece * piece;; i0 -= piece) {
+                carry = fbg_ct_min_backward(i0, std::min(len, i0 + piece), carry, [&](uint32_t i) { return lp[i + 1]; }, [&](uint32_t i) { return pm[i]; },
+                                            [&](uint32_t i, uint32_t g) { got[i] = g; });
+                if (i0 == 0) break;
+            }
+            if (got != want) { std::printf("cand_tail: run of %u in pieces of %u differs\n", len, piece); return 1; }
+            n_runs++;
+        }
+    }
+    std::printf("cand_tail ok %llu %llu %llu\n", n_groups, n_heads, n_runs);
+    return 0;
+}
+
 static int pindex_stages_selftest()
 {
     std::printf("stages");
@@ -114,6 +235,7 @@
     if (argc == 4 && (std::string(argv[1]) == "twin-hash" || std::string(argv[1]) == "twin-slots"))
         return twin_hash_selftest(argv[2], std::atoi(argv[3]), std::string(argv[1]) == "twin-slots");
     if (argc == 2 && std::string(argv[1]) == "tie-extent") return tie_extent_selftest();
+    if (argc == 2 && std::string(argv[1]) == "cand-tail") return cand_tail_selftest();
     if (argc == 2 && std::string(argv[1]) == "pindex-stages") return pindex_stages_selftest();
     if (argc < 6) {
         std::fprintf(stderr, "usage: %s FASTA GAP_LIMIT ELASTIC PATHS OUT.gfa [BOUNDARY ...]\n", argv[0]);
diff --git a/founderblockgraphs_amd/csrc/rank_scan.hip b/founderblockgraphs_amd/csrc/rank_scan.hip
--- a/founderblockgraphs_amd/csrc/rank_scan.hip
+++ b/founderblockgraphs_amd/csrc/rank_scan.hip
@@ -7,6 +7,7 @@
 
 #include "rank_common.h"
 #include "tie_extent.h"
+#include "cand_tail.h"
 
 #define RS_ITEMS 4
 #define RS_THREADS 256
@@ -741,7 +742,7 @@
         q_start = offs[a.K];
     }
     __syncthreads();
-    if (!exact) {
+    if (exact == 0 || (exact == 2 && q_count <= 64)) {
         for (uint32_t i = threadIdx.x; i < s; i += blockDim.x) {
             const uint32_t dst = atomicAdd(&offs[cls[i]], 1u);
             rs_set_pos<L>(a, k0 + dst, member(i));
@@ -780,13 +781,17 @@
     }
 }
 
-template <int L> __device__ __forceinline__ uint32_t rs_slot_lcp(const RankArgs &a, uint64_t k)
-{
-    if (k == (a.first_part ? a.own_lo : 0) || k >= (a.last_part ? a.own_hi : a.N)) return 0;
-    const Slot x = rs_slot<L>(a, k - 1), y = rs_slot<L>(a, k);
+__device__ __forceinline__ uint32_t rs_pair_lcp(const RankArgs &a, const Slot &x, const Slot &y)
+{
     if (x.key != y.key) return min(min(rs_key_lcp(x.key, y.key, a.b, a.key_bits), x.rem), y.rem);
     const uint32_t from = (x.rem < (uint32_t)a.K || y.rem < (uint32_t)a.K) ? 0u : (uint32_t)a.K;
     return fbg_clamp_lcp(fbg_extend_match(a.T, (uint64_t)x.pos + from, (uint64_t)y.pos + from, 0) + from);
+}
+
+template <int L> __device__ __forceinline__ uint32_t rs_slot_lcp(const RankArgs &a, uint64_t k)
+{
+    if (k == (a.first_part ? a.own_lo : 0) || k >= (a.last_part ? a.own_hi : a.N)) return 0;
+    return rs_pair_lcp(a, rs_slot<L>(a, k - 1), rs_slot<L>(a, k));
 }
 
 template <int L> __global__ void k_rank_materialize(RankArgs a, uint32_t *sa, uint32_t *isa, uint32_t *pl, uint32_t *pr)
@@ -874,6 +879,274 @@
     if (lane == 0) rs_update(a, col, best);
 }
 
+#define RC_SMALL 4
+
+__device__ __forceinline__ bool rc_text_less(const uint8_t *__restrict__ T, uint64_t po, uint64_t pc, uint64_t wo, uint64_t wc)
+{
+    const uint64_t x = wo ^ wc;
+    if (x == 0) {
+        const uint32_t h = fbg_extend_match(T, po, pc, 8);
+        return T[po + h] < T[pc + h];
+    }
+    const uint32_t sh = (uint32_t)(__ffsll((unsigned long long)x) - 1) & ~7u;
+    return ((wo >> sh) & 0xff) < ((wc >> sh) & 0xff);
+}
+
+__device__ __forceinline__ void rc_wave_sync()
+{
+    __builtin_amdgcn_fence(__ATOMIC_RELEASE, "wavefront");
+    __builtin_amdgcn_wave_barrier();
+    __builtin_amdgcn_fence(__ATOMIC_ACQUIRE, "wavefront");
+}
+
+__device__ __forceinline__ void rc_bitonic_pairs(uint32_t *buf, uint32_t base, uint32_t t0, uint32_t t1, uint32_t step, uint32_t j, uint32_t k)
+{
+    for (uint32_t t = t0; t < t1; t += step) {
+        const uint32_t i = base + (((t & ~(j - 1)) << 1) | (t & (j - 1))), l = i + j;
+        const uint32_t x = buf[i], y = buf[l];
+        if ((x > y) == ((i & k) == 0)) { buf[i] = y; buf[l] = x; }
+    }
+}
+
+#define RC_WORDS 1024
+__global__ __launch_bounds__(256) void k_cand_region(RankArgs a, const uint32_t *__restrict__ counts, const uint32_t *__restrict__ offsets,
+                                                     uint32_t *__restrict__ out, int gallop, uint32_t cap, uint32_t pmax, uint32_t wcap, uint32_t lcap)
+{
+    constexpr int L = FBG_SLOTS_PACKED;
+    extern __shared__ uint64_t rc_lds[];
+    uint64_t *wbuf = rc_lds;
+    uint32_t *buf = reinterpret_cast<uint32_t *>(wbuf + wcap);
+    uint32_t *glist = buf + pmax;
+    uint16_t *hlist = reinterpret_cast<uint16_t *>(glist + lcap);
+    __shared__ uint32_t gcount, hcount;
+    const uint32_t c = min(min(counts[blockIdx.x], a.region), cap), o = offsets[blockIdx.x];
+    if (c == 0) return;
+    const uint32_t wc = min(c, wcap), hcap = cap / 2 + 2;
+    uint32_t P = 2;
+    while (P < c) P <<= 1;
+    for (uint32_t i = threadIdx.x; i < P; i += blockDim.x) buf[i] = i < c ? a.cand[(size_t)blockIdx.x * a.region + i] : 0xffffffffu;
+    if (threadIdx.x == 0) { gcount = 0; hcount = 0; }
+    __syncthreads();
+    const uint32_t wv = threadIdx.x >> 6, lane = threadIdx.x & 63;
+    const uint32_t Q = P >= 256 ? P >> 2 : P;
+    for (uint32_t k = 2; k <= P; k <<= 1)
+        for (uint32_t j = k >> 1; j > 0; j >>= 1) {
+            if (j >= Q) {
+                __syncthreads();
+                rc_bitonic_pairs(buf, 0, threadIdx.x, P >> 1, blockDim.x, j, k);
+                __syncthreads();
+            } else if (wv * Q < P) {
+                rc_bitonic_pairs(buf, wv * Q, lane, Q >> 1, 64, j, k);
+                rc_wave_sync();
+            }
+        }
+    __syncthreads();
+    for (uint32_t i0 = threadIdx.x; i0 < c; i0 += 4 * blockDim.x) {
+        uint64_t k[4], w[4], wp[4], wn[4];
+#pragma unroll
+        for (int q = 0; q < 4; q++) k[q] = buf[min(i0 + (uint32_t)q * blockDim.x, c - 1)];
+#pragma unroll
+        for (int q = 0; q < 4; q++) {
+            w[q] = a.keys[k[q]];
+            wp[q] = a.keys[k[q] > 0 ? k[q] - 1 : k[q]];
+            wn[q] = a.keys[k[q] + 1 < a.N ? k[q] + 1 : k[q]];
+        }
+#pragma unroll
+        for (int q = 0; q < 4; q++) {
+            const uint32_t i = i0 + (uint32_t)q * blockDim.x;
+            if (i >= c) continue;
+            out[o + i] = (uint32_t)k[q];
+            if (i < wc) wbuf[i] = w[q];
+            const uint64_t key = w[q] >> a.pb;
+            if (!(k[q] > 0 && (wp[q] >> a.pb) == key) && k[q] + 1 < a.N && (wn[q] >> a.pb) == key) {
+                const uint32_t e = atomicAdd(&hcount, 1u);
+                if (e < hcap) hlist[e] = (uint16_t)i;
+                else a.counters[1] = 1;
+            }
+        }
+    }
+    __syncthreads();
+    const uint32_t n_heads = min(hcount, hcap);
+    for (uint32_t h = threadIdx.x; h < n_heads; h += blockDim.x) {
+        const uint32_t i = hlist[h];
+        const uint64_t k0 = buf[i], w0 = i < wc ? wbuf[i] : a.keys[k0], key = w0 >> a.pb;
+        auto word_at = [&](uint32_t d) -> uint64_t {
+            const uint32_t j = i + d;
+            return j < wc && buf[j] == k0 + d ? wbuf[j] : a.keys[k0 + d];
+        };
+        auto key_at = [&](uint64_t k) -> uint64_t {
+            return fbg_ct_key_from(i, wc, k0, k, [&](uint32_t j) { return (uint64_t)buf[j]; }, [&](uint32_t j) { return wbuf[j] >> a.pb; },
+                                   [&](uint64_t s) { return a.keys[s] >> a.pb; });
+        };
+        uint32_t s = 1;
+        if (gallop) s = fbg_tie_extent(k0, a.N, RS_BIG_MEMBERS, key, key_at);
+        else while (k0 + s < a.N && s <= RS_BIG_MEMBERS && key_at(k0 + s) == key) s++;
+        if (s > 64) {
+            if (s > RS_BIG_MEMBERS) { a.counters[1] = 1; continue; }
+            const unsigned long long e = atomicAdd(&a.counters[5], 1ull);
+            if (e >= RS_BIG_GROUPS) { a.counters[1] = 1; continue; }
+            a.big[2 * e] = (uint32_t)k0;
+            a.big[2 * e + 1] = s;
+            continue;
+        }
+        if (s > RC_SMALL) {
+            const uint32_t e = atomicAdd(&gcount, 1u);
+            if (e < lcap) glist[e] = i | s << 16;
+            else a.counters[1] = 1;
+            continue;
+        }
+        uint32_t p[RC_SMALL];
+        uint64_t w8[RC_SMALL];
+#pragma unroll
+        for (int d = 0; d < RC_SMALL; d++) p[d] = (uint32_t)(((uint32_t)d < s ? word_at(d) : w0) & a.pmask);
+        uint32_t from = (uint32_t)a.K;
+#pragma unroll
+        for (int d = 0; d < RC_SMALL; d++)
+            if (rs_rem<L>(a, p[d]) < (uint32_t)a.K) from = 0;
+#pragma unroll
+        for (int d = 0; d < RC_SMALL; d++) w8[d] = fbg_load8(a.T, (uint64_t)p[d] + from);
+        uint32_t rank[RC_SMALL];
+        fbg_ct_small_ranks<RC_SMALL>(s, [&](int x, int y) { return rc_text_less(a.T, (uint64_t)p[x] + from, (uint64_t)p[y] + from, w8[x], w8[y]); }, rank);
+#pragma unroll
+        for (int d = 0; d < RC_SMALL; d++)
+            if ((uint32_t)d < s) a.keys[k0 + rank[d]] = key << a.pb | p[d];
+    }
+    __syncthreads();
+    const uint32_t groups = min(gcount, lcap);
+    for (uint32_t e = threadIdx.x >> 6; e < groups; e += blockDim.x >> 6) {
+        const uint32_t i = glist[e] & 0xffffu, s = glist[e] >> 16;
+        const uint64_t k0 = buf[i];
+        const uint32_t d = lane < s ? lane : 0u, j = i + d;
+        const uint64_t w = j < wc && buf[j] == k0 + d ? wbuf[j] : a.keys[k0 + d];
+        const uint32_t p = (uint32_t)(w & a.pmask);
+        const uint32_t from = __ballot(rs_rem<L>(a, p) < (uint32_t)a.K) ? 0u : (uint32_t)a.K;
+        const uint64_t w8 = fbg_load8(a.T, (uint64_t)p + from);
+        const uint32_t rank = fbg_ct_rank(lane, s, [&](uint32_t x, uint32_t) {
+            const uint32_t px = (uint32_t)__shfl((int)p, (int)x, 64);
+            const uint64_t wx = (uint64_t)(uint32_t)__shfl((int)(uint32_t)w8, (int)x, 64) | (uint64_t)(uint32_t)__shfl((int)(uint32_t)(w8 >> 32), (int)x, 64) << 32;
+            return lane < s && x != lane && rc_text_less(a.T, (uint64_t)px + from, (uint64_t)p + from, wx, w8);
+        });
+        if (lane < s) a.keys[k0 + rank] = (w & ~a.pmask) | p;
+    }
+}
+
+#define RC_HEAD 0x80000000u
+#define RC_TAIL 0x40000000u
+#define RC_COL 0x3fffffffu
+__global__ __launch_bounds__(256) void k_cand_lcp(RankArgs a, uint64_t T, uint32_t *__restrict__ cf, uint32_t *__restrict__ lp, uint32_t *__restrict__ ln)
+{
+    constexpr int L = FBG_SLOTS_PACKED;
+    const uint64_t t = (uint64_t)blockIdx.x * blockDim.x + threadIdx.x;
+    if (t >= T) return;
+    const uint64_t k = a.cand[t];
+    const uint64_t next_cand = t + 1 < T ? (uint64_t)a.cand[t + 1] : ~0ull;
+    const bool has_p = k > 0, has_n = k + 1 < a.N;
+    const uint64_t w = a.keys[k], wp = has_p ? a.keys[k - 1] : 0ull, wn = has_n ? a.keys[k + 1] : 0ull;
+    auto slot_of = [&](uint64_t word) {
+        Slot s;
+        s.key = word >> a.pb;
+        s.pos = word & a.pmask;
+        s.rem = rs_rem<L>(a, s.pos);
+        s.col = rs_col_of_rem(a, s.rem);
+        return s;
+    };
+    const Slot y = slot_of(w), x = slot_of(wp), z = slot_of(wn);
+    uint32_t f = y.col;
+    if (!(has_p && x.col == y.col)) f |= RC_HEAD;
+    if (!(has_n && z.col == y.col)) f |= RC_TAIL;
+    cf[t] = f;
+    lp[t] = has_p ? rs_pair_lcp(a, x, y) : 0u;
+    if (next_cand != k + 1) ln[t] = has_n ? rs_pair_lcp(a, y, z) : 0u;
+}
+
+__device__ __forceinline__ uint32_t rc_end_lcp(const RankArgs &a, uint64_t T, uint64_t t, uint64_t len, const uint32_t *__restrict__ lp,
+                                               const uint32_t *__restrict__ ln)
+{
+    const uint64_t e = t + len;
+    return e < T && a.cand[e] == a.cand[e - 1] + 1 ? lp[e] : ln[e - 1];
+}
+
+__global__ __launch_bounds__(256) void k_cand_runs(RankArgs a, uint64_t T, const uint32_t *__restrict__ cf, const uint32_t *__restrict__ lp,
+                                                   const uint32_t *__restrict__ ln, uint32_t *__restrict__ pm)
+{
+    const uint64_t t = (uint64_t)blockIdx.x * blockDim.x + threadIdx.x;
+    if (t >= T) return;
+    const uint32_t f0 = cf[t], col = f0 & RC_COL;
+    if (col == (uint32_t)a.n || !(f0 & RC_HEAD)) return;
+    const uint64_t room = T - t;
+    uint64_t len = 0;
+    bool tried = false;
+    for (uint64_t i0 = 0; i0 < room && !len; i0 += 4) {
+        uint32_t g[4];
+#pragma unroll
+        for (int q = 0; q < 4; q++) g[q] = cf[min(t + i0 + q, T - 1)];
+#pragma unroll
+        for (int q = 0; q < 4; q++)
+            if (!len && i0 + q < room && (g[q] & RC_TAIL)) len = i0 + q + 1;
+        const uint64_t known = len ? len : i0 + 5;
+        if (!tried && a.runs_wave_min >= 2 && known >= a.runs_wave_min) {
+            tried = true;
+            const unsigned long long e = atomicAdd(&a.counters[7], 1ull);
+            if (e < a.wl_cap) { a.wl[2 * e] = (uint32_t)t; a.wl[2 * e + 1] = a.cand[t]; return; }
+        }
+    }
+    if (!len) len = room;
+    const uint32_t n_mem = (uint32_t)len;
+    fbg_ct_min_forward(0u, n_mem, FBG_CT_NONE, [&](uint32_t i) { return lp[t + i]; }, [&](uint32_t i, uint32_t v) { pm[t + i] = v; });
+    const uint32_t end = rc_end_lcp(a, T, t, len, lp, ln);
+    uint32_t best = 0;
+    fbg_ct_min_backward(0u, n_mem, FBG_CT_NONE, [&](uint32_t i) { return i + 1 < n_mem ? lp[t + i + 1] : end; },
+                        [&](uint32_t i) { return pm[t + i]; }, [&](uint32_t, uint32_t g) { best = max(best, g); });
+    rs_update(a, col, best);
+}
+
+__global__ __launch_bounds__(64) void k_cand_runs_long(RankArgs a, uint64_t T, const uint32_t *__restrict__ cf, const uint32_t *__restrict__ lp,
+                                                       const uint32_t *__restrict__ ln, uint32_t *__restrict__ pm)
+{
+    if (blockIdx.x >= a.counters[7]) return;
+    const uint64_t t = a.wl[2 * blockIdx.x];
+    const uint32_t lane = threadIdx.x;
+    const uint32_t col = cf[t] & RC_COL;
+    uint64_t len = 0;
+    uint32_t carry = FBG_CT_NONE;
+    for (uint64_t c0 = 0; t + c0 < T; c0 += 64) {
+        const uint64_t idx = t + c0 + lane;
+        const bool valid = idx < T;
+        const uint32_t f = valid ? cf[idx] : 0u;
+        const unsigned long long stop = __ballot(valid && (f & RC_TAIL)), inval = __ballot(!valid);
+        const uint32_t first_stop = stop ? (uint32_t)__ffsll((long long)stop) - 1 : 64u, first_inv = inval ? (uint32_t)__ffsll((long long)inval) - 1 : 64u;
+        const uint32_t cnt = min(min(first_stop + 1, first_inv), 64u);
+        uint32_t v = lane < cnt ? lp[idx] : FBG_CT_NONE;
+        for (int d = 1; d < 64; d <<= 1) {
+            const uint32_t o = __shfl_up(v, d, 64);
+            if (lane >= (uint32_t)d) v = min(v, o);
+        }
+        v = min(v, carry);
+        if (lane < cnt) pm[idx] = v;
+        carry = __shfl(v, 63, 64);
+        len += cnt;
+        if (first_stop < 64 || first_inv < 64) break;
+    }
+    if (len == 0) return;
+    const uint32_t end = rc_end_lcp(a, T, t, len, lp, ln);
+    uint32_t best = 0;
+    carry = FBG_CT_NONE;
+    for (uint64_t c0 = (len - 1) / 64 * 64;; c0 -= 64) {
+        const uint64_t i = c0 + lane;
+        uint32_t v = i < len ? (i + 1 < len ? lp[t + i + 1] : end) : FBG_CT_NONE;
+        for (int d = 1; d < 64; d <<= 1) {
+            const uint32_t o = __shfl_down(v, d, 64);
+            if (lane + (uint32_t)d < 64) v = min(v, o);
+        }
+        v = min(v, carry);
+        if (i < len) best = max(best, max(pm[t + i], v) + 1);
+        carry = __shfl(v, 0, 64);
+        if (c0 == 0) break;
+    }
+    for (int d = 32; d > 0; d >>= 1) best = max(best, (uint32_t)__shfl_xor(best, d, 64));
+    if (lane == 0) rs_update(a, col, best);
+}
+
 struct FinishArgs {
     const uint32_t *gmax;
     uint64_t n, x0, x1;
@@ -949,7 +1222,19 @@
     return FBG_OK;
 }
 
-static int rs_order_candidates(fbg_ctx *ctx, RankArgs &a, int layout, uint64_t T, bool sorted_already, int *launches)
+static int rs_check_sorted(fbg_ctx *ctx, const uint32_t *sorted, uint64_t T)
+{
+    hipStream_t st = ctx->stream;
+    unsigned long long *d_inv = &fbg_scalars(ctx)->cand_inversions, inv = 0;
+    FBG_HIP_TRY(ctx, hipMemsetAsync(d_inv, 0, sizeof(inv), st));
+    hipLaunchKernelGGL(k_cand_inversions, dim3(fbg_blocks(T, 256)), dim3(256), 0, st, sorted, T, d_inv);
+    FBG_HIP_TRY(ctx, hipMemcpyAsync(&inv, d_inv, sizeof(inv), hipMemcpyDeviceToHost, st));
+    FBG_HIP_TRY(ctx, hipStreamSynchronize(st));
+    ctx->diag.cand_inversions = (int64_t)inv;
+    return FBG_OK;
+}
+
+static int rs_order_candidates(fbg_ctx *ctx, RankArgs &a, int layout, uint64_t T, bool sorted_already, int big_mode, int *launches)
 {
     hipStream_t st = ctx->stream;
     FBG_TRY(fbg_reserve(ctx, ctx->dp_a, T * 4));
@@ -960,19 +1245,31 @@
         FBG_TRY(fbg_with_tmp(ctx, [&](void *tmp, size_t &bytes) {
             return rocprim::radix_sort_keys(tmp, bytes, flat, sorted, (size_t)T, 0u, 32u, st);
         }));
-    if (ctx->opt.cand_sort_check) {
-        unsigned long long *d_inv = &fbg_scalars(ctx)->cand_inversions, inv = 0;
-        FBG_HIP_TRY(ctx, hipMemsetAsync(d_inv, 0, sizeof(inv), st));
-        hipLaunchKernelGGL(k_cand_inversions, dim3(fbg_blocks(T, 256)), dim3(256), 0, st, sorted, T, d_inv);
-        FBG_HIP_TRY(ctx, hipMemcpyAsync(&inv, d_inv, sizeof(inv), hipMemcpyDeviceToHost, st));
-        FBG_HIP_TRY(ctx, hipStreamSynchronize(st));
-        ctx->diag.cand_inversions = (int64_t)inv;
-    }
+    if (ctx->opt.cand_sort_check) FBG_TRY(rs_check_sorted(ctx, sorted, T));
     a.cand = sorted;
     a.pm = ctx->dp_b.as<uint32_t>();
     RS_LAUNCH(k_tie_groups, layout, dim3(fbg_blocks(T, 64)), dim3(64), st, a, T, 1, ctx->opt.tie_gallop != 0 ? 1 : 0);
-    RS_LAUNCH(k_tie_big, layout, dim3(RS_BIG_GROUPS), dim3(256), st, a, 0);
+    RS_LAUNCH(k_tie_big, layout, dim3(RS_BIG_GROUPS), dim3(256), st, a, big_mode);
     *launches += 3;
+    return FBG_OK;
+}
+
+static int rs_region_groups(fbg_ctx *ctx, RankArgs &a, unsigned rs_blocks, uint64_t T, uint32_t mx, const uint32_t *d_counts, const uint32_t *d_offs, int *launches)
+{
+    hipStream_t st = ctx->stream;
+    FBG_TRY(fbg_reserve(ctx, ctx->dp_a, T * 4));
+    FBG_TRY(fbg_reserve(ctx, ctx->dp_b, T * 4));
+    uint32_t *sorted = ctx->dp_a.as<uint32_t>();
+    uint32_t pmax = 2;
+    while (pmax < mx) pmax <<= 1;
+    const uint32_t wcap = std::min<uint32_t>(mx, RC_WORDS), lcap = mx / (RC_SMALL + 1) + 1;
+    const size_t lds = (size_t)wcap * 8 + (size_t)pmax * 4 + (size_t)lcap * 4 + (size_t)(mx / 2 + 2) * 2;
+    hipLaunchKernelGGL(k_cand_region, dim3(rs_blocks), dim3(256), lds, st, a, d_counts, d_offs, sorted, ctx->opt.tie_gallop != 0 ? 1 : 0, mx, pmax, wcap, lcap);
+    if (ctx->opt.cand_sort_check) FBG_TRY(rs_check_sorted(ctx, sorted, T));
+    a.cand = sorted;
+    a.pm = ctx->dp_b.as<uint32_t>();
+    hipLaunchKernelGGL(k_tie_big<FBG_SLOTS_PACKED>, dim3(RS_BIG_GROUPS), dim3(256), 0, st, a, 2);
+    *launches += 2;
     return FBG_OK;
 }
 
@@ -1003,6 +1300,7 @@
                       rs_lean_setup(a, a.pb, rs_blocks, &lf);
     ctx->diag.rank_lean_launched = lean ? 1 : 0;
     if (ctx->opt.cand_sort_check) ctx->diag.cand_inversions = 0;
+    ctx->diag.cand_tail_used = 0;
     if (lean)
     {
         if (ctx->ix.msd_ext_valid && a.keys == ctx->keysA.as<uint64_t>() && a.b == 2 && a.pb <= 30 && a.own_lo == 0 && a.own_hi == ctx->N) {
@@ -1072,6 +1370,9 @@
             const uint32_t lds_cap = cap_opt > 0 && cap_opt < RS_CAND_LDS ? (uint32_t)cap_opt : RS_CAND_LDS;
             const bool local = lean && ctx->opt.cand_local_sort && mx <= lds_cap;
             ctx->diag.cand_local_sorted = local ? 1 : 0;
+            const bool tail = local && ctx->opt.cand_tail != 0 && a.n <= RC_COL;
+            ctx->diag.cand_tail_used = tail ? 1 : 0;
+            if (tail) return rs_region_groups(ctx, a, rs_blocks, T, mx, d_counts, d_offs, launches);
             if (local) {
                 FBG_TRY(fbg_reserve(ctx, ctx->dp_a, T * 4));
                 hipLaunchKernelGGL(k_cand_sort_compact, dim3(rs_blocks), dim3(256), 0, st, a.cand, d_counts, d_offs, region, ctx->dp_a.as<uint32_t>());
@@ -1079,7 +1380,7 @@
                 FBG_TRY(fbg_reserve(ctx, ctx->dp_e, T * 4));
                 hipLaunchKernelGGL(k_cand_compact, dim3(rs_blocks), dim3(256), 0, st, a.cand, d_counts, d_offs, region, ctx->dp_e.as<uint32_t>());
             }
-            FBG_TRY(rs_order_candidates(ctx, a, layout, T, local, launches));
+            FBG_TRY(rs_order_candidates(ctx, a, layout, T, local, lean ? 2 : 0, launches));
         }
         return FBG_OK;
     }();
@@ -1149,7 +1450,18 @@
     if (reject) return fbg_stage_end(ctx, FBG_STAGE_RANKSCAN, launches);
     FBG_TRY(rs_classify(ctx, a, layout, &T, &launches));
     if (T == ~0ull) return fbg_stage_end(ctx, FBG_STAGE_RANKSCAN, launches);
-    if (T > 0) {
+    if (T > 0 && ctx->diag.cand_tail_used == 1) {
+        int rc = fbg_reserve(ctx, ctx->cand_cf, T * 4);
+        if (rc == FBG_OK) rc = fbg_reserve(ctx, ctx->cand_lp, T * 4);
+        if (rc == FBG_OK) rc = fbg_reserve(ctx, ctx->cand_ln, T * 4);
+        if (rc != FBG_OK) { (void)rs_join(ctx); return rc; }
+        uint32_t *cf = ctx->cand_cf.as<uint32_t>(), *lp = ctx->cand_lp.as<uint32_t>(), *ln = ctx->cand_ln.as<uint32_t>();
+        hipLaunchKernelGGL(k_cand_lcp, dim3(fbg_blocks(T, 256)), dim3(256), 0, st, a, T, cf, lp, ln);
+        hipLaunchKernelGGL(k_cand_runs, dim3(fbg_blocks(T, 256)), dim3(256), 0, st, a, T, cf, lp, ln, a.pm);
+        launches += 2;
+        if (a.runs_wave_min) { hipLaunchKernelGGL(k_cand_runs_long, dim3(a.wl_cap), dim3(64), 0, st, a, T, cf, lp, ln, a.pm); launches++; }
+    }
+    else if (T > 0) {
         RS_LAUNCH(k_runs, layout, dim3(fbg_blocks(T, 64)), dim3(64), st, a, T);
         launches++;
         if (a.runs_wave_min) { RS_LAUNCH(k_runs_long, layout, dim3(a.wl_cap), dim3(64), st, a); launches++; }
```

Result: faster. 73.16 million, median of 6 (+2.3%).
